# pramasoul/lac

Measured on AMD Instinct MI355X. Metric: encoded symbols/sec at vocab=32000, batch=4096 streams; bit-exact round-trip, higher is better.
Workload: dtype u32; 1 GPU; c3: vocab=32000, 4096 streams/GPU, 16 symbols/stream per job, prec=48, uint32 pmf rows; vocab=32000, streams=4096, prec=48, pmf_bits=32, input=pmf, parallelism=streams sharded over 1 GPU(s)

## Files before the change

include/lac.h:

```cpp
#ifndef LAC_H
#define LAC_H

#include <stdint.h>

#ifdef __cplusplus
extern "C" {
#endif

typedef struct lac_ctx lac_ctx;

enum {
    LAC_OK = 0,
    LAC_E_ARG = -1,
    LAC_E_PREC = -2,
    LAC_E_SYMBOL_RANGE = -3,
    LAC_E_ZERO_WIDTH = -4,
    LAC_E_TABLE = -5,
    LAC_E_DECODE_RANGE = -6,
    LAC_E_CAPACITY = -7,
    LAC_E_HIP = -8,
    LAC_E_STATE = -9,
    LAC_E_FLUSH_ZERO_WIDTH = -10,
    LAC_E_FLUSH_LOOP = -11,
    LAC_E_UNDETERMINED = -12
};

enum {
    LAC_OPT_ENCODE_PATH = 1,
    LAC_OPT_FUSED_MIN_STREAMS = 2,
    LAC_OPT_MAPPING = 3,
    LAC_OPT_TERMINATION = 4,
    LAC_OPT_DECODE_PATH = 5,
    LAC_OPT_Q1_SHAPE = 6,
    LAC_OPT_DECODE_FINE = 7,
    LAC_OPT_BLOCK_WAVES = 8,
    LAC_OPT_DECODE_STOP = 9,
    LAC_OPT_Q1_STEP = 10
};
enum {
    LAC_MAP_CEIL = 0,
    LAC_MAP_FLOOR = 1
};
enum {
    LAC_TERM_FLUSH = 0,
    LAC_TERM_ACSAMPLER = 1
};
enum {
    LAC_PATH_AUTO = 0,
    LAC_PATH_SPLIT = 1,
    LAC_PATH_FUSED = 2,
    LAC_PATH_STATS = 3,
    LAC_PATH_BLOCK = 4
};

const char *lac_version(void);
const char *lac_last_error(void);

int lac_open(int device, int prec, int64_t vocab, int64_t streams, int pmf_bits,
             uint64_t capacity_bits, lac_ctx **out);
int lac_close(lac_ctx *ctx);

int lac_set_option(lac_ctx *ctx, int option, int64_t value);

int lac_set_stream_lengths(lac_ctx *ctx, const int64_t *len_dev, void *stream);

int lac_encode_reset(lac_ctx *ctx, void *stream);

int lac_encode(lac_ctx *ctx, const void *pmf_dev, int64_t step_stride, int64_t stream_stride,
               const int32_t *sym_dev, int64_t steps, uint64_t *trace_dev, void *stream);

int lac_encode_job(lac_ctx *ctx, const void *pmf_dev, int64_t step_stride, int64_t stream_stride,
                   const int32_t *sym_dev, int64_t steps, uint64_t *trace_dev, void *stream);

int lac_encode_rebase(lac_ctx *ctx, void *stream);

int lac_encode_drain(lac_ctx *ctx, uint8_t *dst_dev, uint64_t dst_stride_bytes, uint64_t *fill_dev, void *stream);

int lac_encode_finish(lac_ctx *ctx, void *stream);

int lac_stream_status(lac_ctx *ctx, int32_t *err_host, int64_t *err_step_host, void *stream);

int lac_encoded_lengths(lac_ctx *ctx, uint64_t *nbits_host, void *stream);

int lac_encoded_device(lac_ctx *ctx, const uint8_t **bits_dev, uint64_t *stride_bytes,
                       const uint64_t **nbits_dev);

int lac_copy_bits(lac_ctx *ctx, uint8_t *dst_host, uint64_t dst_stride, void *stream);

int lac_copy_bits_dev(lac_ctx *ctx, uint8_t *dst_dev, uint64_t dst_stride, void *stream);

int lac_copy_nbits_dev(lac_ctx *ctx, uint64_t *dst_dev, void *stream);

int lac_pack_bits(lac_ctx *ctx, uint8_t *dst_dev, int hdr_bytes, uint64_t *len_dev, void *stream);

int lac_pack_bits_at(lac_ctx *ctx, uint8_t *dst_dev, uint64_t dst_bytes, int hdr_bytes, const uint64_t *base_dev,
                     uint64_t *end_dev, uint64_t *len_out, void *stream);

int lac_pack_jobs(int device, const uint64_t *planeA_dev, uint64_t plane_stride, const uint64_t *nbits_dev,
                  int64_t jobs, int64_t streams, uint64_t cap_words, uint8_t *dst_dev, uint64_t dst_bytes,
                  int hdr_bytes, const uint64_t *base_dev, uint64_t *ends_dev, uint64_t *lens_out, void *stream);

int lac_unpack_jobs(int device, const uint8_t *src_dev, uint64_t src_bytes, int hdr_bytes,
                    const uint64_t *counts_dev, const uint64_t *base_dev,
                    int64_t jobs, int64_t streams,
                    uint8_t *bits_dev, uint64_t stride_bytes, uint64_t job_stride_bytes,
                    uint64_t *nbits_dev, uint64_t *ends_dev, int32_t *status_dev, void *stream);

int lac_set_output(lac_ctx *ctx, uint64_t *planeA_dev, uint64_t *nbits_dev);

int lac_host_alloc(uint64_t bytes, void **host_out, void **dev_out);
int lac_host_free(void *host);

int lac_encoder_registers(lac_ctx *ctx, int64_t *l_host, int64_t *h_host, void *stream);

int lac_flush_digits(lac_ctx *ctx, int8_t *digits_host, int32_t *count_host, void *stream);

typedef struct lac_enc_state {
    int64_t l, h;
    uint64_t L, wa, wc;
    int64_t nsym;
    int32_t err, nflush;
    int64_t err_step;
    int8_t flush[8];
} lac_enc_state;
int lac_encode_get_state(lac_ctx *ctx, lac_enc_state *host_out, uint64_t *planes_host, void *stream);
int lac_encode_set_state(lac_ctx *ctx, const lac_enc_state *host_in, const uint64_t *planes_host, void *stream);

int lac_decode_open(lac_ctx *ctx, const uint8_t *bits_dev, uint64_t stride_bytes,
                    const uint64_t *nbits_dev, void *stream);

int lac_decode_open_packed(lac_ctx *ctx, const uint8_t *src_dev, uint64_t src_bytes, int hdr_bytes,
                           const uint64_t *counts_dev, const uint64_t *base_dev, uint64_t *end_dev,
                           void *stream);

int lac_decode_open_window(lac_ctx *ctx, const uint8_t *bits_dev, uint64_t stride_bytes,
                           const uint64_t *nbits_dev, const uint64_t *base_words_dev, void *stream);
int lac_decode_refill(lac_ctx *ctx, void *stream);
int lac_decode_window_base(lac_ctx *ctx, uint64_t *base_words_host, void *stream);

int lac_decode_step(lac_ctx *ctx, const void *pmf_dev, int64_t stream_stride,
                    int32_t *sym_out_dev, void *stream);

int lac_decode_steps(lac_ctx *ctx, const void *pmf_dev, int64_t step_stride, int64_t stream_stride,
                     int64_t steps, int32_t *sym_out_dev, void *stream);

#define LAC_LOGITS_BF16 1
#define LAC_LOGITS_F32 2

int lac_q1_k(int prec, int64_t vocab);

int lac_encode_logits_job(lac_ctx *ctx, const void *logits_dev, int logit_type, int64_t step_stride,
                          int64_t stream_stride, const int32_t *sym_dev, int64_t steps, uint64_t *trace_dev,
                          void *stream);

int lac_encode_logits(lac_ctx *ctx, const void *logits_dev, int logit_type, int64_t step_stride,
                      int64_t stream_stride, const int32_t *sym_dev, int64_t steps, uint64_t *trace_dev,
                      void *stream);

int lac_decode_logits_steps(lac_ctx *ctx, const void *logits_dev, int logit_type, int64_t step_stride,
                            int64_t stream_stride, int64_t steps, int32_t *sym_out_dev, void *stream);

int lac_decode_logits_step(lac_ctx *ctx, const void *logits_dev, int logit_type, int64_t stream_stride,
                           int32_t *sym_out_dev , void *stream);
int lac_encode_logits_step(lac_ctx *ctx, const void *logits_dev, int logit_type, int64_t stream_stride,
                           const int32_t *sym_dev , uint64_t *trace_dev, void *stream);

int lac_q1_group_aborted(lac_ctx *ctx, int64_t *aborted, void *stream);

int lac_quantize_logits(lac_ctx *ctx, const void *logits_dev, int logit_type, int64_t step_stride,
                        int64_t stream_stride, int64_t steps, uint32_t *pmf_out_dev, void *stream);

int lac_decode_determined(lac_ctx *ctx, int64_t *ndet_host, void *stream);

typedef struct lac_dec_state {
    int64_t l, h, x;
    uint64_t pos;
    int64_t nsym;
    int32_t err, det;
    int64_t err_step, ndet;
} lac_dec_state;

int lac_decode_get_state(lac_ctx *ctx, lac_dec_state *host_out, void *stream);
int lac_decode_set_state(lac_ctx *ctx, const lac_dec_state *host_in, void *stream);

#define LAC_TAIL_DECIDE 0
#define LAC_TAIL_FLUSH 1
typedef struct lac_tail_state {
    int64_t l, h, lb, hb;
    int32_t err, done;
    int64_t still, nsym;
} lac_tail_state;

int lac_decode_tail_begin(lac_ctx *ctx, void *stream);
int lac_decode_tail_step(lac_ctx *ctx, const void *pmf_dev, int64_t stream_stride, int mode,
                         int64_t *sym_out_dev, int32_t *code_out_dev, void *stream);
int lac_decode_tail_get_state(lac_ctx *ctx, lac_tail_state *host_out, void *stream);
int lac_decode_tail_set_state(lac_ctx *ctx, const lac_tail_state *host_in, void *stream);

int lac_hc_encode_symbol(int prec, int64_t *l, int64_t *h, int64_t lo, int64_t hi, int8_t *digits,
                         int32_t *ndigits);
int lac_hc_encode_flush(int prec, int64_t l, int64_t h, int8_t *digits, int32_t *ndigits);
int lac_hc_decode_emit(int prec, int64_t *regs, int64_t lo, int64_t hi, int renormalise);

int lac_profile_enable(lac_ctx *ctx, int on);
int lac_profile_read(lac_ctx *ctx, double *ms_total , int64_t *launches , int reset);

#ifdef __cplusplus
}
#endif
#endif
```

lac_amd/_lib.py:

```python
from __future__ import annotations

import ctypes as C
import os

HERE = os.path.dirname(os.path.abspath(__file__))
LIB_PATH = os.environ.get("LAC_LIB") or os.path.join(HERE, "liblac.so")

LAC_OK = 0
LAC_E_ARG = -1
LAC_E_PREC = -2
LAC_E_SYMBOL_RANGE = -3
LAC_E_ZERO_WIDTH = -4
LAC_E_TABLE = -5
LAC_E_DECODE_RANGE = -6
LAC_E_CAPACITY = -7
LAC_E_HIP = -8
LAC_E_STATE = -9
LAC_E_FLUSH_ZERO_WIDTH = -10
LAC_E_FLUSH_LOOP = -11
LAC_E_UNDETERMINED = -12

STATUS_NAMES = {
    LAC_OK: "LAC_OK", LAC_E_ARG: "LAC_E_ARG", LAC_E_PREC: "LAC_E_PREC",
    LAC_E_SYMBOL_RANGE: "LAC_E_SYMBOL_RANGE", LAC_E_ZERO_WIDTH: "LAC_E_ZERO_WIDTH",
    LAC_E_TABLE: "LAC_E_TABLE", LAC_E_DECODE_RANGE: "LAC_E_DECODE_RANGE",
    LAC_E_CAPACITY: "LAC_E_CAPACITY", LAC_E_HIP: "LAC_E_HIP", LAC_E_STATE: "LAC_E_STATE",
    LAC_E_FLUSH_ZERO_WIDTH: "LAC_E_FLUSH_ZERO_WIDTH", LAC_E_FLUSH_LOOP: "LAC_E_FLUSH_LOOP",
    LAC_E_UNDETERMINED: "LAC_E_UNDETERMINED",
}

_vp, _i, _i64, _u64 = C.c_void_p, C.c_int, C.c_int64, C.c_uint64
PROTOTYPES = [
    ("lac_version", C.c_char_p, []),
    ("lac_last_error", C.c_char_p, []),
    ("lac_open", _i, [_i, _i, _i64, _i64, _i, _u64, C.POINTER(_vp)]),
    ("lac_close", _i, [_vp]),
    ("lac_set_stream_lengths", _i, [_vp, _vp, _vp]),
    ("lac_encode_reset", _i, [_vp, _vp]),
    ("lac_encode", _i, [_vp, _vp, _i64, _i64, _vp, _i64, _vp, _vp]),
    ("lac_encode_job", _i, [_vp, _vp, _i64, _i64, _vp, _i64, _vp, _vp]),
    ("lac_set_option", _i, [_vp, _i, _i64]),
    ("lac_encode_finish", _i, [_vp, _vp]),
    ("lac_encode_rebase", _i, [_vp, _vp]),
    ("lac_encode_drain", _i, [_vp, _vp, _u64, _vp, _vp]),
    ("lac_stream_status", _i, [_vp, _vp, _vp, _vp]),
    ("lac_encoded_lengths", _i, [_vp, _vp, _vp]),
    ("lac_encoded_device", _i, [_vp, C.POINTER(_vp), C.POINTER(_u64), C.POINTER(_vp)]),
    ("lac_copy_bits", _i, [_vp, _vp, _u64, _vp]),
    ("lac_copy_bits_dev", _i, [_vp, _vp, _u64, _vp]),
    ("lac_copy_nbits_dev", _i, [_vp, _vp, _vp]),
    ("lac_pack_bits", _i, [_vp, _vp, C.c_int, _vp, _vp]),
    ("lac_pack_bits_at", _i, [_vp, _vp, _u64, C.c_int, _vp, _vp, _vp, _vp]),
    ("lac_pack_jobs", _i, [C.c_int, _vp, _u64, _vp, _i64, _i64, _u64, _vp, _u64, C.c_int, _vp, _vp, _vp, _vp]),
    ("lac_unpack_jobs", _i, [C.c_int, _vp, _u64, C.c_int, _vp, _vp, _i64, _i64, _vp, _u64, _u64, _vp, _vp, _vp, _vp]),
    ("lac_decode_open_packed", _i, [_vp, _vp, _u64, C.c_int, _vp, _vp, _vp, _vp]),
    ("lac_set_output", _i, [_vp, _vp, _vp]),
    ("lac_host_alloc", _i, [_u64, C.POINTER(_vp), C.POINTER(_vp)]),
    ("lac_host_free", _i, [_vp]),
    ("lac_encode_get_state", _i, [_vp, _vp, _vp, _vp]),
    ("lac_encode_set_state", _i, [_vp, _vp, _vp, _vp]),
    ("lac_flush_digits", _i, [_vp, _vp, _vp, _vp]),
    ("lac_encoder_registers", _i, [_vp, _vp, _vp, _vp]),
    ("lac_decode_open", _i, [_vp, _vp, _u64, _vp, _vp]),
    ("lac_decode_open_window", _i, [_vp, _vp, _u64, _vp, _vp, _vp]),
    ("lac_decode_refill", _i, [_vp, _vp]),
    ("lac_decode_window_base", _i, [_vp, _vp, _vp]),
    ("lac_decode_step", _i, [_vp, _vp, _i64, _vp, _vp]),
    ("lac_decode_steps", _i, [_vp, _vp, _i64, _i64, _i64, _vp, _vp]),
    ("lac_decode_determined", _i, [_vp, _vp, _vp]),
    ("lac_decode_get_state", _i, [_vp, _vp, _vp]),
    ("lac_decode_set_state", _i, [_vp, _vp, _vp]),
    ("lac_decode_tail_begin", _i, [_vp, _vp]),
    ("lac_decode_tail_step", _i, [_vp, _vp, _i64, _i, _vp, _vp, _vp]),
    ("lac_decode_tail_get_state", _i, [_vp, _vp, _vp]),
    ("lac_decode_tail_set_state", _i, [_vp, _vp, _vp]),
    ("lac_hc_encode_symbol", _i, [_i, _vp, _vp, _i64, _i64, _vp, _vp]),
    ("lac_hc_encode_flush", _i, [_i, _i64, _i64, _vp, _vp]),
    ("lac_hc_decode_emit", _i, [_i, _vp, _i64, _i64, _i]),
    ("lac_q1_group_aborted", _i, [_vp, _vp, _vp]),
    ("lac_profile_enable", _i, [_vp, _i]),
    ("lac_profile_read", _i, [_vp, _vp, _vp, _i]),
    ("lac_q1_k", _i, [_i, _i64]),
    ("lac_encode_logits_job", _i, [_vp, _vp, _i, _i64, _i64, _vp, _i64, _vp, _vp]),
    ("lac_encode_logits", _i, [_vp, _vp, _i, _i64, _i64, _vp, _i64, _vp, _vp]),
    ("lac_decode_logits_steps", _i, [_vp, _vp, _i, _i64, _i64, _i64, _vp, _vp]),
    ("lac_quantize_logits", _i, [_vp, _vp, _i, _i64, _i64, _i64, _vp, _vp]),
    ("lac_decode_logits_step", _i, [_vp, _vp, _i, _i64, _vp, _vp]),
    ("lac_encode_logits_step", _i, [_vp, _vp, _i, _i64, _vp, _vp, _vp]),
]

KERNEL_IDS = {"row_stats": 0, "encode": 1, "finish": 2, "decode_step": 3, "encode_fused": 4, "decode_wave": 5,
              "q1_stats": 6, "q1_decode": 7}
LAC_LOGITS_BF16, LAC_LOGITS_F32 = 1, 2
LAC_OPT_ENCODE_PATH = 1
LAC_OPT_FUSED_MIN_STREAMS = 2
LAC_PATH_AUTO, LAC_PATH_SPLIT, LAC_PATH_FUSED, LAC_PATH_STATS, LAC_PATH_BLOCK = 0, 1, 2, 3, 4
LAC_OPT_MAPPING = 3
LAC_OPT_TERMINATION = 4
LAC_OPT_DECODE_PATH = 5
LAC_OPT_Q1_SHAPE = 6
LAC_OPT_DECODE_FINE = 7
LAC_OPT_BLOCK_WAVES = 8
LAC_OPT_DECODE_STOP = 9
LAC_OPT_Q1_STEP = 10
Q1_STEP_MODES = {"auto": 0, "fused": 1, "split": 2}
LAC_MAP_CEIL, LAC_MAP_FLOOR = 0, 1
LAC_TERM_FLUSH, LAC_TERM_ACSAMPLER = 0, 1
LAC_TAIL_DECIDE, LAC_TAIL_FLUSH = 0, 1


class LacLibraryError(RuntimeError):
    pass


class LacError(RuntimeError):
    def __init__(self, code, msg=""):
        super().__init__(f"{STATUS_NAMES.get(code, code)}: {msg}")
        self.code = code


_lib = None


def load():
    global _lib
    if _lib is not None:
        return _lib
    if not os.path.exists(LIB_PATH):
        raise LacLibraryError(f"{LIB_PATH} is missing: build it with `python -m lac_amd.build` "
                              "(hipcc --offload-arch=gfx950); there is no CPU fallback")
    try:
        lib = C.CDLL(LIB_PATH)
    except OSError as e:
        raise LacLibraryError(f"cannot load {LIB_PATH}: {e}") from e
    for name, res, args in PROTOTYPES:
        try:
            f = getattr(lib, name)
        except AttributeError:
            if os.environ.get("LAC_LIB"):
                continue
            raise LacLibraryError(f"{LIB_PATH} lacks {name}: rebuild it (python -m lac_amd.build)") from None
        f.restype = res
        f.argtypes = args
    _lib = lib
    return lib


def check(rc):
    if rc != LAC_OK:
        raise LacError(rc, load().lac_last_error().decode(errors="replace"))
    return rc
```

lac_amd/batch.py:

```python
from __future__ import annotations

import ctypes as C
import sys

import numpy as np

from . import _lib
from ._lib import LacError, check



def _torch():
    import torch
    return torch


def _stream_handle(device):
    torch = _torch()
    return C.c_void_p(torch.cuda.current_stream(device).cuda_stream)


ENC_STATE = np.dtype([("l", "<i8"), ("h", "<i8"), ("L", "<u8"), ("wa", "<u8"), ("wc", "<u8"), ("nsym", "<i8"),
                      ("err", "<i4"), ("nflush", "<i4"), ("err_step", "<i8"), ("flush", "i1", (8,))])

# ... 208 lines not shown
            raise ValueError("lengths must fit int64")
        dev = torch.from_numpy(np.ascontiguousarray(n, dtype=np.int64)).to(self.device)
        check(self.lib.lac_set_stream_lengths(self.ctx, C.c_void_p(dev.data_ptr()), self._stream))
        self._len_keep = dev

    def lengths(self):
        n = np.zeros(self.streams, dtype=np.uint64)
        check(self.lib.lac_encoded_lengths(self.ctx, n.ctypes.data_as(C.c_void_p), self._stream))
        return n

    def device_bits(self):
        p, s, n = C.c_void_p(), C.c_uint64(), C.c_void_p()
        check(self.lib.lac_encoded_device(self.ctx, C.byref(p), C.byref(s), C.byref(n)))
        return p.value, s.value, n.value

    def bits_tensor(self, stride=None):
        torch = _torch()
        _, s, _ = self.device_bits()
        stride = int(stride or s)
        out = torch.zeros((self.streams, stride), dtype=torch.uint8, device=self.device)
        check(self.lib.lac_copy_bits_dev(self.ctx, C.c_void_p(out.data_ptr()), stride, self._stream))
        return out

    def bits_stride(self):
        return int(self.device_bits()[1])

    def copy_bits_into(self, out):
        if out.dim() != 2 or out.shape[0] != self.streams or out.stride(1) != 1 or out.dtype != _torch().uint8:
            raise ValueError("out must be a uint8 [streams, W] tensor with contiguous rows")
        check(self.lib.lac_copy_bits_dev(self.ctx, C.c_void_p(out.data_ptr()), out.stride(0), self._stream))
        return out

    def copy_nbits_into(self, out):
        if out.shape != (self.streams,) or not out.is_contiguous() or out.element_size() != 8:
            raise ValueError("out must be a contiguous 8-byte integer tensor [streams]")
        check(self.lib.lac_copy_nbits_dev(self.ctx, C.c_void_p(out.data_ptr()), self._stream))
        return out

    def pack_bits(self, out, hdr_bytes, length):
        if hdr_bytes not in (2, 4) or (hdr_bytes == 2 and self.bits_stride() * 8 >= 1 << 16):
            raise ValueError(f"hdr_bytes={hdr_bytes}: 2-byte headers need streams of < 65536 bits "
                             f"(this coder's hold {self.bits_stride() * 8}), else 4")
        need = self.streams * (hdr_bytes + self.bits_stride())
        if out.dtype != _torch().uint8 or not out.is_contiguous() or out.numel() < need or out.device != self.device:
            raise ValueError(f"out must be a contiguous uint8 device tensor of >= {need} bytes on {self.device}")
        if length.numel() != 1 or length.element_size() != 8 or length.device != self.device:
            raise ValueError("length must be a one-element 8-byte integer tensor on the coder's device")
        check(self.lib.lac_pack_bits(self.ctx, C.c_void_p(out.data_ptr()), int(hdr_bytes),
                                     C.c_void_p(length.data_ptr()), self._stream))
        return out, length

    def pack_bits_at(self, out, hdr_bytes, base, end, len_out=None):
        if hdr_bytes not in (2, 4) or (hdr_bytes == 2 and self.bits_stride() * 8 >= 1 << 16):
            raise ValueError(f"hdr_bytes={hdr_bytes}: 2-byte headers need streams of < 65536 bits "
                             f"(this coder's hold {self.bits_stride() * 8}), else 4")
        if out.dtype != _torch().uint8 or not out.is_contiguous() or out.device != self.device:
            raise ValueError(f"out must be a contiguous uint8 device tensor on {self.device}")
        for t in (base, end):
            if t is not None and (t.numel() < 1 or t.element_size() != 8 or t.device != self.device):
                raise ValueError("base / end must be 8-byte integer tensors on the coder's device")
        check(self.lib.lac_pack_bits_at(self.ctx, C.c_void_p(out.data_ptr()), out.numel(), int(hdr_bytes),
                                        None if base is None else C.c_void_p(base.data_ptr()),
                                        C.c_void_p(end.data_ptr()),
                                        None if len_out is None else C.c_void_p(int(len_out)), self._stream))
        return out

    def set_output(self, planes=None, nbits=None):
        if (planes is None) != (nbits is None):
            raise ValueError("planes and nbits: both or neither")
        if planes is not None:
            for t, n in ((planes, self.output_words()), (nbits, self.streams)):
                if t.element_size() != 8 or not t.is_contiguous() or t.numel() < n or t.device != self.device:
                    raise ValueError(f"output buffers: contiguous 8-byte tensors of >= {n} elements on {self.device}")
        check(self.lib.lac_set_output(self.ctx, None if planes is None else C.c_void_p(planes.data_ptr()),
                                      None if nbits is None else C.c_void_p(nbits.data_ptr())))
        self._output = (planes, nbits)

    def output_words(self):
        return self.streams * (self.bits_stride() // 8) + 1

    def nbits_tensor(self):
        torch = _torch()
        out = torch.empty((self.streams,), dtype=torch.int64, device=self.device)
        check(self.lib.lac_copy_nbits_dev(self.ctx, C.c_void_p(out.data_ptr()), self._stream))
        return out

    def to_bytes(self):
        self.raise_on_error()
        n = self.lengths()
        _, s, _ = self.device_bits()
        host = np.zeros((self.streams, s), dtype=np.uint8)
        check(self.lib.lac_copy_bits(self.ctx, host.ctypes.data_as(C.c_void_p), s, self._stream))
        return [host[b, :(int(n[b]) + 7) // 8].tobytes() for b in range(self.streams)], n

    def flush_digits(self):
        d = np.zeros((self.streams, 8), dtype=np.int8)
        c = np.zeros(self.streams, dtype=np.int32)
        check(self.lib.lac_flush_digits(self.ctx, d.ctypes.data_as(C.c_void_p), c.ctypes.data_as(C.c_void_p),
                                        self._stream))
        return [d[b, :max(int(c[b]), 0)].tolist() for b in range(self.streams)]

    def decode_open(self, bits=None, nbits=None):
        if bits is None:
            check(self.lib.lac_decode_open(self.ctx, None, 0, None, self._stream))
            self._dec_keep = None
            return
        torch = _torch()
        if bits.dtype != torch.uint8 or bits.device != self.device:
            raise TypeError("bits must be a uint8 tensor on the coder's device")
        if bits.dim() != 2 or bits.shape[0] != self.streams or bits.stride(1) != 1:
            raise ValueError("bits must be [streams, stride] with contiguous rows")
        if bits.stride(0) % 8 or bits.data_ptr() % 8:
            raise ValueError("bits rows must be 8-byte aligned (row stride a multiple of 8 bytes)")
        if nbits is None or nbits.dtype not in (torch.int64, torch.uint64) or nbits.device != self.device:
            raise TypeError("nbits must be an int64/uint64 tensor on the coder's device")
        if tuple(nbits.shape) != (self.streams,) or not nbits.is_contiguous():
            raise ValueError(f"nbits must be a contiguous [{self.streams}] tensor")
        self._dec_keep = (bits, nbits)
        check(self.lib.lac_decode_open(self.ctx, C.c_void_p(bits.data_ptr()), bits.stride(0),
                                       C.c_void_p(nbits.data_ptr()), self._stream))

    def decode_open_packed(self, payload, hdr_bytes, counts=None, base=None, end=None):
        torch = _torch()
        if hdr_bytes not in (0, 2, 4):
            raise ValueError(f"hdr_bytes={hdr_bytes}: 2 or 4, or 0 with counts")
        if payload.dtype != torch.uint8 or payload.dim() != 1 or not payload.is_contiguous() \
                or payload.device != self.device:
            raise ValueError(f"payload must be a contiguous 1-D uint8 device tensor on {self.device}")
        if payload.numel() == 0:
            raise ValueError("payload is empty")
        if hdr_bytes == 0:
            if counts is None or counts.element_size() != 8 or counts.is_floating_point() \
                    or counts.device != self.device:
                raise ValueError("hdr_bytes=0 needs counts: an 8-byte integer tensor on the coder's device")
            if tuple(counts.shape) != (self.streams,) or not counts.is_contiguous():
                raise ValueError(f"counts must be a contiguous [{self.streams}] tensor")
        for t in (base, end):
            if t is not None and (t.numel() < 1 or t.element_size() != 8 or t.device != self.device):
                raise ValueError("base / end must be 8-byte integer tensors on the coder's device")
        check(self.lib.lac_decode_open_packed(self.ctx, C.c_void_p(payload.data_ptr()), payload.numel(),
                                              int(hdr_bytes),
                                              C.c_void_p(counts.data_ptr()) if hdr_bytes == 0 else None,
                                              None if base is None else C.c_void_p(base.data_ptr()),
                                              None if end is None else C.c_void_p(end.data_ptr()), self._stream))
        self._dec_keep = None

    def decode_open_window(self, bits, nbits=None, base=None):
        torch = _torch()
        if isinstance(bits, HostBits):
            if bits.streams != self.streams or bits.device != self.device:
                raise ValueError("HostBits of another stream count or device")
            if bits.dev_addr is None:
                raise ValueError("HostBits is closed")
            ptr, stride, nbits = bits.dev_addr, bits.stride, bits.nbits
        else:
            if bits.dtype != torch.uint8 or bits.device != self.device:
                raise TypeError("bits must be a uint8 tensor on the coder's device")
            if bits.dim() != 2 or bits.shape[0] != self.streams or bits.stride(1) != 1:
                raise ValueError("bits must be [streams, stride] with contiguous rows")
            ptr, stride = bits.data_ptr(), bits.stride(0)
        if nbits is None or nbits.dtype not in (torch.int64, torch.uint64) or nbits.device != self.device:
            raise TypeError("nbits must be an int64/uint64 tensor on the coder's device")
        if tuple(nbits.shape) != (self.streams,) or not nbits.is_contiguous():
            raise ValueError(f"nbits must be a contiguous [{self.streams}] tensor")
        if base is not None and not isinstance(base, torch.Tensor):
            b = np.asarray(base)
            if b.shape != (self.streams,) or b.dtype.kind not in "iu" or (b.size and int(b.min()) < 0):
                raise ValueError(f"base must be {self.streams} integers >= 0")
            base = torch.from_numpy(np.ascontiguousarray(b).astype(np.int64)).to(self.device)
        if base is not None and (base.element_size() != 8 or base.is_floating_point() or base.device != self.device
                                 or tuple(base.shape) != (self.streams,) or not base.is_contiguous()):
            raise ValueError(f"base must be a contiguous 8-byte integer [{self.streams}] tensor on the coder's device")
        check(self.lib.lac_decode_open_window(self.ctx, C.c_void_p(ptr), stride, C.c_void_p(nbits.data_ptr()),
                                              None if base is None else C.c_void_p(base.data_ptr()), self._stream))
        self._dec_keep = (bits, nbits, base)

    def refill(self):
        check(self.lib.lac_decode_refill(self.ctx, self._stream))

    def window_base(self):
        n = np.zeros(self.streams, dtype=np.uint64)
        check(self.lib.lac_decode_window_base(self.ctx, n.ctypes.data_as(C.c_void_p), self._stream))
        return n

    def determined(self):
        n = np.zeros(self.streams, dtype=np.int64)
        check(self.lib.lac_decode_determined(self.ctx, n.ctypes.data_as(C.c_void_p), self._stream))
        return n

    def decode(self, pmf, out=None):
        torch = _torch()
        self._check_pmf(pmf)
        if pmf.dim() == 2:
            pmf = pmf.unsqueeze(0)
        if pmf.dim() != 3:
            raise ValueError("give decode a [steps, streams, V] (or expanded) table")
        if pmf.shape[1] not in (1, self.streams):
            raise ValueError(f"pmf must be [steps, {self.streams} or 1, {self.vocab}], got {tuple(pmf.shape)}")
        steps = pmf.shape[0]
        step_stride = pmf.stride(0) if steps > 1 else 0
        stream_stride = pmf.stride(1) if pmf.shape[1] > 1 else 0
        if out is None:
            out = torch.empty((steps, self.streams), dtype=torch.int32, device=self.device)
        else:
            self._check_out(out, steps)
        check(self.lib.lac_decode_steps(self.ctx, C.c_void_p(pmf.data_ptr()), step_stride, stream_stride, steps,
                                        C.c_void_p(out.data_ptr()), self._stream))
        return out


    def _logits_args(self, logits, steps=None):
        torch = _torch()
        typ = {torch.bfloat16: _lib.LAC_LOGITS_BF16, torch.float32: _lib.LAC_LOGITS_F32}.get(logits.dtype)
        if typ is None:
            raise TypeError(f"logits must be bfloat16 or float32, got {logits.dtype}")
        if logits.device != self.device:
            raise ValueError(f"logits are on {logits.device}, coder on {self.device}")
        if logits.dim() == 2:
            logits = logits.unsqueeze(0)
        if logits.dim() != 3 or logits.shape[1] not in (1, self.streams) or logits.shape[2] != self.vocab:
            raise ValueError(f"logits must be [steps, {self.streams}, {self.vocab}]")
        if logits.stride(2) != 1:
            raise ValueError("logit rows must be contiguous")
        n = logits.shape[0] if steps is None else steps
        if logits.shape[0] not in (1, n):
            raise ValueError("logits steps do not match the symbols")
        step_stride = logits.stride(0) if logits.shape[0] > 1 else 0
        stream_stride = logits.stride(1) if logits.shape[1] > 1 else 0
        return typ, step_stride, stream_stride, n, logits

    def _logits_encode_args(self, logits, sym, trace):
        torch = _torch()
        if sym.dtype != torch.int32 or sym.device != self.device:
            raise TypeError("sym must be an int32 tensor on the coder's device")
        sym = sym.contiguous()
        steps = sym.shape[0] if sym.dim() == 2 else 1
        if sym.numel() != steps * self.streams:
            raise ValueError(f"sym must be [steps, {self.streams}]")
        typ, ss, bs, steps, logits = self._logits_args(logits, steps)
        tp = None
        if trace is not None:
            if trace.dtype != torch.int64 or trace.numel() != steps * self.streams * 2 or not trace.is_contiguous():
                raise ValueError("trace must be a contiguous int64 tensor [steps, streams, 2]")
            tp = C.c_void_p(trace.data_ptr())
        self._keep = (logits, sym)
        return (self.ctx, C.c_void_p(logits.data_ptr()), typ, ss, bs, C.c_void_p(sym.data_ptr()), steps, tp,
                self._stream)

    def encode_logits(self, logits, sym, trace=None):
        check(self.lib.lac_encode_logits(*self._logits_encode_args(logits, sym, trace)))

    def encode_logits_job(self, logits, sym, trace=None):
        check(self.lib.lac_encode_logits_job(*self._logits_encode_args(logits, sym, trace)))

    def decode_logits(self, logits, out=None):
        torch = _torch()
        typ, ss, bs, steps, logits = self._logits_args(logits)
        if out is None:
            out = torch.empty((steps, self.streams), dtype=torch.int32, device=self.device)
        else:
            self._check_out(out, steps)
        check(self.lib.lac_decode_logits_steps(self.ctx, C.c_void_p(logits.data_ptr()), typ, ss, bs, steps,
                                               C.c_void_p(out.data_ptr()), self._stream))
        return out

    def _logits_step_args(self, logits):
        typ, _, bs, steps, logits = self._logits_args(logits)
        if steps != 1:
            raise ValueError(f"one position: logits must be [{self.streams}, {self.vocab}]")
        return typ, bs, logits

    def decode_logits_step(self, logits, out=None):
        torch = _torch()
        typ, bs, logits = self._logits_step_args(logits)
        if out is None:
            out = torch.empty((1, self.streams), dtype=torch.int32, device=self.device)
        else:
            self._check_out(out, 1)
        check(self.lib.lac_decode_logits_step(self.ctx, C.c_void_p(logits.data_ptr()), typ, bs,
                                              C.c_void_p(out.data_ptr()), self._stream))
        return out

    def encode_logits_step(self, logits, sym, trace=None):
        args = self._logits_encode_args(logits, sym, trace)
        if args[6] != 1:
            raise ValueError(f"one position: sym must be [{self.streams}]")
        check(self.lib.lac_encode_logits_step(*args[:3], args[4], args[5], args[7], args[8]))

    def set_q1_step(self, mode):
        v = _lib.Q1_STEP_MODES.get(mode, mode)
        check(self.lib.lac_set_option(self.ctx, _lib.LAC_OPT_Q1_STEP, int(v)))

    def quantize_logits(self, logits):
        torch = _torch()
        typ, ss, bs, steps, logits = self._logits_args(logits)
        out = torch.empty((steps, self.streams, self.vocab), dtype=torch.int32, device=self.device)
        check(self.lib.lac_quantize_logits(self.ctx, C.c_void_p(logits.data_ptr()), typ, ss, bs, steps,
                                           C.c_void_p(out.data_ptr()), self._stream))
        return out

    def set_q1_shape(self, shape: int):
        check(self.lib.lac_set_option(self.ctx, _lib.LAC_OPT_Q1_SHAPE, int(shape)))

    def q1_k(self):
        return int(self.lib.lac_q1_k(self.prec, self.vocab))


class DrainSink:

    def __init__(self, coder: BatchCoder, stage_bytes: int | None = None):
        torch = _torch()
        self.coder = coder
        self.stage_bytes = int(stage_bytes if stage_bytes is not None else coder.bits_stride())
        if self.stage_bytes <= 0 or self.stage_bytes % 8:
            raise ValueError("stage_bytes must be a positive multiple of 8")
        self.stage = torch.zeros((coder.streams, self.stage_bytes), dtype=torch.uint8, device=coder.device)
        self.fill = torch.zeros((coder.streams,), dtype=torch.int64, device=coder.device)
        self.parts = [bytearray() for _ in range(coder.streams)]

    def pull(self):
        self.coder.drain(self.stage, self.fill)
        n = self.fill.cpu().numpy()
        if n.any():
            host = self.stage[:, :int(n.max())].cpu().numpy()
            for b in np.flatnonzero(n):
                self.parts[b] += host[b, :int(n[b])].tobytes()
            self.fill.zero_()
        return n

    def finish(self):
        self.pull()
        self.coder.finish()
        tail, nb = self.coder.to_bytes()
        drained = np.array([len(p) for p in self.parts], dtype=np.uint64)
        return [bytes(p) + t for p, t in zip(self.parts, tail)], nb + 8 * drained


class HostBits:

    def __init__(self, data, nbits, device):
        torch = _torch()
        self.lib = _lib.load()
        self.device = torch.device(device)
        self.streams = len(data)
        nb = np.ascontiguousarray(np.asarray(nbits).astype(np.int64))
        if nb.shape != (self.streams,) or (nb.size and int(nb.min()) < 0):
            raise ValueError(f"nbits must be {self.streams} counts >= 0")
        for b, d in enumerate(data):
            if 8 * len(d) < int(nb[b]):
                raise ValueError(f"stream {b}: {len(d)} bytes hold fewer than {int(nb[b])} bits")
        self.stride = max(8, (max((len(d) for d in data), default=0) + 7) // 8 * 8)
        self.nbytes = self.stride * max(self.streams, 1)
        h, d = C.c_void_p(), C.c_void_p()
        with torch.cuda.device(self.device):
            check(self.lib.lac_host_alloc(self.nbytes, C.byref(h), C.byref(d)))
        self._h, self.dev_addr = h.value, d.value
        self.array = np.ctypeslib.as_array((C.c_uint8 * self.nbytes).from_address(self._h)) \
            .reshape(max(self.streams, 1), self.stride)
        self.array[...] = 0
        for b, s in enumerate(data):
            self.array[b, :len(s)] = np.frombuffer(s, dtype=np.uint8)
        self.nbits = torch.from_numpy(nb).to(self.device)

    def close(self):
        if getattr(self, "_h", None):
            self.array = None
            self.lib.lac_host_free(self._h)
            self._h = self.dev_addr = None

    def __del__(self):
        if sys is None or sys.is_finalizing():
            return
        try:
            self.close()
        except Exception:
            pass


def logits_row_multiple(dtype) -> int:
    torch = _torch()
    if dtype not in (torch.bfloat16, torch.float32):
        raise TypeError(f"logits must be bfloat16 or float32, got {dtype}")
    return 8 if dtype == torch.bfloat16 else 4


def pad_logits(logits):
    torch = _torch()
    m = logits_row_multiple(logits.dtype)
    V = logits.shape[-1]
    Vp = (V + m - 1) // m * m
    if Vp != V:
        logits = torch.nn.functional.pad(logits, (0, Vp - V), value=float("-inf"))
    return logits.contiguous()


def digits_of(E: int, k: int):
    if k <= 0:
        return []
    return [E >> (k - 1)] + [(E >> (k - 1 - i)) & 1 for i in range(1, k)]
```

lac_amd/csrc/lac_encode.hip:

```cpp
#include "lac_host.h"
#include "lac_drain.h"
#include "lac_wire.h"

#include <type_traits>

namespace {

#if LAC_ENC_PHASES
__device__ unsigned long long g_enc_phase[8];
#endif
constexpr int kEncUnroll = LAC_ENC_UNROLL;

template <typename E, int VEC>
__global__ __launch_bounds__(256) void k_row_stats(const E *__restrict__ pmf, int64_t step_stride,
                                                   int64_t stream_stride, const int32_t *__restrict__ sym,
                                                   int64_t B, int64_t rows, int64_t V, int64_t t0,
                                                   RowStats *__restrict__ out, const EncState *states,
                                                   const int64_t *__restrict__ slen) {
    const int lane = (int)lane_id();
    const int64_t r = (int64_t)blockIdx.x * kWavesPerBlock + (threadIdx.x >> 6);
    if (r >= rows) return;
    const int64_t t = t0 + r / B, b = r % B;
    if (slen && !live_row(slen, b, states[b].nsym, r / B)) return;
    const RowSums rs = row_reduce<E, VEC>(pmf + t * step_stride + b * stream_stride, V, sym[t * B + b]);
    if (lane == 0) {
        RowStats st;
        if (rs.T >> 64) {
            st.lo = st.hi = st.tot = 0;
            st.minp = 1;
        } else {
            st.lo = (uint64_t)rs.lo;
            st.hi = (uint64_t)rs.lo + rs.ps;
            st.tot = (uint64_t)rs.T;
            st.minp = rs.T ? rs.minp : 0;
        }
        st.inv_tot = st.tot ? 1.0 / (double)st.tot : 0.0;
        st.pad = 0;
        out[r] = st;
    }
}

struct SP {
    uint64_t lo, hi, tot, flo, fhi, fthr;
    int n, prec;
    uint64_t cap_words, *pa, *pc;
    int lane;
};
template <bool CEIL, bool T32, bool FT>
__device__ inline int straight_steps(const SP &sp, EncState &st, int64_t &l, int64_t &h, bool &ok) {
    auto store = [&](uint64_t idx, uint64_t wa, uint64_t wc) {
        if (sp.lane == 0) { sp.pa[idx] = wa; sp.pc[idx] = wc; }
    };
    typedef typename std::conditional<T32, uint32_t, uint64_t>::type CT;
    struct Row {
        CT lo, hi, T;
        uint64_t fl, fh, ft;
    };
    auto rd = [&](int j) {
        Row r;
        if constexpr (T32) {
            r.lo = (uint32_t)__builtin_amdgcn_readlane((int)(uint32_t)sp.lo, j);
            r.hi = (uint32_t)__builtin_amdgcn_readlane((int)(uint32_t)sp.hi, j);
            r.T = (uint32_t)__builtin_amdgcn_readlane((int)(uint32_t)sp.tot, j);
        } else {
            r.lo = readlane_u64(sp.lo, j);
            r.hi = readlane_u64(sp.hi, j);
            r.T = readlane_u64(sp.tot, j);
        }
        r.fl = readlane_u64(sp.flo, j);
        r.fh = readlane_u64(sp.fhi, j);
        r.ft = FT ? readlane_u64(sp.fthr, j) : 0;
        return r;
    };
    const int n = sp.n, prec = sp.prec;
    const int64_t nsym0 = st.nsym;
    Row nx = rd(0);
    int i = 0;
    int kk = 0;
    uint64_t e = 0;
    bool fudged = false;
    while (i < n) {
        for (; i < n; i++) {
            const Row r = LAC_ENC_PIPE ? nx : rd(i);
            if constexpr (LAC_ENC_PIPE) nx = rd(i + 1 < n ? i + 1 : i);
            const uint64_t w = (uint64_t)(h - l + 1);
            if constexpr (FT) {
                if (!nonneg_uni((int64_t)(w - r.ft))) {
                    fudged = true;
                    break;
                }
            }
            uint64_t a, bb;
            if constexpr (T32) {
                a = frac_mul_div32<CEIL>(r.fl, r.lo, w, r.T);
                bb = frac_mul_div32<CEIL>(r.fh, r.hi, w, r.T);
            } else {
                a = frac_mul_div<true>(r.fl, r.lo, w, r.T, CEIL);
                bb = frac_mul_div<true>(r.fh, r.hi, w, r.T, CEIL);
            }
            h = l + (int64_t)bb - 1;
            l = l + (int64_t)a;
            const uint64_t d = (uint64_t)(h - l);
            const int sh = bitlen64(d);
            kk = prec - sh;
            e = kk > 0 ? (uint64_t)l >> sh : 0;
            l = (int64_t)(((uint64_t)l - (e << sh)) << kk);
            h = l + (int64_t)((d + 1) << kk) - 1;
            const int off0 = (int)(st.L & 63);
            const int avail = off0 ? 64 - off0 : 0;
            if (__builtin_expect(kk > avail, 0)) break;
            st.wc |= (e >> kk) << ((64 - off0) & 63);
            st.wa |= (e & ((1ull << kk) - 1)) << ((64 - off0 - kk) & 63);
            st.L += (uint64_t)kk;
        }
        if (i >= n) break;
        if constexpr (FT) {
            if (fudged) break;
        }
        if (!plane_append(st.L, st.wa, st.wc, kk, e, sp.cap_words, store)) {
            st.err = LAC_E_CAPACITY;
            ok = false;
            break;
        }
        i++;
    }
    st.nsym = nsym0 + i;
    return i;
}

template <typename E, int MAP>
__global__ __launch_bounds__(256) void k_encode(const RowStats *__restrict__ stats, const int32_t *__restrict__ sym,
                                                int64_t B, int64_t t0, int64_t nsteps, const E *pmf,
                                                int64_t step_stride, int64_t stream_stride, int64_t V, int prec,
                                                EncState *states, uint64_t *planeA, uint64_t *planeC,
                                                uint64_t cap_words, uint64_t *trace, int mapping,
                                                bool allow_fudge, const int64_t *__restrict__ slen) {
    const int lane = (int)lane_id();
    const int64_t b = (int64_t)blockIdx.x * kWavesPerBlock + wave_in_block();
    if (b >= B) return;
    EncState st = states[b];
    if (slen) {
        nsteps = live_steps(slen, b, st.nsym, nsteps);
        if (nsteps == 0) return;
    }
    if (st.err || st.nflush >= 0) {
        if (lane == 0 && !st.err && st.nflush >= 0) { st.err = LAC_E_STATE; st.err_step = st.nsym; states[b] = st; }
        return;
    }
    uint64_t *pa = planeA + (uint64_t)b * cap_words, *pc = planeC + (uint64_t)b * cap_words;
    int64_t l = (int64_t)rfl_u64((uint64_t)st.l), h = (int64_t)rfl_u64((uint64_t)st.h);
    st.L = rfl_u64(st.L);
    st.wa = rfl_u64(st.wa);
    st.wc = rfl_u64(st.wc);
    st.nsym = (int64_t)rfl_u64((uint64_t)st.nsym);
#if LAC_ENC_PHASES
    PhaseClock clock, *clk = &clock;
    clock.start();
#else
    NoClock *clk = nullptr;
#endif
    bool ok = true;
    for (int64_t g0 = 0; g0 < nsteps && ok; g0 += 64) {
        const int n = (int)((nsteps - g0) < 64 ? (nsteps - g0) : 64);
        RowStats my = {0, 0, 0, 0, 0.0, 0};
        int32_t mys = 0;
        if (lane < n) {
            my = stats[(g0 + lane) * B + b];
            mys = sym[(t0 + g0 + lane) * B + b];
        }
        const bool frac_ok = lane < n && !(my.tot >> 62);
        const uint64_t flo = frac_ok ? row_frac(my.lo, my.tot) : kNoFrac;
        const uint64_t fhi = frac_ok ? row_frac(my.hi, my.tot) : kNoFrac;
        int i0 = 0;
#if LAC_ENC_STRAIGHT
        if constexpr (sizeof(E) == 8) {
            const uint64_t half = 1ull << (prec - 1);
            const bool lfast = lane >= n || (frac_ok && my.tot != 0 && my.hi > my.lo && (uint32_t)mys < (uint32_t)V &&
                                             (MAP != LAC_MAP_FLOOR || ((my.tot - 1) >> (prec - 1)) < my.hi - my.lo));
            const uint64_t d0 = (uint64_t)(h - l);
            if (!trace && prec <= 61 && __ballot(!lfast) == 0 && nonneg_uni((int64_t)(d0 - half)) &&
                !(d0 >> prec)) {
                constexpr bool CEIL = MAP != LAC_MAP_FLOOR;
                const bool t32 = __ballot(lane < n && (my.tot >> 32)) == 0;
                const bool ft = CEIL && __ballot(lane < n && my.tot > half) != 0;
                uint64_t ftl = 0;
                if (ft) {
                    ftl = lane < n && my.minp ? div_floor((u128)my.tot + (my.minp - 1), my.minp) : 0;
                    ftl = ftl < (1ull << 62) ? ftl : (1ull << 62);
                }
                SP sp{my.lo, my.hi, my.tot, flo, fhi, ftl, n, prec, cap_words, pa, pc, lane};
                if (t32)
                    i0 = ft ? straight_steps<CEIL, true, true>(sp, st, l, h, ok)
                            : straight_steps<CEIL, true, false>(sp, st, l, h, ok);
                else
                    i0 = ft ? straight_steps<CEIL, false, true>(sp, st, l, h, ok)
                            : straight_steps<CEIL, false, false>(sp, st, l, h, ok);
                if (!ok || i0 >= n) continue;
            }
        }
        if (i0 == 0) {
            const uint64_t half = 1ull << (prec - 1);
            const bool lfast = lane >= n || (frac_ok && my.tot != 0 && my.tot <= half && !(my.tot >> 32) &&
                                             my.hi > my.lo && (uint32_t)mys < (uint32_t)V);
            const uint64_t d0 = (uint64_t)(h - l);
            if (!trace && prec <= 61 && __ballot(!lfast) == 0 && nonneg_uni((int64_t)(d0 - half)) &&
                !(d0 >> prec)) {
                constexpr bool CEIL = MAP != LAC_MAP_FLOOR;
                const int64_t nsym0 = st.nsym;
                auto store = [&](uint64_t idx, uint64_t wa, uint64_t wc) {
                    if (lane == 0) { pa[idx] = wa; pc[idx] = wc; }
                };
                auto rd = [&](int j, uint32_t &lo, uint32_t &hi, uint32_t &T, uint64_t &fl, uint64_t &fh) {
                    lo = (uint32_t)__builtin_amdgcn_readlane((int)(uint32_t)my.lo, j);
                    hi = (uint32_t)__builtin_amdgcn_readlane((int)(uint32_t)my.hi, j);
                    T = (uint32_t)__builtin_amdgcn_readlane((int)(uint32_t)my.tot, j);
                    fl = readlane_u64(flo, j);
                    fh = readlane_u64(fhi, j);
                };
                uint32_t nlo, nhi, nT;
                uint64_t nfl, nfh;
                if constexpr (LAC_ENC_PIPE) rd(0, nlo, nhi, nT, nfl, nfh);
                int i = 0;
                int kk = 0;
                uint64_t e = 0;
                while (i < n) {
                    for (; i < n; i++) {
                        uint32_t lo, hi, T;
                        uint64_t fl, fh;
                        if constexpr (LAC_ENC_PIPE) {
                            lo = nlo, hi = nhi, T = nT, fl = nfl, fh = nfh;
                            rd(i + 1 < n ? i + 1 : i, nlo, nhi, nT, nfl, nfh);
                        } else {
                            rd(i, lo, hi, T, fl, fh);
                        }
                        const uint64_t w = (uint64_t)(h - l + 1);
                        const uint64_t a = frac_mul_div32<CEIL>(fl, lo, w, T), bb = frac_mul_div32<CEIL>(fh, hi, w, T);
                        h = l + (int64_t)bb - 1;
                        l = l + (int64_t)a;
                        const uint64_t d = (uint64_t)(h - l);
                        const int sh = bitlen64(d);
                        kk = prec - sh;
                        e = kk > 0 ? (uint64_t)l >> sh : 0;
                        l = (int64_t)(((uint64_t)l - (e << sh)) << kk);
                        h = l + (int64_t)((d + 1) << kk) - 1;
                        const int off0 = (int)(st.L & 63);
                        const int avail = off0 ? 64 - off0 : 0;
                        if (__builtin_expect(kk > avail, 0)) break;
                        st.wc |= (e >> kk) << ((64 - off0) & 63);
                        st.wa |= (e & ((1ull << kk) - 1)) << ((64 - off0 - kk) & 63);
                        st.L += (uint64_t)kk;
                    }
                    if (i >= n) break;
                    if (!plane_append(st.L, st.wa, st.wc, kk, e, cap_words, store)) {
                        st.err = LAC_E_CAPACITY;
                        ok = false;
                        break;
                    }
                    i++;
                }
                st.nsym = nsym0 + i;
                continue;
            }
        }
#endif
        uint64_t fthr = lane < n && my.minp ? div_floor((u128)my.tot + (my.minp - 1), my.minp) : 0;
        fthr = fthr < (1ull << 62) ? fthr : (1ull << 62);
        if (clk) clk->mark(4);
        for (int i = i0; i < n; i++) {
            const uint64_t lo = readlane_u64(my.lo, i), hi = readlane_u64(my.hi, i);
            const uint64_t T = readlane_u64(my.tot, i), minp = readlane_u64(my.minp, i);
            const uint64_t invb = readlane_u64(__builtin_bit_cast(uint64_t, my.inv_tot), i);
            const uint64_t fl = readlane_u64(flo, i), fh = readlane_u64(fhi, i), ft = readlane_u64(fthr, i);
            const int64_t s = __builtin_amdgcn_readlane(mys, i);
            const int64_t t = t0 + g0 + i;
            const E *row = pmf + t * step_stride + b * stream_stride;
            if (clk) clk->mark(0);
            if (!coder_step<E, true>(st, l, h, lo, hi, T, minp, s, row, V, prec, pa, pc, cap_words,
                                     trace ? trace + 2 * (t * B + b) : nullptr, lane, MAP,
                                     __builtin_bit_cast(double, invb), allow_fudge, fl, fh, ft, clk)) {
                ok = false;
                break;
            }
        }
    }
    if (lane == 0) store_state(st, l, h, pa, pc, cap_words, &states[b]);
#if LAC_ENC_PHASES
    if (lane == 0) {
        for (int k = 0; k < 5; k++) atomicAdd(&g_enc_phase[k], (unsigned long long)clock.acc[k]);
        atomicAdd(&g_enc_phase[6], (unsigned long long)st.nsym);
    }
#endif
}


template <typename E, int VEC>
__global__ LAC_ENC_BOUNDS void k_encode_fused(const E *__restrict__ pmf, int64_t step_stride,
                                                      int64_t stream_stride, const int32_t *__restrict__ sym,
                                                      int64_t B, int64_t t0, int64_t nsteps, int64_t V, int prec,
                                                      EncState *states, uint64_t *planeA, uint64_t *planeC,
                                                      uint64_t cap_words, uint64_t *trace, uint64_t *nbits, int flags,
                                                      int mapping, int term, const int64_t *__restrict__ slen) {
    const int lane = (int)lane_id();
    const int64_t b = (int64_t)blockIdx.x * kStreamWaves + (threadIdx.x >> 6);
    if (b >= B) return;
    EncState st = (flags & kReset) ? fresh_state(prec) : states[b];
    uint64_t *pa = planeA + (uint64_t)b * cap_words, *pc = planeC + (uint64_t)b * cap_words;
    if (slen) nsteps = live_steps(slen, b, st.nsym, nsteps);
    if (st.err || st.nflush >= 0) {
        if (!st.err && st.nflush >= 0 && nsteps > 0) { st.err = LAC_E_STATE; st.err_step = st.nsym; }
        if (lane == 0) {
            states[b] = st;
            if (flags & kFinish) nbits[b] = st.err ? 0 : st.L;
        }
        return;
    }
    int64_t l = st.l, h = st.h;
    RowGroup<E, VEC> buf;
    if (LAC_XPF && nsteps > 0) row_group_load<E, VEC>(buf, pmf + t0 * step_stride + b * stream_stride, 0, V / VEC);
    for (int64_t i = 0; i < nsteps; i++) {
        const int64_t t = t0 + i;
        const E *row = pmf + t * step_stride + b * stream_stride;
#if LAC_XPF
        const E *next = i + 1 < nsteps ? row + step_stride : nullptr;
#else
        const E *next = nullptr;
        row_group_load<E, VEC>(buf, row, 0, V / VEC);
#endif
        const int64_t s = sym[t * B + b];
        const RowSums rs = row_reduce_pf<E, VEC>(row, V, s, buf, next);
        if (rs.T >> 64) { st.err = LAC_E_TABLE; break; }
        const uint64_t lo = (uint64_t)rs.lo;
        if (!coder_step<E>(st, l, h, lo, lo + rs.ps, (uint64_t)rs.T, rs.minp, s, row, V, prec, pa, pc, cap_words,
                           trace ? trace + 2 * (t * B + b) : nullptr, lane, mapping))
            break;
    }
    if (lane == 0) {
        store_state(st, l, h, pa, pc, cap_words, &st);
        if (flags & kFinish) finish_stream(st, pa, pc, cap_words, prec, &nbits[b], term);
        states[b] = st;
    }
}

__global__ __launch_bounds__(256) void k_finish(EncState *states, uint64_t *planeA, uint64_t *planeC,
                                                uint64_t cap_words, int64_t B, int prec, uint64_t *nbits, int term) {
    const int64_t b = (int64_t)blockIdx.x * blockDim.x + threadIdx.x;
    if (b >= B) return;
    EncState st = states[b];
    finish_stream(st, planeA + (uint64_t)b * cap_words, planeC + (uint64_t)b * cap_words, cap_words, prec, &nbits[b],
                  term);
    states[b] = st;
}

__device__ inline uint64_t block_excl_sum1024(uint64_t v, uint64_t *wsum, uint64_t &total) {
    const int w = threadIdx.x >> 6;
    const uint64_t inc = wave_incl_scan_u64(v);
    if ((threadIdx.x & 63) == 63) wsum[w] = inc;
    __syncthreads();
    uint64_t before = 0;
    total = 0;
    for (int i = 0; i < 16; i++) {
        const uint64_t x = wsum[i];
        before += i < w ? x : 0;
        total += x;
    }
    __syncthreads();
    return before + inc - v;
}

__global__ __launch_bounds__(1024) void k_pack(const uint64_t *__restrict__ planes, uint64_t pstride,
                                               uint64_t cap_words, const uint64_t *__restrict__ nbits_all,
                                               int64_t B, int hdr, uint8_t *__restrict__ dst, uint64_t dst_bytes,
                                               const uint64_t *__restrict__ base_in, uint64_t *__restrict__ ends,
                                               uint64_t *__restrict__ lens) {
    __shared__ uint64_t wsum[16];
    const int t = threadIdx.x;
    const int64_t job = blockIdx.y, first = (int64_t)blockIdx.x * 1024, b = first + t;
    const uint64_t *nbits = nbits_all + job * B;
    const uint64_t *planeA = planes + job * pstride;
    const uint64_t nb = b < B ? nbits[b] : 0, n = (nb + 7) >> 3, nw = (n + 7) >> 3;
    const uint64_t *src = planeA + (uint64_t)(b < B ? b : 0) * cap_words;
    uint64_t w4[4];
#pragma unroll
    for (int i = 0; i < 4; i++) w4[i] = (uint64_t)i < nw ? src[i] : 0;
    const uint64_t base0 = base_in ? *base_in : 0;
    uint64_t pj = 0, pw = 0, all = 0;
    for (int64_t k = t; k < (job + 1) * B; k += 1024) {
        const uint64_t m = (nbits_all[k] + 7) >> 3;
        const int64_t kj = k / B, kb = k - kj * B;
        pj += kj < job ? m : 0;
        pw += kj == job && kb < first ? m : 0;
        all += kj == job ? m : 0;
    }
    uint64_t tj, tw, ta, tb;
    (void)block_excl_sum1024(pj, wsum, tj);
    (void)block_excl_sum1024(pw, wsum, tw);
    (void)block_excl_sum1024(all, wsum, ta);
    const uint64_t excl = block_excl_sum1024(n, wsum, tb);
    const uint64_t hB = (uint64_t)hdr * (uint64_t)B, total = hB + ta;
    const uint64_t start = base0 + (uint64_t)job * hB + tj;
    const uint64_t before_ws = tw;
    const bool fits = start <= dst_bytes && total <= dst_bytes - start;
    if (blockIdx.x == 0 && t == 0) {
        ends[job] = fits ? start + total : start;
        if (lens) lens[job] = fits ? total : ~0ull;
    }
    if (!fits || b >= B) return;
    uint8_t *h = dst + start + (uint64_t)b * hdr;
    for (int i = 0; i < hdr; i++) h[i] = (uint8_t)(nb >> (8 * i));
    uint8_t *d = dst + start + hB + before_ws + excl;
    for (uint64_t wi = 0; wi < nw; wi++) {
        const uint64_t v = wi >= 4 ? src[wi] : wi == 0 ? w4[0] : wi == 1 ? w4[1] : wi == 2 ? w4[2] : w4[3];
        const uint64_t m = n - wi * 8 < 8 ? n - wi * 8 : 8;
        for (uint64_t k = 0; k < m; k++) d[wi * 8 + k] = (uint8_t)(v >> (8 * k));
    }
}

constexpr int kUnpackThreads = 256;

__device__ inline uint64_t unpack_sat_sum(uint64_t v, uint64_t *wsum) {
    const uint64_t s = wave_reduce(v, [](uint64_t a, uint64_t b) { return wire::sat_add(a, b); });
    if ((threadIdx.x & 63) == 0) wsum[threadIdx.x >> 6] = s;
    __syncthreads();
    uint64_t total = 0;
    for (int i = 0; i < kUnpackThreads / 64; i++) total = wire::sat_add(total, wsum[i]);
    __syncthreads();
    return total;
}

__device__ inline uint64_t unpack_excl_scan(uint64_t v, uint64_t *wsum) {
    const int w = threadIdx.x >> 6;
    const uint64_t inc = wave_incl_scan_u64(v);
    if ((threadIdx.x & 63) == 63) wsum[w] = inc;
    __syncthreads();
    uint64_t before = 0;
    for (int i = 0; i < kUnpackThreads / 64; i++) before += i < w ? wsum[i] : 0;
    __syncthreads();
    return before + inc - v;
}

template <int HDR>
__device__ inline void unpack_sum_counts(const uint8_t *__restrict__ src, uint64_t start,
                                         const uint64_t *__restrict__ ck, int64_t B, int64_t first, bool own,
                                         uint64_t stride, uint64_t &all, uint64_t &pw, int &ov) {
#pragma unroll 8
    for (int64_t b = threadIdx.x; b < B; b += kUnpackThreads) {
        const uint64_t nb = wire::read_count(src, start, HDR, ck, b);
        const uint64_t m = wire::stream_bytes(nb);
        all = wire::sat_add(all, m);
        pw = wire::sat_add(pw, own && b < first ? m : 0);
        ov |= own && !wire::stream_fits(nb, stride);
    }
}

__global__ __launch_bounds__(kUnpackThreads) void k_unpack(const uint8_t *__restrict__ src, uint64_t src_bytes, int hdr,
                                                           const uint64_t *__restrict__ counts,
                                                           const uint64_t *__restrict__ base_in, int64_t B,
                                                           uint8_t *__restrict__ bits, uint64_t stride,
                                                           uint64_t job_stride, uint64_t *__restrict__ nbits_out,
                                                           uint64_t *__restrict__ ends, int32_t *__restrict__ status) {
    constexpr int T = kUnpackThreads;
    __shared__ uint64_t wsum[T / 64];
    __shared__ uint64_t s_off[T], s_n[T];
    const int t = threadIdx.x;
    const int64_t job = blockIdx.y, first = (int64_t)blockIdx.x * T;
    wire::Walk w{base_in ? *base_in : 0, true};
    uint64_t before = 0, end = 0;
    int over = 0;
    for (int64_t k = 0; k <= job; k++) {
        if (!wire::walk_header(w, hdr, B, src_bytes)) break;
        const uint64_t *ck = counts ? counts + k * B : nullptr;
        uint64_t all = 0, pw = 0;
        int ov = 0;
        if (hdr == 2) unpack_sum_counts<2>(src, w.start, ck, B, first, k == job, stride, all, pw, ov);
        else if (hdr == 4) unpack_sum_counts<4>(src, w.start, ck, B, first, k == job, stride, all, pw, ov);
        else unpack_sum_counts<0>(src, w.start, ck, B, first, k == job, stride, all, pw, ov);
        const uint64_t payload = unpack_sat_sum(all, wsum);
        if (!wire::walk_payload(w, hdr, B, payload, src_bytes)) break;
        if (k < job) {
            w.start = wire::job_end(w, hdr, B, payload);
        } else {
            before = unpack_sat_sum(pw, wsum);
            over = __syncthreads_or(ov);
            end = wire::job_end(w, hdr, B, payload);
        }
    }
    const int64_t b = first + t;
    uint64_t nb = wire::kNone, m = 0;
    bool sf = false;
    if (w.fits && b < B) {
        nb = wire::read_count(src, w.start, hdr, counts ? counts + job * B : nullptr, b);
        m = wire::stream_bytes(nb);
        sf = wire::stream_fits(nb, stride);
    }
    const uint64_t excl = unpack_excl_scan(m, wsum);
    s_off[t] = w.start + wire::header_bytes(hdr, B) + before + excl;
    s_n[t] = sf ? m : 0;
    if (blockIdx.z == 0) {
        if (b < B) nbits_out[job * B + b] = nb;
        if (blockIdx.x == 0 && t == 0) {
            if (ends) ends[job] = w.fits ? end : w.start;
            if (status) status[job] = wire::job_status(w.fits, over != 0);
        }
    }
    __syncthreads();
    const uint64_t W = stride >> 3;
    const int64_t ns = B - first < T ? B - first : T;
    uint64_t *dst = reinterpret_cast<uint64_t *>(bits + (uint64_t)job * job_stride + (uint64_t)first * stride);
    if (W >= (uint64_t)T) {
        const uint64_t chunk = (W + gridDim.z - 1) / gridDim.z;
        const uint64_t lo = blockIdx.z * chunk, hi = lo + chunk < W ? lo + chunk : W;
        for (int64_t s = 0; s < ns; s++) {
            const uint64_t off = s_off[s], n = s_n[s];
            for (uint64_t wi = lo + t; wi < hi; wi += T) dst[(uint64_t)s * W + wi] = wire::slot_word(src, off, n, wi);
        }
    } else {
        const uint32_t Wn = (uint32_t)W, total = (uint32_t)ns * Wn;
        for (uint32_t q = t; q < total; q += T) {
            const uint32_t s = q / Wn, wi = q - s * Wn;
            dst[q] = wire::slot_word(src, s_off[s], s_n[s], wi);
        }
    }
}

__global__ void k_enc_rebase(EncState *states, int64_t B) {
    const int64_t b = (int64_t)blockIdx.x * blockDim.x + threadIdx.x;
    if (b >= B) return;
    EncState st = states[b];
    if (st.L > 64) st.L = ((st.L - 1) & 63) + 1;
    states[b] = st;
}

__global__ __launch_bounds__(64 * kWavesPerBlock) void k_enc_drain(EncState *states, uint64_t *planeA,
                                                                   uint64_t *planeC, uint64_t cap_words, int64_t B,
                                                                   int prec, uint8_t *dst, uint64_t dst_stride,
                                                                   uint64_t *fill) {
    const int lane = (int)lane_id();
    const int64_t b = (int64_t)blockIdx.x * kWavesPerBlock + wave_in_block();
    if (b >= B) return;
    const EncState st = states[b];
    if (drain::is_idle(__builtin_amdgcn_readfirstlane(st.err), __builtin_amdgcn_readfirstlane(st.nflush),
                       rfl_u64(st.L)))
        return;
    const uint64_t L = rfl_u64(st.L), wlast = (L - 1) >> 6;
    if (wlast >= cap_words) return;
    const uint64_t wa = rfl_u64(st.wa), wc = rfl_u64(st.wc);
    uint64_t *pa = planeA + (uint64_t)b * cap_words, *pc = planeC + (uint64_t)b * cap_words;
    uint64_t g = 0, sg = 0, cy = 0;
    const bool certain = drain::is_certain((int64_t)rfl_u64((uint64_t)st.l), (int64_t)rfl_u64((uint64_t)st.h), prec);
    if (certain) {
        g = wlast;
        sg = drain::resolve_word(wa, wc, 0, &cy);
    } else {
        for (uint64_t top = wlast; top > 0; top = top > 64 ? top - 64 : 0) {
            const bool in = (uint64_t)lane < top;
            const uint64_t i = in ? top - 1 - (uint64_t)lane : 0;
            const uint64_t a = pa[i], c = pc[i];
            uint64_t co;
            const uint64_t s = drain::resolve_word(a, c, 0, &co);
            const uint64_t m = __ballot(in && drain::is_guard(a, c));
            if (m) {
                const int first = __builtin_ctzll(m);
                g = top - 1 - (uint64_t)first;
                sg = rfl_u64(shfl_u64(s, first));
                cy = (__ballot(co != 0) >> first) & 1;
                break;
            }
        }
    }
    if (g == 0) return;
    const uint64_t f = rfl_u64(fill[b]);
    if (!drain::slot_fits(g, f, dst_stride)) return;
    uint64_t *out = reinterpret_cast<uint64_t *>(dst + (uint64_t)b * dst_stride + f);
    uint64_t carry = cy;
    for (uint64_t top = g; top > 0; top = top > 64 ? top - 64 : 0) {
        const bool in = (uint64_t)lane < top;
        const uint64_t i = in ? top - 1 - (uint64_t)lane : 0;
        const uint64_t a0 = pa[i], c0 = pc[i];
        const uint64_t a = in ? a0 : 0, c = in ? c0 : 0;
        uint64_t co;
        const uint64_t s = drain::resolve_word(a, c, 0, &co);
        const uint64_t gen = __ballot(co != 0), prop = __ballot(s == ~0ull);
        uint64_t cout;
        const uint64_t cin = drain::block_carries(gen, prop, carry, &cout);
        if (in) out[i] = drain::to_big_endian(s + ((cin >> lane) & 1));
        carry = cout;
    }
// ... 344 lines not shown
```

lac_amd/csrc/lac_logits.hip:

```cpp
#include "lac_host.h"
#include "lac_dec_dev.h"

namespace {

__constant__ uint32_t c_q1_tab[LAC_Q1_TAB_SIZE] = LAC_Q1_TAB_INIT;

#ifndef LAC_Q1_NT
#define LAC_Q1_NT 1
#endif
#ifndef LAC_Q1_DMA_NT
#define LAC_Q1_DMA_NT LAC_Q1_NT
#endif
#if LAC_Q1_DMA_NT
#define LAC_Q1_DMA_POLICY " nt"
#else
#define LAC_Q1_DMA_POLICY ""
#endif
#ifndef LAC_Q1_DEC_DIRECT
#define LAC_Q1_DEC_DIRECT 1
#endif
#ifndef LAC_Q1_SCHED
#define LAC_Q1_SCHED 0
#endif
#ifndef LAC_Q1_DEFER_DEC
#define LAC_Q1_DEFER_DEC 0
#endif

typedef uint32_t u32x4 __attribute__((ext_vector_type(4)));
typedef short s16x2 __attribute__((ext_vector_type(2)));
__device__ inline s16x2 as_s16x2(uint32_t w) {
    s16x2 r;
    __builtin_memcpy(&r, &w, 4);
    return r;
}
#ifndef LAC_Q1_IMAX
#define LAC_Q1_IMAX 1
#endif

template <typename LT> struct LogitN { static constexpr int N = 16 / sizeof(LT); };

template <typename LT>
__device__ inline float logit_at(const u32x4 &v, int j) {
    if constexpr (sizeof(LT) == 2) {
        const uint32_t w = v[j >> 1];
        return __uint_as_float((j & 1) ? (w & 0xFFFF0000u) : (w << 16));
    } else {
        return __uint_as_float(v[j]);
    }
}

__device__ inline u32x4 ld16(const void *row, int64_t vi, bool nt) {
    const u32x4 *p = reinterpret_cast<const u32x4 *>(row) + vi;
    return nt ? __builtin_nontemporal_load(p) : *p;
}

constexpr int kQ1L = LAC_Q1_DMAX * LAC_Q1_STEPS;

__device__ inline uint32_t cvt_sat_u32(float y) {
    uint32_t r;
    asm("v_cvt_u32_f32 %0, %1" : "=v"(r) : "v"(y));
    return r;
}
__device__ inline float q1_c(float m) { return (float)kQ1L - (float)LAC_Q1_STEPS * m; }
__device__ inline uint32_t q1_j(float x, float c) {
    const uint32_t j = cvt_sat_u32(fmaf(x, (float)LAC_Q1_STEPS, c));
    return j < (uint32_t)kQ1L ? j : (uint32_t)kQ1L;
}
__device__ inline bool q1_fast_row(float m) { return fabsf(m) < 0x1p18f; }

__device__ inline uint32_t q1_entry(int j, uint32_t xsh) {
    const uint32_t v = c_q1_tab[kQ1L - j] >> xsh;
    return v ? v : 1u;
}

__device__ inline void q1_load_tab(uint32_t *tab, uint32_t xsh) {
    for (int i = threadIdx.x; i < LAC_Q1_TAB_SIZE; i += blockDim.x) tab[i] = q1_entry(i, xsh);
    __syncthreads();
}
__device__ inline uint32_t q1_val(float x, float c, const uint32_t *tab) { return tab[q1_j(x, c)]; }

#ifndef LAC_Q1_REP
#define LAC_Q1_REP 32
#endif
#ifndef LAC_Q1_MINW
#define LAC_Q1_MINW 4
#endif
constexpr int kQ1Rep = LAC_Q1_REP;
#ifndef LAC_Q1_FASTFILL
#define LAC_Q1_FASTFILL 1
#endif
template <int REP = kQ1Rep>
__device__ inline void q1_load_tab_rep(uint32_t *tabr, uint32_t xsh) {
    for (int i = threadIdx.x; i < LAC_Q1_TAB_SIZE * REP; i += blockDim.x) tabr[i] = q1_entry(i / REP, xsh);
    __syncthreads();
}
template <int REP, int NTHR>
__device__ inline void q1_fill_tab_rep(uint32_t *tabr, uint32_t xsh) {
    if constexpr (!LAC_Q1_FASTFILL) {
        q1_load_tab_rep<REP>(tabr, xsh);
    } else {
        static_assert(REP % 4 == 0, "16-B writes of copies");
        constexpr int Q = REP / 4, ITEMS = LAC_Q1_TAB_SIZE * Q, IT = (ITEMS + NTHR - 1) / NTHR;
        uint32_t v[IT];
#pragma unroll
        for (int k = 0; k < IT; k++) {
            const int item = (int)threadIdx.x + k * NTHR;
            v[k] = item < ITEMS ? c_q1_tab[kQ1L - item / Q] : 0u;
        }
#pragma unroll
        for (int k = 0; k < IT; k++) {
            const int item = (int)threadIdx.x + k * NTHR;
            uint32_t e = v[k] >> xsh;
            e = e ? e : 1u;
            if (item < ITEMS) reinterpret_cast<u32x4 *>(tabr)[item] = u32x4{e, e, e, e};
        }
        __syncthreads();
    }
}

template <int REP = kQ1Rep>
__device__ inline uint32_t q1_rep_at(const uint32_t *tabr, uint32_t j, uint32_t loff) {
    return *reinterpret_cast<const uint32_t *>(reinterpret_cast<const char *>(tabr) + ((j * (REP * 4)) | loff));
}

typedef float f32x2 __attribute__((ext_vector_type(2)));

template <typename LT, int REP = kQ1Rep>
__device__ inline uint32_t q1_vec_sum(const u32x4 &x, float c, bool fast, const uint32_t *tabr, uint32_t loff) {
    constexpr int N = LogitN<LT>::N;
    uint32_t s = 0;
    if (fast) {
        const f32x2 k = {(float)LAC_Q1_STEPS, (float)LAC_Q1_STEPS}, cc = {c, c};
#pragma unroll
        for (int j = 0; j < N; j += 2) {
            const f32x2 v = {logit_at<LT>(x, j), logit_at<LT>(x, j + 1)};
            const f32x2 y = __builtin_elementwise_fma(v, k, cc);
            s += q1_rep_at<REP>(tabr, cvt_sat_u32(y.x), loff);
            s += q1_rep_at<REP>(tabr, cvt_sat_u32(y.y), loff);
        }
    } else {
#pragma unroll
        for (int j = 0; j < N; j++) s += q1_rep_at<REP>(tabr, q1_j(logit_at<LT>(x, j), c), loff);
    }
    return s;
}

__device__ inline float wave_max_f32(float v) {
    auto mx = [](uint32_t a, uint32_t b) { return __float_as_uint(fmaxf(__uint_as_float(a), __uint_as_float(b))); };
    return __uint_as_float(wave_reduce(__float_as_uint(v), mx));
}

template <int R>
__device__ inline uint64_t wave_multi_sum(uint64_t (&v)[R]) {
    const int lane = (int)lane_id();
    int m = 32;
#pragma unroll
    for (int live = R; live > 1; live >>= 1, m >>= 1) {
        const bool upper = lane & m;
#pragma unroll
        for (int i = 0; i < live / 2; i++) {
            const uint64_t keep = upper ? v[i + live / 2] : v[i];
            const uint64_t give = upper ? v[i] : v[i + live / 2];
            v[i] = keep + shfl_xor_u64(give, m);
        }
    }
    uint64_t r = v[0];
#pragma unroll
    for (int k = 32 / R; k >= 1; k >>= 1) r += shfl_xor_u64(r, k);
    return r;
}

template <int R, int BIT>
__device__ inline void multi_halve(uint32_t (&v)[R]) {
    if constexpr ((R >> BIT) > 1) {
        constexpr int live = R >> BIT;
        const bool upper = (lane_id() >> BIT) & 1;
#pragma unroll
        for (int i = 0; i < live / 2; i++) {
            const uint32_t keep = upper ? v[i + live / 2] : v[i];
            const uint32_t give = upper ? v[i] : v[i + live / 2];
            v[i] = keep + xor_dpp<BIT>(give);
        }
        multi_halve<R, BIT + 1>(v);
    }
}

__device__ inline uint64_t cross_row_sum64(uint32_t r) {
    const auto a = __builtin_amdgcn_permlane16_swap(r, r, false, false);
    const uint64_t r2 = (uint64_t)a[0] + a[1];
    const auto lo = __builtin_amdgcn_permlane32_swap((uint32_t)r2, (uint32_t)r2, false, false);
    const auto hi = __builtin_amdgcn_permlane32_swap((uint32_t)(r2 >> 32), (uint32_t)(r2 >> 32), false, false);
    return (((uint64_t)hi[0] << 32) | lo[0]) + (((uint64_t)hi[1] << 32) | lo[1]);
}

template <int R>
__device__ inline uint64_t wave_multi_sum32(uint32_t (&v)[R]) {
    static_assert(R >= 1 && R <= 16 && (R & (R - 1)) == 0, "R: power of two <= 16");
    multi_halve<R, 0>(v);
    uint32_t r = v[0];
    if constexpr (R < 2) r += xor_dpp<0>(r);
    if constexpr (R < 4) r += xor_dpp<1>(r);
    if constexpr (R < 8) r += xor_dpp<2>(r);
    if constexpr (R < 16) r += xor_dpp<3>(r);
    return cross_row_sum64(r);
}
template <int BIT>
__device__ inline uint32_t halve_pair(uint32_t lo, uint32_t hi) {
    const bool upper = (lane_id() >> BIT) & 1;
    return (upper ? hi : lo) + xor_dpp<BIT>(upper ? lo : hi);
}
__device__ inline uint64_t wave_multi_sum32_tail8(uint32_t r) {
    r += xor_dpp<3>(r);
    return cross_row_sum64(r);
}
constexpr int kHalveOrder[8] = {0, 4, 2, 6, 1, 5, 3, 7};

template <int R>
__device__ inline int q_index(int lane) {
    int idx = 0;
#pragma unroll
    for (int b = 0; (1 << b) < R; b++) idx |= ((lane >> b) & 1) << (__builtin_ctz(R) - 1 - b);
    return idx;
}


__device__ inline u32x4 neg_inf16(int type_bytes) {
    const uint32_t w = type_bytes == 2 ? 0xFF80FF80u : 0xFF800000u;
    return u32x4{w, w, w, w};
}
template <bool BUF, int TB> struct RowSrc;
template <int TB> struct RowSrc<true, TB> {
    __amdgpu_buffer_rsrc_t rs;
    int nvec;
    __device__ RowSrc(const void *row, bool, int nv)
        : rs(__builtin_amdgcn_make_buffer_rsrc(const_cast<void *>(row), 0, nv * 16, 0x00020000)), nvec(nv) {}
    __device__ u32x4 operator()(int vi) const {
        const uint32_t v = (uint32_t)(vi < nvec ? vi : nvec - 1);
        return __builtin_amdgcn_raw_buffer_load_b128(rs, v * 16u, 0, LAC_Q1_NT ? 2 : 0);
    }
};
template <int TB> struct RowSrc<false, TB> {
    const void *row;
    bool ok;
    int nvec;
    __device__ RowSrc(const void *r, bool v, int nv) : row(r), ok(v), nvec(nv) {}
    __device__ u32x4 operator()(int vi) const { return ok && vi < nvec ? ld16(row, vi, LAC_Q1_NT) : neg_inf16(TB); }
};

constexpr int kQ1Waves = 8;

template <int R, typename Src>
__device__ inline void q1_load_tile(u32x4 (&x)[R], const Src &src, int base, int gt, int NT) {
#pragma unroll
    for (int j = 0; j < R; j++) x[j] = src(base + gt + NT * j);
}

template <typename LT, int RW, int R, bool DEC, bool MULTI, bool PF, int NWB>
__global__ __launch_bounds__(64 * NWB, LAC_Q1_MINW) void k_q1_stats(const LT *__restrict__ lg, int64_t step_stride,
                                                              int64_t stream_stride, const int32_t *__restrict__ sym,
                                                              int64_t B, int64_t rows, int64_t V, int64_t t0,
                                                              uint32_t xsh, int64_t G, RowStats *__restrict__ out,
                                                              uint64_t *__restrict__ chunks,
                                                              float *__restrict__ mrow, const uint64_t *gate) {
    if (gate && __hip_atomic_load(gate, __ATOMIC_RELAXED, __HIP_MEMORY_SCOPE_AGENT) == 0) return;
    constexpr int N = LogitN<LT>::N, NT = 64 * RW, NR = NWB / RW;
    constexpr bool IMAX = LAC_Q1_IMAX && sizeof(LT) == 2 && NR == 1 && !MULTI;
    constexpr bool BUF = R <= 8 && !MULTI;
    typedef RowSrc<BUF, sizeof(LT)> Src;
    static_assert(R * N <= 128, "lane sums must fit 32 bits");
    __shared__ uint32_t tabr[LAC_Q1_TAB_SIZE * kQ1Rep];
    constexpr bool DIRECT = DEC && !MULTI && RW * R == 64 && !LAC_Q1_DEFER_DEC && LAC_Q1_DEC_DIRECT;
    __shared__ float smax[2][NWB];
    __shared__ int smaxi[2][NWB];
    __shared__ uint64_t ssum[NWB][2];
    __shared__ uint32_t sps[NR];
    __shared__ unsigned long long bins[DEC ? NR : 1][64];
    const int tid = threadIdx.x, lane = tid & 63, w = BUF ? wave_in_block() : tid >> 6;
    const int g = NR == 1 ? 0 : w / RW, wg = NR == 1 ? w : w % RW;
    int gt = tid - g * NT;
    if (DEC && wg == 0) bins[g][lane] = 0;
    const int nvec = (int)(V / N);
    const int ntiles = MULTI ? (nvec + NT * R - 1) / (NT * R) : 1;
    const int64_t stride = (int64_t)gridDim.x * NR;
    auto row_of = [&](int64_t r) { return lg + (t0 + r / B) * step_stride + (r % B) * stream_stride; };
    u32x4 x[R];
    if (PF) {
        const int64_t r0 = (int64_t)blockIdx.x * NR + g;
        q1_load_tile<R>(x, Src(r0 < rows ? row_of(r0) : lg, r0 < rows, nvec), 0, gt, NT);
    }
    if constexpr (R > 8) q1_load_tab_rep<kQ1Rep>(tabr, xsh);
    else q1_fill_tab_rep<kQ1Rep, 64 * NWB>(tabr, xsh);
    const uint32_t loff = (uint32_t)(lane & (kQ1Rep - 1)) << 2;
    auto ld_vec = [&](const Src &src, int tile, int j) { return src(tile * NT * R + gt + NT * j); };
    constexpr bool DEFER = DEC && LAC_Q1_DEFER_DEC;
    uint64_t pend_tot = 0;
    float pend_m = 0.f;
    int64_t pend_r = -1;
    auto flush_pending = [&]() {
        if (DEFER && pend_r >= 0) {
            chunks[pend_r * 64 + lane] = pend_tot;
            if (lane == 0) mrow[pend_r] = pend_m;
            pend_r = -1;
        }
    };
    int par = 0;
    for (int64_t rb = (int64_t)blockIdx.x * NR; rb < rows; rb += stride, par ^= 1) {
        if (R > 8 && !DEC) asm volatile("" : "+v"(gt));
        const int64_t r = rb + g;
        const bool valid = r < rows;
        const Src row(valid ? row_of(r) : lg, valid, nvec);
        float mx = -INFINITY;
        if (MULTI) {
            for (int tile = 0; tile < ntiles; tile++) {
                if (!PF) q1_load_tile<R>(x, row, tile * NT * R, gt, NT);
#pragma unroll
                for (int j = 0; j < R; j++) {
#pragma unroll
                    for (int e = 0; e < N; e++) mx = fmaxf(mx, logit_at<LT>(x[j], e));
                    if (PF && tile + 1 < ntiles) {
                        x[j] = ld_vec(row, tile + 1, j);
                        __builtin_amdgcn_sched_barrier(0);
                    }
                }
            }
        } else {
            if (!PF) q1_load_tile<R>(x, row, 0, gt, NT);
            if constexpr (!IMAX) {
#pragma unroll
                for (int j = 0; j < R; j++)
#pragma unroll
                    for (int e = 0; e < N; e++) mx = fmaxf(mx, logit_at<LT>(x[j], e));
            }
        }
        float m;
        if constexpr (IMAX) {
            s16x2 pm = {(short)-32768, (short)-32768};
#pragma unroll
            for (int j = 0; j < R; j++) {
                pm = __builtin_elementwise_max(pm, as_s16x2(x[j].x));
                pm = __builtin_elementwise_max(pm, as_s16x2(x[j].y));
                pm = __builtin_elementwise_max(pm, as_s16x2(x[j].z));
                pm = __builtin_elementwise_max(pm, as_s16x2(x[j].w));
            }
            const int li = pm.x > pm.y ? (int)pm.x : (int)pm.y;
            const int wi = (int)wave_reduce((uint32_t)li, [](uint32_t a, uint32_t b) {
                return (uint32_t)((int)a > (int)b ? (int)a : (int)b);
            });
            if (lane == 0) smaxi[par][w] = wi;
            if (!DEC && gt == 0) sps[g] = 0;
            __syncthreads();
            int bi = smaxi[par][0];
#pragma unroll
            for (int i = 1; i < NWB; i++) bi = smaxi[par][i] > bi ? smaxi[par][i] : bi;
            if (bi >= 0 && bi <= 0x7F80) {
                m = __uint_as_float((uint32_t)bi << 16);
            } else {
#pragma unroll
                for (int j = 0; j < R; j++)
#pragma unroll
                    for (int e = 0; e < N; e++) mx = fmaxf(mx, logit_at<LT>(x[j], e));
                mx = wave_max_f32(mx);
                if (lane == 0) smax[par][w] = mx;
                __syncthreads();
                m = smax[par][0];
#pragma unroll
                for (int i = 1; i < NWB; i++) m = fmaxf(m, smax[par][i]);
            }
        } else {
            mx = wave_max_f32(mx);
            if (lane == 0) smax[par][w] = mx;
            if (!DEC && gt == 0) sps[g] = 0;
            __syncthreads();
            m = smax[par][g * RW];
#pragma unroll
            for (int i = 1; i < RW; i++) m = fmaxf(m, smax[par][g * RW + i]);
        }
        const bool fast = q1_fast_row(m);
        const float c = q1_c(m);
        flush_pending();
        int sfull = -1, sr = 0;
        if (!DEC && valid) {
            const int64_t s = sym[(t0 + r / B) * B + r % B];
            const int sc = (int)(s < 0 ? 0 : (s > V ? V : s));
            sfull = sc / N;
            sr = sc - sfull * N;
        }
        uint32_t tot = 0, lo = 0;
        if (sizeof(LT) == 2) {
#pragma unroll
            for (int j = 0; j < R; j++) asm volatile("" : "+v"(x[j]));
        }
        for (int tile = ntiles - 1; tile >= 0; tile--) {
            if (MULTI && !PF && tile != ntiles - 1) q1_load_tile<R>(x, row, tile * NT * R, gt, NT);
            uint32_t sv[R];
            auto take = [&](int j, uint32_t sl) {
                const int vi = tile * NT * R + gt + NT * j;
                sl = vi < nvec ? sl : 0;
                if (DEC) {
                    sv[j] = sl;
                } else {
                    tot += sl;
                    lo += vi < sfull ? sl : 0;
                    if (vi == sfull) {
                        uint32_t pl = 0, ps = 0;
#pragma unroll
                        for (int e = 0; e < N; e++) {
                            const uint32_t q = q1_rep_at(tabr, q1_j(logit_at<LT>(x[j], e), c), loff);
                            pl += e < sr ? q : 0;
                            ps += e == sr ? q : 0;
                        }
                        lo += pl;
                        sps[g] = ps;
                    }
                }
            };
            const int64_t rn = r + stride;
            const bool nvalid = rn < rows;
            const bool down = MULTI && tile > 0;
            const Src rroll = down ? row : Src(nvalid ? row_of(rn) : lg, nvalid, nvec);
            const int troll = down ? tile - 1 : 0;
            auto roll = [&](int j) {
                if (PF) {
                    x[j] = ld_vec(rroll, troll, j);
                    __builtin_amdgcn_sched_barrier(0);
                }
            };
            constexpr bool STREAM = DEC && R == 8;
            auto pair_halve = [&](int k) {
                if constexpr (STREAM) {
                    if (k == 4) sv[0] = halve_pair<0>(sv[0], sv[4]);
                    if (k == 6) { sv[2] = halve_pair<0>(sv[2], sv[6]); sv[0] = halve_pair<1>(sv[0], sv[2]); }
                    if (k == 5) sv[1] = halve_pair<0>(sv[1], sv[5]);
                    if (k == 7) {
                        sv[3] = halve_pair<0>(sv[3], sv[7]);
                        sv[1] = halve_pair<1>(sv[1], sv[3]);
                        sv[0] = halve_pair<2>(sv[0], sv[1]);
                    }
                }
            };
            if (fast) {
#pragma unroll
                for (int q = 0; q < R; q++) {
                    const int j = STREAM ? kHalveOrder[q] : q;
                    take(j, q1_vec_sum<LT>(x[j], c, true, tabr, loff));
                    if (q > 0) pair_halve(STREAM ? kHalveOrder[q - 1] : q - 1);
                    roll(j);
                }
            } else {
#pragma unroll
                for (int q = 0; q < R; q++) {
                    const int j = STREAM ? kHalveOrder[q] : q;
                    take(j, q1_vec_sum<LT>(x[j], c, false, tabr, loff));
                    if (q > 0) pair_halve(STREAM ? kHalveOrder[q - 1] : q - 1);
                    roll(j);
                }
            }
            pair_halve(STREAM ? kHalveOrder[R - 1] : R - 1);
            if (DEC) {
                uint64_t gsum;
                if constexpr (STREAM) gsum = wave_multi_sum32_tail8(sv[0]);
                else gsum = wave_multi_sum32<R>(sv);
                if constexpr (DIRECT) {
                    const int grp = wg + RW * q_index<R>(lane);
                    if (lane < R && valid) chunks[r * 64 + grp] = grp * 64 < nvec ? gsum : 0;
                } else if (lane < R) {
                    const int grp = tile * RW * R + wg + RW * q_index<R>(lane);
                    if (grp * 64 < nvec) atomicAdd(&bins[g][grp / (int)G], (unsigned long long)gsum);
                }
            }
        }
        if (!DEC) {
            const uint64_t t64 = wave_sum_u64(tot), l64 = wave_sum_u64(lo);
            if (lane == 0) { ssum[w][0] = t64; ssum[w][1] = l64; }
        }
        if constexpr (DIRECT) {
            if (valid && w == 0 && lane == 0) mrow[r] = m;
        } else {
            __syncthreads();
        }
        if (DEC) {
            if (!DIRECT && wg == 0) {
                if constexpr (DEFER) {
                    pend_tot = bins[g][lane];
                    pend_m = m;
                    pend_r = valid ? r : -1;
                } else {
                    if (valid) chunks[r * 64 + lane] = bins[g][lane];
                    if (valid && lane == 0) mrow[r] = m;
                }
                bins[g][lane] = 0;
            }
        } else if (gt == 0 && valid) {
            uint64_t T = 0, L = 0;
#pragma unroll
            for (int i = 0; i < RW; i++) { T += ssum[g * RW + i][0]; L += ssum[g * RW + i][1]; }
            RowStats st;
            st.lo = L;
            st.hi = L + sps[g];
            st.tot = T;
            st.minp = 1;
            st.inv_tot = 1.0 / (double)T;
            st.pad = 0;
            out[r] = st;
        }
    }
    flush_pending();
}

typedef __attribute__((address_space(3))) void lvoid_t;

constexpr uint32_t kGroupSpinMax = 1u << 17;

#ifndef LAC_Q1_DEFER
#define LAC_Q1_DEFER 1
#endif

__device__ inline uint64_t group_ld(const uint64_t *p) {
    return __hip_atomic_load(p, __ATOMIC_RELAXED, __HIP_MEMORY_SCOPE_AGENT);
}

template <int NRB>
__device__ inline void group_post(uint64_t *xch, int g, uint32_t seq, uint32_t m) {
    const unsigned b = blockIdx.x;
    __hip_atomic_store(&xch[2 * (b * NRB + g) + (seq & 1)], ((uint64_t)seq << 32) | m, __ATOMIC_RELAXED,
                       __HIP_MEMORY_SCOPE_AGENT);
}
template <int NRB, typename Op>
__device__ inline uint32_t group_poll(uint64_t *xch, uint64_t *abortw, int g, int kg, uint32_t seq, uint32_t m,
                                      Op op, bool *ok) {
    const unsigned b = blockIdx.x, sl = seq & 1, xcd = b & 7, q = (b >> 3) * NRB + g, q0 = (q / kg) * kg;
    const unsigned lane = (unsigned)lane_fresh();
    const unsigned pq = q0 + lane;
    uint32_t val = m;
    bool fine = true;
    if (lane < (unsigned)kg && pq != q && group_ld(abortw) == 0) {
        const unsigned pb = (pq / NRB) * 8 + xcd;
        const uint64_t *px = &xch[2 * (pb * NRB + pq % NRB) + sl];
        uint64_t v = group_ld(px);
        uint32_t n = 0;
        for (; (uint32_t)(v >> 32) != seq && n < kGroupSpinMax; n++) {
            __builtin_amdgcn_s_sleep(2);
            if ((n & 63) == 63 && group_ld(abortw)) break;
            v = group_ld(px);
        }
        if ((uint32_t)(v >> 32) != seq) {
            fine = false;
            if (n >= kGroupSpinMax)
                __hip_atomic_store(abortw, (uint64_t)1, __ATOMIC_RELAXED, __HIP_MEMORY_SCOPE_AGENT);
        }
        val = (uint32_t)v;
    } else if (lane < (unsigned)kg && pq != q) {
        fine = false;
    }
    *ok = __ballot(!fine) == 0;
    return wave_reduce(val, op);
}

__device__ inline uint32_t f32_max_bits(uint32_t a, uint32_t b) {
    return __float_as_uint(fmaxf(__uint_as_float(a), __uint_as_float(b)));
}

__device__ inline void group_add(uint64_t *p, uint64_t v) {
    (void)__hip_atomic_fetch_add(p, v, __ATOMIC_RELAXED, __HIP_MEMORY_SCOPE_AGENT);
}
constexpr uint64_t kGroupPoison = 1ull << 62;

template <typename LT, bool DEC, int REP = kRLRep, int LASTN = 1024, int NT = 1024, bool GROUP = false>
__global__ __launch_bounds__(1024, 4) void k_q1_stats_rl(const LT *__restrict__ lg, int64_t step_stride,
                                                         int64_t stream_stride, const int32_t *__restrict__ sym,
                                                         int64_t B, int64_t rows, int64_t V, int64_t t0, uint32_t xsh,
                                                         int64_t G, RowStats *__restrict__ out,
                                                         uint64_t *__restrict__ chunks, float *__restrict__ mrow,
                                                         uint64_t *__restrict__ xch, int split, int kg, int rpx) {
    constexpr int N = LogitN<LT>::N, R = 8, L = 8, NW = 16, NRB = 1024 / NT, NWR = NT / 64;
    constexpr int SL = (L - 1) * NT + LASTN;
    constexpr bool IMAX = LAC_Q1_IMAX && sizeof(LT) == 2;
    static_assert(R == kRLRegVec && L == kRLSlots, "q1_slot_cap (lac_select.h) counts these vectors");
    static_assert((R + L) * N <= 128, "lane sums must fit 32 bits");
    constexpr bool DEFER = LAC_Q1_DEFER && !(sizeof(LT) == 2 && REP == kRLRep);
    static_assert(NT == 256 || NT == 512 || NT == 1024, "rows of 4, 8 or 16 waves");
    static_assert(LASTN % 64 == 0 && LASTN <= NT, "the last slot is trimmed by whole waves");
    constexpr bool TRIM = LASTN < NT;
    __shared__ uint32_t tabr[LAC_Q1_TAB_SIZE * REP];
    __shared__ u32x4 slots[NRB * SL];
    __shared__ float smax[NW];
    __shared__ int smaxi[NW];
    __shared__ uint64_t ssum[NW][2];
    __shared__ uint32_t sps[NRB];
    __shared__ unsigned long long gtot[DEC ? NRB * NWR * (R + L) : 1];
    int tid = threadIdx.x;
    const int lane = tid & 63, w = wave_in_block();
    const int g = w / NWR, wg = w % NWR;
    q1_load_tab_rep<REP>(tabr, xsh);
    const uint32_t loff = (uint32_t)(lane & (REP - 1)) << 2;
    const int sq = (int)(blockIdx.x >> 3) * NRB + g;
    const int hh = GROUP ? sq % kg : 0;
    const bool idle = GROUP && sq / kg >= rpx;
    const int vofs = hh * split;
    const int nvec = GROUP ? (idle ? 1 : hh < kg - 1 ? split : (int)(V / N) - (kg - 1) * split) : (int)(V / N);
    const bool noslot = TRIM && wg * 64 >= LASTN;
    const int64_t stride = GROUP ? 8 * (int64_t)rpx : (int64_t)gridDim.x * NRB;
    const int64_t b0 = GROUP ? 0 : (int64_t)blockIdx.x * NRB;
    const int64_t roff = GROUP ? (int64_t)(sq / kg) * 8 + (blockIdx.x & 7) : g;
    auto row_of = [&](int64_t r) {
        return lg + (t0 + r / B) * step_stride + (r % B) * stream_stride + (int64_t)vofs * N;
    };
    __shared__ uint32_t sxv[NRB];
    __shared__ int sxok[NRB];
    __shared__ int sxact[NRB];
    uint32_t seq = 0;
    bool pok = true;
    auto group_post_v = [&](uint32_t v, bool act) {
        seq += act ? 1 : 0;
        if (act && tid == g * NT) group_post<NRB>(xch, g, seq, v);
    };
    auto group_poll_v = [&](uint32_t v, bool act, auto op) {
        if (wg == 0) {
            bool ok = true;
            const uint32_t res = act ? group_poll<NRB>(xch, xch + 2 * NRB * gridDim.x, g, kg, seq, v, op, &ok) : v;
            if (tid == g * NT) {
                sxv[g] = res;
                sxok[g] = ok;
                sxact[g] = act;
            }
        }
        __syncthreads();
        pok = pok && sxok[g] != 0;
        return sxv[g];
    };
    auto group_combine = [&](uint32_t v, bool act, auto op) {
        group_post_v(v, act);
        return group_poll_v(v, act, op);
    };
    int64_t pend_r = -1;
    uint64_t pend = 0;
    auto flush_chunks = [&]() {
        if (pend_r < 0) return;
        const int ln = lane_fresh();
        if constexpr (GROUP) {
            if (pend) group_add(&chunks[pend_r * 64 + ln], pend);
        } else {
            chunks[pend_r * 64 + ln] = pend;
        }
        pend_r = -1;
    };
    auto gti = [&]() { return tid - g * NT; };
    auto vidx = [&](int j) { const int vi = j * NT + gti(); return vi < nvec ? vi : nvec - 1; };
    auto ld_reg = [&](const RowSrc<true, sizeof(LT)> &src, int j) { return src(j * NT + gti()); };
    const uint32_t slot_base = (uint32_t)(uintptr_t)(lvoid_t *)&slots[g * SL + wg * 64];
    auto ld_lds = [&](const LT *rw, int k) {
        if ((k == L - 1 && noslot) || idle) return;
        const u32x4 *src = reinterpret_cast<const u32x4 *>(rw) + vidx(R + k);
        uint32_t keep;
        asm volatile("s_mov_b32 %0, m0\n\ts_mov_b32 m0, %2\n\ts_nop 0\n\tglobal_load_lds_dwordx4 %1, off" LAC_Q1_DMA_POLICY "\n\ts_mov_b32 m0, %0"
                     : "=&s"(keep)
                     : "v"(src), "s"(slot_base + (uint32_t)(k * NT * 16))
                     : "memory");
    };
    auto epilogue = [&](int64_t er, bool eok) {
        if constexpr (DEC) {
            if (wg == 0 && er >= 0) {
                const int ngrp = (nvec + 63) / 64, ln = lane_fresh(), gofs = vofs / 64;
                const int g0 = ln * (int)G, ga = g0 > gofs ? g0 : gofs;
                const int gb = g0 + (int)G < gofs + ngrp ? g0 + (int)G : gofs + ngrp;
                uint64_t ct = 0;
                for (int gi = ga; gi < gb; gi++) ct += gtot[g * NWR * (R + L) + gi - gofs];
                pend = ct + (GROUP && !eok ? kGroupPoison : 0);
                pend_r = er;
                if (!DEFER) flush_chunks();
            }
        } else if (gti() == 0) {
            const uint64_t ps = sps[g];
            if (er < 0) return;
            uint64_t T = 0, Ls = 0;
#pragma unroll
            for (int i = 0; i < NWR; i++) { T += ssum[g * NWR + i][0]; Ls += ssum[g * NWR + i][1]; }
            if constexpr (GROUP) {
                RowStats *o = out + er;
                group_add(&o->tot, T + (eok ? 0 : kGroupPoison));
                group_add(&o->lo, Ls);
                group_add(&o->hi, Ls + ps);
                if (hh == 0) __hip_atomic_store(&o->minp, (uint64_t)1, __ATOMIC_RELAXED, __HIP_MEMORY_SCOPE_AGENT);
            } else {
                RowStats st;
                st.lo = Ls;
                st.hi = Ls + ps;
                st.tot = T;
                st.minp = 1;
                st.inv_tot = 1.0 / (double)T;
                st.pad = 0;
                out[er] = st;
            }
        }
    };
    u32x4 x[R];
    {
        const int64_t r0 = b0 + roff;
        const LT *rw = r0 < rows ? row_of(r0) : lg;
        const RowSrc<true, sizeof(LT)> src(rw, true, idle ? 0 : nvec);
#pragma unroll
        for (int k = 0; k < L; k++) ld_lds(rw, k);
#pragma unroll
        for (int j = 0; j < R; j++) x[j] = ld_reg(src, j);
    }
    for (int64_t rb = b0; rb < rows; rb += stride) {
        asm volatile("" : "+v"(tid));
        const int64_t r = rb + roff;
        const bool valid = !idle && r < rows;
        const int64_t rn = r + stride;
        const LT *nrow = rn < rows ? row_of(rn) : lg;
        __builtin_amdgcn_s_waitcnt(0);
        asm volatile("" ::: "memory");
        auto slot = [&](int k) {
            return (k == L - 1 && noslot) ? neg_inf16(sizeof(LT)) : slots[g * SL + k * NT + gti()];
        };
        float m;
        pok = true;
        if constexpr (IMAX) {
            s16x2 pm = {(short)-32768, (short)-32768};
            auto pmax = [&](const u32x4 &v) {
                pm = __builtin_elementwise_max(pm, as_s16x2(v.x));
                pm = __builtin_elementwise_max(pm, as_s16x2(v.y));
                pm = __builtin_elementwise_max(pm, as_s16x2(v.z));
                pm = __builtin_elementwise_max(pm, as_s16x2(v.w));
            };
#pragma unroll
            for (int j = 0; j < R; j++) pmax(x[j]);
#pragma unroll
            for (int k = 0; k < L; k++) pmax(slot(k));
            const int li = pm.x > pm.y ? (int)pm.x : (int)pm.y;
            const int wi = (int)wave_reduce((uint32_t)li, [](uint32_t a, uint32_t b) {
                return (uint32_t)((int)a > (int)b ? (int)a : (int)b);
            });
            if (lane == 0) smaxi[w] = wi;
            if (!DEC && gti() == 0) sps[g] = 0;
            __syncthreads();
            int bi = 0;
            bool all_ok = true;
#pragma unroll
            for (int gg = 0; gg < NRB; gg++) {
                int bm = smaxi[gg * NWR];
#pragma unroll
                for (int i = 1; i < NWR; i++) bm = smaxi[gg * NWR + i] > bm ? smaxi[gg * NWR + i] : bm;
                all_ok = all_ok && bm >= 0 && bm <= 0x7F80;
                bi = gg == g ? bm : bi;
            }
            bool my_ok = true;
            if constexpr (GROUP) {
                bi = (int)group_combine((uint32_t)bi, valid, [](uint32_t a, uint32_t b) {
                    return (int)a > (int)b ? a : b;
                });
                my_ok = !valid || (bi >= 0 && bi <= 0x7F80);
                all_ok = true;
#pragma unroll
                for (int gg = 0; gg < NRB; gg++)
                    all_ok = all_ok && (!sxact[gg] || ((int)sxv[gg] >= 0 && (int)sxv[gg] <= 0x7F80));
            }
            if (all_ok) {
                m = __uint_as_float((uint32_t)bi << 16);
            } else {
                float mx = -INFINITY;
#pragma unroll
                for (int j = 0; j < R; j++)
#pragma unroll
                    for (int e = 0; e < N; e++) mx = fmaxf(mx, logit_at<LT>(x[j], e));
#pragma unroll
                for (int k = 0; k < L; k++) {
                    const u32x4 v = slot(k);
#pragma unroll
                    for (int e = 0; e < N; e++) mx = fmaxf(mx, logit_at<LT>(v, e));
                }
                mx = wave_max_f32(mx);
                if (lane == 0) smax[w] = mx;
                __syncthreads();
                m = smax[g * NWR];
#pragma unroll
                for (int i = 1; i < NWR; i++) m = fmaxf(m, smax[g * NWR + i]);
                if constexpr (GROUP) {
                    const float mf = __uint_as_float(group_combine(
                        __float_as_uint(m), valid && !my_ok, [](uint32_t a, uint32_t b) { return f32_max_bits(a, b); }));
                    m = my_ok ? __uint_as_float((uint32_t)bi << 16) : mf;
                }
            }
        } else {
            float mx = -INFINITY;
#pragma unroll
            for (int j = 0; j < R; j++)
#pragma unroll
                for (int e = 0; e < N; e++) mx = fmaxf(mx, logit_at<LT>(x[j], e));
#pragma unroll
            for (int k = 0; k < L; k++) {
                const u32x4 v = slot(k);
#pragma unroll
                for (int e = 0; e < N; e++) mx = fmaxf(mx, logit_at<LT>(v, e));
            }
            mx = wave_max_f32(mx);
            if (lane == 0) smax[w] = mx;
            if (!DEC && gti() == 0) sps[g] = 0;
            __syncthreads();
            m = smax[g * NWR];
#pragma unroll
            for (int i = 1; i < NWR; i++) m = fmaxf(m, smax[g * NWR + i]);
            if constexpr (GROUP)
                m = __uint_as_float(group_combine(__float_as_uint(m), valid,
                                                  [](uint32_t a, uint32_t b) { return f32_max_bits(a, b); }));
        }
        if (DEC && valid && gti() == 0 && hh == 0) mrow[r] = m;
        if constexpr (DEC) flush_chunks();
        const bool fast = q1_fast_row(m);
// ... 655 lines not shown
        s[j] = v0 + 64 * j < nvec ? q : 0u;
    }
}

template <typename LT>
__device__ inline void q1_step_entries(const u32x4 &xv, float c, const uint32_t *tab, uint32_t loff,
                                       uint32_t (&loc)[LogitN<LT>::N]) {
    uint32_t ls = 0;
#pragma unroll
    for (int e = 0; e < LogitN<LT>::N; e++) {
        ls += q1_rep_at<kStepRep>(tab, q1_j(logit_at<LT>(xv, e), c), loff);
        loc[e] = ls;
    }
}

template <typename LT, int R, bool SMALL>
__global__ __launch_bounds__(kQ1StepMaxThreads) void k_q1_step_dec(const LT *__restrict__ lg, int64_t stream_stride,
                                                                   int64_t V, int prec, uint32_t xsh,
                                                                   DecState *states, const uint8_t *bits,
                                                                   uint64_t stride, const uint64_t *nbits,
                                                                   int32_t *sym_out,
                                                                   const int64_t *__restrict__ slen) {
    __shared__ StepShared sh;
    constexpr int N = LogitN<LT>::N;
    const int lane = (int)lane_id(), w = wave_in_block(), nw = (int)(blockDim.x >> 6);
    const int64_t b = blockIdx.x;
    DecState st = states[b];
    dec_state_uniform(st);
    if (st.err || live_steps(slen, b, st.nsym, 1) == 0) {
        if (threadIdx.x == 0) sym_out[b] = -1;
        return;
    }
    const int nvec = (int)(V / N);
    const uint8_t *mybits = bits + b * stride;
    const uint64_t mynbits = rfl_u64(nbits[b]);
    BitWin win{0, 0};
    if (w == 0) win = bit_window(mybits, mynbits, st.pos);
    if (threadIdx.x == 0) sh.found = 0;
    u32x4 x[R];
    uint32_t s[R];
    float c;
    q1_step_row<LT, R>(lg + b * stream_stride, nvec, xsh, sh, x, s, c);
    uint32_t ts = 0, sv[R];
#pragma unroll
    for (int j = 0; j < R; j++) {
        ts += s[j];
        sv[j] = s[j];
    }
    const uint64_t wt = wave_sum_u64((uint64_t)ts);
    const uint64_t gsum = wave_multi_sum32<R>(sv);
    if (lane < R) sh.jtot[w * kQ1StepMaxR + q_index<R>(lane)] = gsum;
    if (lane == 0) sh.wtot[w] = wt;
    __syncthreads();
    uint64_t T = 0, wb = 0;
    for (int i = 0; i < nw; i++) {
        const uint64_t t = sh.wtot[i];
        wb += i < w ? t : 0;
        T += t;
    }
    int err = 0;
    uint64_t wd = 0, vh = 0, thi = 0, tgt = 0;
    {
        T = rfl_u64(T);
        const int64_t l = st.l, h = st.h, xx = st.x;
        if (xx < l || xx > h) err = LAC_E_DECODE_RANGE;
        wd = (uint64_t)(h - l + 1);
        const uint64_t v = (uint64_t)(xx - l);
        if (!err && T > wd) err = LAC_E_TABLE;
        if (!err) {
            const uint64_t past = st.pos > mynbits ? st.pos - mynbits : 0;
            const int u = past < (uint64_t)prec ? (int)past : prec;
            vh = v + ((1ull << u) - 1);
            if (SMALL) {
                const double iw = recip(wd);
                tgt = div_small_u<false>(v, T, 0, wd, iw);
                thi = vh == v ? tgt : (vh < wd ? div_small_u<false>(vh, T, 0, wd, iw) : 0);
            } else {
                div_pair(v, vh < wd ? vh : 0, T, 0, wd, recip(wd), &tgt, &thi);
            }
        }
    }
    if (!err && wb <= tgt && tgt < wb + wt) {
        uint64_t base = wb;
        int js = -1;
#pragma unroll
        for (int j = 0; j < R; j++) {
            const uint64_t t = sh.jtot[w * kQ1StepMaxR + j];
            const bool in = js < 0 && tgt < base + t;
            js = in ? j : js;
            base += js < 0 ? t : 0;
        }
        js = __builtin_amdgcn_readfirstlane(js);
        u32x4 xv = x[0];
        uint32_t sj = s[0];
#pragma unroll
        for (int j = 1; j < R; j++)
            if (j == js) {
                xv = x[j];
                sj = s[j];
            }
        const uint64_t in = wave_incl_scan_u64((uint64_t)sj);
        const uint64_t exb = base + in - sj;
        const uint64_t mk = __ballot(exb + sj > tgt);
        if (js >= 0 && mk) {
            const int L = __ffsll((unsigned long long)mk) - 1;
            const uint32_t rel = (uint32_t)(tgt - exb);
            uint32_t loc[N];
            q1_step_entries<LT>(xv, c, sh.tab, (uint32_t)(lane & (kStepRep - 1)) * 4u, loc);
            uint32_t k = 0, lo = 0, hi = ~0u;
#pragma unroll
            for (int e = 0; e < N; e++) {
                const bool le = loc[e] <= rel;
                k += le ? 1u : 0u;
                lo = le ? loc[e] : lo;
                hi = (!le && loc[e] < hi) ? loc[e] : hi;
            }
            if (lane == L) {
                sh.res[0] = (uint64_t)(w * 64 * R + 64 * js + L) * N + k;
                sh.res[1] = exb + lo;
                sh.res[2] = exb + hi;
                sh.found = 1;
            }
        }
    }
    __syncthreads();
    if (w == 0) {
        int64_t sym = -1;
        if (!err && !sh.found) err = LAC_E_DECODE_RANGE;
        if (!err) {
            sym = (int64_t)rfl_u64(sh.res[0]);
            const uint64_t lo_c = rfl_u64(sh.res[1]), hi_c = rfl_u64(sh.res[2]);
            uint64_t a, bb;
            if (SMALL) {
                div_small_u2<false>(lo_c, hi_c, wd, T - 1, T, recip(T), &a, &bb);
            } else {
                div_pair(lo_c, hi_c, wd, T - 1, T, recip(T), &a, &bb);
            }
            const bool det = vh < wd && thi < hi_c;
            if (st.det && det) st.ndet++;
            else st.det = 0;
            err = LAC_Q1D_NB ? decode_advance_nb(st, a, bb, win, mynbits, prec)
                             : decode_advance<true>(st, a, bb, win, mynbits, prec);
        }
        if (err) {
            st.err = err;
            st.err_step = st.nsym;
        }
        if (lane == 0) {
            states[b] = st;
            sym_out[b] = err ? -1 : (int32_t)sym;
        }
    }
}

template <typename LT, int R>
__global__ __launch_bounds__(kQ1StepMaxThreads) void k_q1_step_enc(const LT *__restrict__ lg, int64_t stream_stride,
                                                                   const int32_t *__restrict__ sym, int64_t V,
                                                                   int prec, uint32_t xsh,
                                                                   EncState *states, uint64_t *planeA,
                                                                   uint64_t *planeC, uint64_t cap_words,
                                                                   uint64_t *trace,
                                                                   const int64_t *__restrict__ slen) {
    __shared__ StepShared sh;
    constexpr int N = LogitN<LT>::N;
    const int lane = (int)lane_id(), w = wave_in_block(), nw = (int)(blockDim.x >> 6);
    const int64_t b = blockIdx.x;
    EncState st = states[b];
    if (live_steps(slen, b, st.nsym, 1) == 0) return;
    if (st.err || st.nflush >= 0) {
        if (threadIdx.x == 0 && !st.err && st.nflush >= 0) {
            st.err = LAC_E_STATE;
            st.err_step = st.nsym;
            states[b] = st;
        }
        return;
    }
    const int nvec = (int)(V / N);
    const int32_t s0 = __builtin_amdgcn_readfirstlane(sym[b]);
    const int sc = (uint32_t)s0 < (uint32_t)V ? s0 : 0;
    const int vs = sc / N, es = sc % N, ws = vs / (64 * R), js = (vs / 64) % R, ls = vs % 64;
    u32x4 x[R];
    uint32_t s[R];
    float c;
    q1_step_row<LT, R>(lg + b * stream_stride, nvec, xsh, sh, x, s, c);
    uint32_t ts = 0;
#pragma unroll
    for (int j = 0; j < R; j++) ts += s[j];
    const uint64_t wt = wave_sum_u64((uint64_t)ts);
    if (lane == 0) sh.wtot[w] = wt;
    if (w == ws) {
        uint32_t cl = 0, sj = s[0];
        u32x4 xv = x[0];
#pragma unroll
        for (int j = 0; j < R; j++) {
            cl += j < js ? s[j] : 0u;
            if (j == js) {
                xv = x[j];
                sj = s[j];
            }
        }
        cl += lane < ls ? sj : 0u;
        const uint64_t pre = wave_sum_u64((uint64_t)cl);
        uint32_t loc[N];
        q1_step_entries<LT>(xv, c, sh.tab, (uint32_t)(lane & (kStepRep - 1)) * 4u, loc);
        uint32_t below = 0, upto = loc[0];
#pragma unroll
        for (int e = 1; e < N; e++) {
            below = e == es ? loc[e - 1] : below;
            upto = e == es ? loc[e] : upto;
        }
        if (lane == ls) {
            sh.res[0] = pre + below;
            sh.res[1] = (uint64_t)(upto - below);
        }
    }
    __syncthreads();
    if (w != 0) return;
    uint64_t T = 0, lo = sh.res[0];
    for (int i = 0; i < nw; i++) {
        const uint64_t t = sh.wtot[i];
        lo += i < ws ? t : 0;
        T += t;
    }
    T = rfl_u64(T);
    lo = rfl_u64(lo);
    const uint64_t hi = lo + rfl_u64(sh.res[1]);
    uint64_t *pa = planeA + (uint64_t)b * cap_words, *pc = planeC + (uint64_t)b * cap_words;
    int64_t l = (int64_t)rfl_u64((uint64_t)st.l), h = (int64_t)rfl_u64((uint64_t)st.h);
    st.L = rfl_u64(st.L);
    st.wa = rfl_u64(st.wa);
    st.wc = rfl_u64(st.wc);
    st.nsym = (int64_t)rfl_u64((uint64_t)st.nsym);
    int64_t err_step0 = st.err_step;
    const uint64_t fthr = T < (1ull << 62) ? T : (1ull << 62);
    const double inv = 1.0 / (double)T;
    coder_step<uint32_t, true>(st, l, h, lo, hi, T, 1, (int64_t)s0, (const uint32_t *)nullptr, V, prec, pa, pc,
                               cap_words, trace ? trace + 2 * b : nullptr, lane, LAC_MAP_CEIL, inv, false, kNoFrac,
                               kNoFrac, fthr);
    asm volatile("" : "+v"(err_step0));
    st.err_step = err_step0;
    if (lane == 0) store_state(st, l, h, pa, pc, cap_words, &states[b]);
}


}

static int q1_shift(lac_ctx *c, uint32_t *xsh) {
    int cl = 0;
    while (((int64_t)1 << cl) < c->V) cl++;
    int k = c->prec - 1 - cl;
    if (k > LAC_Q1_KMAX) k = LAC_Q1_KMAX;
    if (k < 1) return fail(LAC_E_PREC, "prec %d leaves no q1 precision for vocab %lld", c->prec, (long long)c->V);
    *xsh = (uint32_t)(LAC_Q1_KMAX - k);
    return LAC_OK;
}

static int logits_check(lac_ctx *c, const void *lg, int type, int64_t step_stride, int64_t stream_stride,
                        int64_t steps) {
    if (type != LAC_LOGITS_BF16 && type != LAC_LOGITS_F32) return fail(LAC_E_ARG, "logit type %d", type);
    if (steps < 0 || step_stride < 0 || stream_stride < 0) return fail(LAC_E_ARG, "negative size/stride");
    const int n = type == LAC_LOGITS_BF16 ? 8 : 4;
    if (steps > 0 && ((uintptr_t)lg % 16 || c->V % n || step_stride % n || stream_stride % n))
        return fail(LAC_E_ARG, "logits rows must be 16-byte aligned with vocab and strides multiples of %d", n);
    if (c->mapping != LAC_MAP_CEIL || c->term != LAC_TERM_FLUSH)
        return fail(LAC_E_STATE, "the logits path codes with the CDFPredictor mapping and flush termination");
    return LAC_OK;
}

struct Q1Args {
    const void *lg;
    int64_t ss, bs;
    const int32_t *sym;
    int64_t rows, t0;
    uint32_t xsh;
};

#define LAC_Q1_ARGS                                                                                            \
    (const LT *)a.lg, a.ss, a.bs, a.sym, c->B, a.rows, c->V, a.t0, a.xsh, p.groups_per_chunk, c->stats, c->q1chunks, \
        c->q1m

template <typename LT, bool DEC, int I = 0>
static int q1_tiled_launch(lac_ctx *c, const Q1Args &a, hipStream_t st, const Q1Plan &p,
                           const uint64_t *gate = nullptr) {
    if constexpr (I == kQ1TiledForms) {
        return fail(LAC_E_ARG, "q1 shape %d has no tiled form", p.shape);
    } else {
        if (p.tiled != I) return q1_tiled_launch<LT, DEC, I + 1>(c, a, st, p, gate);
        constexpr int RW = kQ1Tiled[I][1], R = kQ1Tiled[I][2], NWB = kQ1Tiled[I][5];
        constexpr bool MULTI = kQ1Tiled[I][3] != 0, PF = kQ1Tiled[I][4] != 0;
        static_assert(NWB == 16 || NWB == kQ1Waves, "kQ1Tiled's block sizes");
        static int per_cu = 0;
        if (!per_cu) {
            int n = 0;
            if (hipOccupancyMaxActiveBlocksPerMultiprocessor(&n, k_q1_stats<LT, RW, R, DEC, MULTI, PF, NWB>, 64 * NWB,
                                                             0) != hipSuccess ||
                n < 1)
                n = 1;
            per_cu = n;
        }
        constexpr int NR = NWB / RW;
        const int64_t need = (a.rows + NR - 1) / NR, cap = (int64_t)c->cus * per_cu;
        const unsigned grid = (unsigned)(need < cap ? need : cap);
        ProfScope ps(c, gate ? -1 : KID_Q1_STATS, st);
        k_q1_stats<LT, RW, R, DEC, MULTI, PF, NWB><<<grid, 64 * NWB, 0, st>>>(LAC_Q1_ARGS, gate);
        CHECK_LAUNCH();
        return LAC_OK;
    }
}

static int q1_group_setup(lac_ctx *c, const Q1Args &a, hipStream_t st, const Q1Group &g, bool dec, unsigned *grid,
                          int *rpx_out) {
    if (!c->pxch) HIPCHK(hipMalloc(&c->pxch, sizeof(uint64_t) * (8 * (int64_t)c->cus + 1)));
    const int64_t spx = (int64_t)(c->cus / 8) * g.nrb, rcap = spx / g.k, rneed = (a.rows + 7) / 8;
    const int64_t rpx = rneed < rcap ? rneed : rcap;
    *grid = (unsigned)(8 * ((rpx * g.k + g.nrb - 1) / g.nrb));
    *rpx_out = (int)rpx;
    HIPCHK(hipMemsetAsync(c->pxch, 0, sizeof(uint64_t) * (2 * g.nrb * (int64_t)*grid + 1), st));
    if (dec) HIPCHK(hipMemsetAsync(c->q1chunks, 0, sizeof(uint64_t) * 64 * a.rows, st));
    else HIPCHK(hipMemsetAsync(c->stats, 0, sizeof(RowStats) * a.rows, st));
    return LAC_OK;
}

template <typename LT, bool DEC>
static int q1_group_repair(lac_ctx *c, const Q1Args &a, hipStream_t st, const Q1Plan &p, unsigned grid) {
    c->xch_abort = 2 * p.group.nrb * (int64_t)grid;
    return q1_tiled_launch<LT, DEC>(c, a, st, p, c->pxch + c->xch_abort);
}

template <typename LT, bool DEC, bool GROUP>
static int q1_slot_launch(lac_ctx *c, const Q1Args &a, hipStream_t st, const Q1Plan &p) {
    const bool wide = p.family == Q1_WIDE || p.family == Q1_WIDE_GROUP;
    const int64_t nrb = wide ? 1 : 1024 / p.nt, need = (a.rows + nrb - 1) / nrb;
    unsigned grid = (unsigned)(need < c->cus ? need : c->cus);
    int rpx = 0, rc;
    if (GROUP && (rc = q1_group_setup(c, a, st, p.group, DEC, &grid, &rpx))) return rc;
#define LAC_Q1_SLOT_ARGS LAC_Q1_ARGS, GROUP ? c->pxch : nullptr, GROUP ? p.group.split : 0, GROUP ? p.group.k : 1, rpx
#define LAC_Q1_RL(REP, LASTN, NT)                       \
    if (p.rep == REP && p.lastn == LASTN && p.nt == NT) \
    k_q1_stats_rl<LT, DEC, REP, LASTN, NT, GROUP><<<grid, 1024, 0, st>>>(LAC_Q1_SLOT_ARGS)
    {
        ProfScope ps(c, KID_Q1_STATS, st);
        if (wide && (GROUP || !p.wide_slots)) {
            k_q1_stats_wide<LT, kQ1WideR, DEC, GROUP><<<grid, 512, 0, st>>>(LAC_Q1_SLOT_ARGS);
        } else if (wide) {
            if constexpr (!GROUP)
                k_q1_stats_wide<LT, kQ1WideR, DEC, false, kQ1WideL><<<grid, 512, 0, st>>>(LAC_Q1_SLOT_ARGS);
        } else LAC_Q1_RL(16, kRLLastTrim, 1024);
        else LAC_Q1_RL(kRLRep, 1024, 1024);
        else LAC_Q1_RL(16, 320, 512);
        else LAC_Q1_RL(kRLRep, 512, 512);
        else LAC_Q1_RL(kRLRep, 256, 256);
        else if constexpr (!DEC) {
            LAC_Q1_RL(16, 192, 256);
        } else if constexpr (!GROUP) {
            LAC_Q1_RL(kRLRep, 192, 256);
        }
        CHECK_LAUNCH();
    }
#undef LAC_Q1_RL
#undef LAC_Q1_SLOT_ARGS
    if constexpr (GROUP) return q1_group_repair<LT, DEC>(c, a, st, p, grid);
    return LAC_OK;
}

template <typename LT, bool DEC>
static int q1_launch(lac_ctx *c, const Q1Args &a, hipStream_t st, const Q1Plan &p) {
    if (p.family == Q1_TILED) return q1_tiled_launch<LT, DEC>(c, a, st, p);
    if (p.family == Q1_RL || p.family == Q1_WIDE) return q1_slot_launch<LT, DEC, false>(c, a, st, p);
    return q1_slot_launch<LT, DEC, true>(c, a, st, p);
}

template <typename LT, bool DEC>
static int q1_stats(lac_ctx *c, const Q1Args &a, hipStream_t st) {
    Q1Plan p;
    if (q1_plan(c->cus, c->V, (int)sizeof(LT), DEC, c->q1_shape, &p))
        return fail(LAC_E_ARG, "q1 shape %d does not hold a row of %lld vectors", c->q1_shape,
                    (long long)(c->V / LogitN<LT>::N));
    return q1_launch<LT, DEC>(c, a, st, p);
}

template <typename LT>
static int q1_encode(lac_ctx *c, const Q1Args &a0, int64_t steps, uint64_t *trace, hipStream_t st, int flags) {
    int rc;
    if ((flags & kReset) && (rc = enc_reset_launch(c, st))) return rc;
    for (int64_t t0 = 0; t0 < steps; t0 += c->chunk_steps) {
        const int64_t n = (steps - t0) < c->chunk_steps ? (steps - t0) : c->chunk_steps;
        Q1Args a = a0;
        a.rows = n * c->B;
        a.t0 = t0;
        if ((rc = q1_stats<LT, false>(c, a, st))) return rc;
        if ((rc = enc_stats_launch(c, a.sym, t0, n, trace, st))) return rc;
    }
    if ((flags & kFinish) && (rc = enc_finish_launch(c, LAC_TERM_FLUSH, st))) return rc;
    return LAC_OK;
}

template <typename LT>
static int q1_decode(lac_ctx *c, const Q1Args &a0, int64_t steps, int32_t *out, hipStream_t st) {
    int rc0 = ensure_chunk_buffers(c);
    if (rc0) return rc0;
    const unsigned blocks = (unsigned)((c->B + kWavesPerBlock - 1) / kWavesPerBlock);
    const int64_t nvec = c->V / LogitN<LT>::N;
    for (int64_t t0 = 0; t0 < steps; t0 += c->chunk_steps) {
        const int64_t n = (steps - t0) < c->chunk_steps ? (steps - t0) : c->chunk_steps;
        Q1Args a = a0;
        a.rows = n * c->B;
        a.t0 = t0;
        int rc = q1_stats<LT, true>(c, a, st);
        if (rc) return rc;
        ProfScope ps(c, KID_Q1_DECODE, st);
        const int64_t G = q1_groups_per_chunk(nvec);
#define LAC_Q1_DEC(GC)                                                                                            \
    k_q1_decode<LT, GC><<<blocks, 64 * kWavesPerBlock, 0, st>>>((const LT *)a.lg, a.ss, a.bs, t0, n, c->V, c->prec, \
                                                               a.xsh, G, c->q1chunks, c->q1m, c->dec, c->dbits,    \
                                                               c->dstride, c->dnbits, out, c->B, stream_lengths(c))
        if (c->prec > 50)
            k_q1_decode<LT, 0, false><<<blocks, 64 * kWavesPerBlock, 0, st>>>(
                (const LT *)a.lg, a.ss, a.bs, t0, n, c->V, c->prec, a.xsh, G, c->q1chunks, c->q1m, c->dec, c->dbits,
                c->dstride, c->dnbits, out, c->B, stream_lengths(c));
        else switch (G) {
        case 1: LAC_Q1_DEC(1); break;
        case 2: LAC_Q1_DEC(2); break;
        case 3: LAC_Q1_DEC(3); break;
        case 4: LAC_Q1_DEC(4); break;
        case 5: LAC_Q1_DEC(5); break;
        case 6: LAC_Q1_DEC(6); break;
        case 7: LAC_Q1_DEC(7); break;
        case 8: LAC_Q1_DEC(8); break;
        default: LAC_Q1_DEC(0); break;
        }
#undef LAC_Q1_DEC
        CHECK_LAUNCH();
    }
    return LAC_OK;
}

template <typename LT>
static int q1_step_decode(lac_ctx *c, const Q1Args &a, const Q1StepPlan &p, int32_t *out, hipStream_t st) {
    ProfScope ps(c, KID_Q1_DECODE, st);
#define LAC_Q1_STEP_DEC(R, SMALL)                                                                               \
    k_q1_step_dec<LT, R, SMALL><<<(unsigned)c->B, p.threads, 0, st>>>((const LT *)a.lg, a.bs, c->V, c->prec, a.xsh, \
                                                                      c->dec, c->dbits, c->dstride, c->dnbits, out, \
                                                                      stream_lengths(c))
    if (c->prec > 50) {
        if (p.R == 4) LAC_Q1_STEP_DEC(4, false);
        else if (p.R == 8) LAC_Q1_STEP_DEC(8, false);
        else LAC_Q1_STEP_DEC(16, false);
    } else {
        if (p.R == 4) LAC_Q1_STEP_DEC(4, true);
        else if (p.R == 8) LAC_Q1_STEP_DEC(8, true);
        else LAC_Q1_STEP_DEC(16, true);
    }
#undef LAC_Q1_STEP_DEC
    CHECK_LAUNCH();
    return LAC_OK;
}

template <typename LT>
static int q1_step_encode(lac_ctx *c, const Q1Args &a, const Q1StepPlan &p, uint64_t *trace, hipStream_t st) {
    ProfScope ps(c, KID_ENCODE, st);
#define LAC_Q1_STEP_ENC(R)                                                                                        \
    k_q1_step_enc<LT, R><<<(unsigned)c->B, p.threads, 0, st>>>((const LT *)a.lg, a.bs, a.sym, c->V, c->prec, a.xsh, \
                                                               c->enc, c->planeA, c->planeC, c->cap_words, trace,   \
                                                               stream_lengths(c))
    if (p.R == 4) LAC_Q1_STEP_ENC(4);
    else if (p.R == 8) LAC_Q1_STEP_ENC(8);
    else LAC_Q1_STEP_ENC(16);
#undef LAC_Q1_STEP_ENC
    CHECK_LAUNCH();
    return LAC_OK;
}

static int q1_step_choose(lac_ctx *c, int logit_type, Q1StepPlan *p) {
    *p = q1_step_plan(c->cus, c->V, logit_type == LAC_LOGITS_BF16 ? 2 : 4, c->B, c->q1_step);
    if (p->rc)
        return fail(p->rc, "the fused logits step holds rows of <= %d vectors for <= %lld streams", kQ1StepMaxVec,
                    (long long)(kQ1StepMaxStreams < c->cus ? kQ1StepMaxStreams : c->cus));
    return LAC_OK;
}

extern "C" {

int lac_decode_logits_step(lac_ctx *c, const void *logits_dev, int logit_type, int64_t stream_stride,
                           int32_t *sym_out_dev, void *stream) {
    if (!c || !logits_dev || !sym_out_dev) return fail(LAC_E_ARG, "NULL argument");
    if (c->mode != 1) return fail(LAC_E_STATE, "call lac_decode_open first");
    int rc = logits_check(c, logits_dev, logit_type, 0, stream_stride, 1);
    uint32_t xsh = 0;
    Q1StepPlan p;
    if (rc || (rc = q1_shift(c, &xsh)) || (rc = q1_step_choose(c, logit_type, &p))) return rc;
    HIPCHK(hipSetDevice(c->device));
    const Q1Args a{logits_dev, 0, stream_stride, nullptr, 0, 0, xsh};
    if (!p.fused)
        return logit_type == LAC_LOGITS_BF16 ? q1_decode<uint16_t>(c, a, 1, sym_out_dev, S(stream))
                                             : q1_decode<float>(c, a, 1, sym_out_dev, S(stream));
    return logit_type == LAC_LOGITS_BF16 ? q1_step_decode<uint16_t>(c, a, p, sym_out_dev, S(stream))
                                         : q1_step_decode<float>(c, a, p, sym_out_dev, S(stream));
}

int lac_encode_logits_step(lac_ctx *c, const void *logits_dev, int logit_type, int64_t stream_stride,
                           const int32_t *sym_dev, uint64_t *trace_dev, void *stream) {
    if (!c || !logits_dev || !sym_dev) return fail(LAC_E_ARG, "NULL argument");
    int rc = logits_check(c, logits_dev, logit_type, 0, stream_stride, 1);
    uint32_t xsh = 0;
    Q1StepPlan p;
    if (rc || (rc = q1_shift(c, &xsh)) || (rc = q1_step_choose(c, logit_type, &p))) return rc;
    HIPCHK(hipSetDevice(c->device));
    c->mode = 0;
    const Q1Args a{logits_dev, 0, stream_stride, sym_dev, 0, 0, xsh};
    if (!p.fused)
        rc = logit_type == LAC_LOGITS_BF16 ? q1_encode<uint16_t>(c, a, 1, trace_dev, S(stream), 0)
                                           : q1_encode<float>(c, a, 1, trace_dev, S(stream), 0);
    else
        rc = logit_type == LAC_LOGITS_BF16 ? q1_step_encode<uint16_t>(c, a, p, trace_dev, S(stream))
                                           : q1_step_encode<float>(c, a, p, trace_dev, S(stream));
    if (rc == LAC_OK) enc_mark_open(c);
    return rc;
}

static int logits_encode(lac_ctx *c, const void *logits_dev, int logit_type, int64_t step_stride,
                         int64_t stream_stride, const int32_t *sym_dev, int64_t steps, uint64_t *trace_dev,
                         void *stream, int flags) {
    if (!c || (steps > 0 && (!logits_dev || !sym_dev))) return fail(LAC_E_ARG, "NULL argument");
    int rc = logits_check(c, logits_dev, logit_type, step_stride, stream_stride, steps);
    uint32_t xsh = 0;
    if (rc || (rc = q1_shift(c, &xsh))) return rc;
    if (steps == 0 && !flags) return LAC_OK;
    HIPCHK(hipSetDevice(c->device));
    c->mode = 0;
    const Q1Args a{logits_dev, step_stride, stream_stride, sym_dev, 0, 0, xsh};
    return logit_type == LAC_LOGITS_BF16 ? q1_encode<uint16_t>(c, a, steps, trace_dev, S(stream), flags)
                                         : q1_encode<float>(c, a, steps, trace_dev, S(stream), flags);
}

int lac_encode_logits_job(lac_ctx *c, const void *logits_dev, int logit_type, int64_t step_stride,
                          int64_t stream_stride, const int32_t *sym_dev, int64_t steps, uint64_t *trace_dev,
                          void *stream) {
    const int rc = logits_encode(c, logits_dev, logit_type, step_stride, stream_stride, sym_dev, steps, trace_dev,
                                 stream, kReset | kFinish);
    if (rc == LAC_OK) enc_mark_finished(c);
    return rc;
}

int lac_encode_logits(lac_ctx *c, const void *logits_dev, int logit_type, int64_t step_stride,
                      int64_t stream_stride, const int32_t *sym_dev, int64_t steps, uint64_t *trace_dev,
                      void *stream) {
    const int rc = logits_encode(c, logits_dev, logit_type, step_stride, stream_stride, sym_dev, steps, trace_dev,
                                 stream, 0);
    if (rc == LAC_OK && steps > 0) enc_mark_open(c);
    return rc;
}

int lac_decode_logits_steps(lac_ctx *c, const void *logits_dev, int logit_type, int64_t step_stride,
                            int64_t stream_stride, int64_t steps, int32_t *sym_out_dev, void *stream) {
    if (!c || (steps > 0 && (!logits_dev || !sym_out_dev))) return fail(LAC_E_ARG, "NULL argument");
    if (c->mode != 1) return fail(LAC_E_STATE, "call lac_decode_open first");
    int rc = logits_check(c, logits_dev, logit_type, step_stride, stream_stride, steps);
    uint32_t xsh = 0;
    if (rc || (rc = q1_shift(c, &xsh))) return rc;
    if (steps == 0) return LAC_OK;
    HIPCHK(hipSetDevice(c->device));
    const Q1Args a{logits_dev, step_stride, stream_stride, nullptr, 0, 0, xsh};
    return logit_type == LAC_LOGITS_BF16 ? q1_decode<uint16_t>(c, a, steps, sym_out_dev, S(stream))
                                         : q1_decode<float>(c, a, steps, sym_out_dev, S(stream));
}

int lac_quantize_logits(lac_ctx *c, const void *logits_dev, int logit_type, int64_t step_stride,
                        int64_t stream_stride, int64_t steps, uint32_t *pmf_out_dev, void *stream) {
    if (!c || (steps > 0 && (!logits_dev || !pmf_out_dev))) return fail(LAC_E_ARG, "NULL argument");
    if (logit_type != LAC_LOGITS_BF16 && logit_type != LAC_LOGITS_F32) return fail(LAC_E_ARG, "logit type");
    const int n = logit_type == LAC_LOGITS_BF16 ? 8 : 4;
    if (steps < 0 || step_stride < 0 || stream_stride < 0) return fail(LAC_E_ARG, "negative size/stride");
    if (steps > 0 && ((uintptr_t)logits_dev % 16 || c->V % n || step_stride % n || stream_stride % n))
        return fail(LAC_E_ARG, "logits rows must be 16-byte aligned with vocab and strides multiples of %d", n);
    uint32_t xsh = 0;
    int rc = q1_shift(c, &xsh);
    if (rc) return rc;
    if (steps == 0) return LAC_OK;
    HIPCHK(hipSetDevice(c->device));
    hipStream_t st = S(stream);
    const int64_t rows = steps * c->B;
    const unsigned blocks = (unsigned)((rows + kWavesPerBlock - 1) / kWavesPerBlock);
    if (logit_type == LAC_LOGITS_BF16)
        k_quantize_logits<uint16_t><<<blocks, 64 * kWavesPerBlock, 0, st>>>(
            (const uint16_t *)logits_dev, step_stride, stream_stride, c->B, rows, c->V, xsh, pmf_out_dev);
    else
        k_quantize_logits<float><<<blocks, 64 * kWavesPerBlock, 0, st>>>(
            (const float *)logits_dev, step_stride, stream_stride, c->B, rows, c->V, xsh, pmf_out_dev);
    CHECK_LAUNCH();
    return LAC_OK;
}

int lac_q1_group_aborted(lac_ctx *c, int64_t *aborted, void *stream) {
    if (!c || !aborted) return fail(LAC_E_ARG, "NULL argument");
    *aborted = 0;
    if (c->xch_abort < 0 || !c->pxch) return LAC_OK;
    HIPCHK(hipSetDevice(c->device));
    uint64_t v = 0;
    HIPCHK(hipMemcpyAsync(&v, c->pxch + c->xch_abort, sizeof v, hipMemcpyDeviceToHost, S(stream)));
    HIPCHK(hipStreamSynchronize(S(stream)));
    *aborted = v ? 1 : 0;
    return LAC_OK;
}

}
```

lac_amd/csrc/lac_select.h:

```cpp
#pragma once
#include <stdint.h>

#include "lac.h"

#if defined(__HIPCC__) || defined(__CUDACC__)
#define LAC_SEL_HD __host__ __device__
#else
#define LAC_SEL_HD
#endif

constexpr int kRLRep = 8;
constexpr int kRLRegVec = 8, kRLSlots = 8;
constexpr int kRLLastTrim = 704;
constexpr int kRLTrimMaxVec = 15 * 1024 + kRLLastTrim;
constexpr int kQ1WideR = 40;
constexpr int kQ1WideThreads = 512;
constexpr int kQ1WideMaxVec = kQ1WideThreads * kQ1WideR;
constexpr int kQ1WideL = 11;
constexpr int kQ1WideSlotMaxVec = kQ1WideThreads * (kQ1WideR + kQ1WideL);
constexpr int kQ1MaxSeg = 16;

constexpr int kQ1Shapes[][3] = {{1, 4, 0}, {2, 8, 0}, {4, 8, 0}, {8, 8, 0}, {8, 16, 0}, {8, 8, 1}, {8, 4, 1}};
constexpr int kQ1Tiled[][6] = {{1, 1, 4, 0, 0, 8}, {2, 2, 8, 0, 0, 8},  {3, 4, 8, 0, 0, 8},     {4, 8, 8, 0, 0, 8},
                               {6, 8, 8, 0, 1, 8}, {8, 8, 8, 1, 0, 8}, {10, 16, 16, 1, 0, 16}, {14, 16, 8, 1, 1, 16}};
constexpr int kQ1TiledForms = sizeof(kQ1Tiled) / sizeof(kQ1Tiled[0]);
inline bool q1_shape_live(int sh) {
    return sh >= 0 && sh <= 23 && sh != 5 && sh != 7 && sh != 9 && sh != 11 && sh != 12 && sh != 13 && sh != 16;
}

inline int64_t q1_groups_per_chunk(int64_t nvec) {
    const int64_t groups = (nvec + 63) / 64;
    return groups <= 64 ? 1 : (groups + 63) / 64;
}

struct Q1Group {
    int k = 0, split = 0, nrb = 1;
    bool rep16 = false;
    double score = 0;
};
inline int q1_rl_lastn(int nrb, bool rep16) {
    const int nt = 1024 / nrb;
    return !rep16 ? nt : nrb == 1 ? kRLLastTrim : nrb == 2 ? 320 : 192;
}
inline int64_t q1_slot_cap(int nrb, bool rep16) {
    return (int64_t)(kRLRegVec + kRLSlots - 1) * (1024 / nrb) + q1_rl_lastn(nrb, rep16);
}
inline bool q1_split(int64_t nvec, int64_t kmin, int64_t kmax, int64_t lim, Q1Group *g) {
    const int64_t ngrp = (nvec + 63) / 64;
    for (int64_t k = kmin < 2 ? 2 : kmin; k <= kQ1MaxSeg && k <= kmax; k++) {
        const int64_t sp = 64 * ((ngrp + k - 1) / k), last = nvec - (k - 1) * sp;
        if (last > 0 && sp <= lim && last <= lim) {
            g->k = (int)k;
            g->split = (int)sp;
            return true;
        }
    }
    return false;
}
inline bool q1_group_form(int cus, int64_t nvec, int nrb, bool rep16, Q1Group *g) {
    const int64_t spx = (int64_t)(cus / 8) * nrb;
    if (!q1_split(nvec, 2, spx, q1_slot_cap(nrb, rep16), g)) return false;
    g->nrb = nrb;
    g->rep16 = rep16;
    g->score = (double)nvec / (g->k * (16384.0 / nrb)) * (double)((spx / g->k) * g->k) / (double)spx;
    return true;
}
inline bool q1_group(int cus, int64_t nvec, bool dec, bool bf16, int nrb, Q1Group *best) {
    bool any = false;
    for (int n = 1; n <= 4; n *= 2) {
        if (nrb && n != nrb) continue;
        for (int rep16 = 1; rep16 >= 0; rep16--) {
            if (dec && n == 4 && rep16) continue;
            Q1Group g;
            if (!q1_group_form(cus, nvec, n, rep16 != 0, &g)) continue;
            if (!rep16) g.score *= dec ? 0.95 : bf16 ? 0.75 : 1.0;
            if (!any || g.score > best->score + 1e-9) *best = g;
            any = true;
        }
    }
    return any;
}
inline bool q1_wide_group(int cus, int64_t nvec, Q1Group *g) {
    g->nrb = 1;
    return q1_split(nvec, (nvec + kQ1WideMaxVec - 1) / kQ1WideMaxVec, cus / 8, kQ1WideMaxVec, g);
}

enum { Q1_TILED, Q1_RL, Q1_WIDE, Q1_RL_GROUP, Q1_WIDE_GROUP };
struct Q1Plan {
    int shape = 0;
    int family = Q1_TILED;
    int tiled = -1;
    int rep = 0, lastn = 0, nt = 0;
    bool wide_slots = false;
    Q1Group group;
    int repair = 0;
    int64_t groups_per_chunk = 1;
};

inline int q1_tiled_form(int sh) {
    for (int i = 0; i < kQ1TiledForms; i++)
        if (kQ1Tiled[i][0] == sh) return i;
    return -1;
}

inline int q1_plan(int cus, int64_t V, int type_bytes, bool dec, int forced_shape, Q1Plan *out) {
    const bool bf16 = type_bytes == 2;
    const int64_t nvec = V / (bf16 ? 8 : 4);
    auto holds = [&](int i) { return nvec <= 64 * kQ1Shapes[i - 1][0] * kQ1Shapes[i - 1][1]; };
    Q1Plan p;
    p.groups_per_chunk = q1_groups_per_chunk(nvec);
    int sh = forced_shape;
    bool grouped = false;
    if (sh == 0) {
        static const int order[] = {1, 2, 3, 6};
        if (nvec > 4096 && nvec <= 8192) sh = 18;
        else if (!dec && !bf16 && nvec > 2048 && nvec <= 4096) sh = 17;
        for (int i : order) {
            if (sh) break;
            if (holds(i)) sh = i;
        }
        if (sh == 0 && nvec <= 16384) sh = 15;
        if (sh == 0 && nvec <= kQ1WideSlotMaxVec) sh = 22;
        if (sh == 0 && q1_group(cus, nvec, dec, bf16, 0, &p.group)) {
            Q1Group wg;
            grouped = true;
            sh = p.group.nrb == 1 ? 19 : p.group.nrb == 2 ? 20 : 21;
            if (p.group.nrb > 1 && q1_wide_group(cus, nvec, &wg) && nvec >= 0.75 * wg.k * kQ1WideMaxVec) {
                p.group = wg;
                sh = 23;
            }
        }
        if (sh == 0) sh = dec ? 10 : (!bf16 ? 14 : 8);
    } else if (sh >= 19 && sh <= 21) {
        grouped = q1_group(cus, nvec, dec, bf16, sh == 19 ? 1 : sh == 20 ? 2 : 4, &p.group);
    } else if (sh == 23) {
        grouped = q1_wide_group(cus, nvec, &p.group);
    }
    p.shape = sh;
    const int nrb = sh == 15 || sh == 19 ? 1 : sh == 18 || sh == 20 ? 2 : 4;
    if (sh == 15 || (sh >= 17 && sh <= 21)) {
        if (sh >= 19 ? !grouped : nvec > q1_slot_cap(nrb, false)) return LAC_E_ARG;
        const bool trim = sh >= 19 ? p.group.rep16 : nvec <= q1_slot_cap(nrb, true);
        p.family = sh >= 19 ? Q1_RL_GROUP : Q1_RL;
        p.rep = trim && !(sh == 17 && dec) ? 16 : kRLRep;
        p.lastn = q1_rl_lastn(nrb, trim);
        p.nt = 1024 / nrb;
    } else if (sh == 22 || sh == 23) {
        if (sh == 23 ? !grouped : nvec > kQ1WideSlotMaxVec) return LAC_E_ARG;
        p.family = sh == 23 ? Q1_WIDE_GROUP : Q1_WIDE;
        p.wide_slots = sh == 22 && nvec > kQ1WideMaxVec;
    } else {
        if (sh != 8 && sh != 10 && sh != 14 && (sh > 7 || !q1_shape_live(sh) || !holds(sh))) return LAC_E_ARG;
        p.tiled = q1_tiled_form(sh);
    }
    if (grouped) p.tiled = q1_tiled_form(p.repair = dec ? 10 : (!bf16 ? 14 : 8));
    *out = p;
    return LAC_OK;
}

constexpr int kQ1StepMaxThreads = 1024;
constexpr int kQ1StepMaxR = 16;
constexpr int kQ1StepMaxVec = kQ1StepMaxThreads * kQ1StepMaxR;
#ifndef LAC_Q1_STEP_MAX_STREAMS
#define LAC_Q1_STEP_MAX_STREAMS 256
#endif
constexpr int64_t kQ1StepMaxStreams = LAC_Q1_STEP_MAX_STREAMS;
enum { Q1_STEP_AUTO = 0, Q1_STEP_FUSED = 1, Q1_STEP_SPLIT = 2 };
struct Q1StepPlan {
    bool fused = false;
    int rc = LAC_OK;
    int threads = 0, R = 0;
};
inline Q1StepPlan q1_step_plan(int cus, int64_t V, int type_bytes, int64_t streams, int mode) {
    Q1StepPlan p;
    const int64_t nvec = V / (type_bytes == 2 ? 8 : 4);
    const int64_t cap = kQ1StepMaxStreams < cus ? kQ1StepMaxStreams : cus;
    const bool fits = nvec >= 1 && nvec <= kQ1StepMaxVec && streams >= 1 && streams <= cap;
    if (mode == Q1_STEP_SPLIT) return p;
    if (!fits) {
        if (mode == Q1_STEP_FUSED) p.rc = LAC_E_ARG;
        return p;
    }
    p.fused = true;
    p.R = nvec <= 4 * kQ1StepMaxThreads ? 4 : nvec <= 8 * kQ1StepMaxThreads ? 8 : 16;
    const int64_t thr = ((nvec + p.R - 1) / p.R + 63) / 64 * 64;
    p.threads = (int)(thr < kQ1StepMaxThreads ? thr : kQ1StepMaxThreads);
    return p;
}

#ifndef LAC_LEAN
#define LAC_LEAN 1
#endif
#ifndef LAC_LEAN_HELP
#define LAC_LEAN_HELP 1
#endif
#ifndef LAC_LEAN_CW32
#define LAC_LEAN_CW32 1
#endif
template <typename E> constexpr int LeanCW = sizeof(E) == 8 ? 2 : LAC_LEAN_CW32;
LAC_SEL_HD inline void lean_chunk_layout_n(int64_t V, int vec, int cw, int64_t *CI, int64_t *nch) {
    const int64_t nvec = V / vec, nit = (nvec + 63) / 64, per = 64 * cw;
    const int64_t ci = nit ? (nit + per - 1) / per : 1;
    *CI = ci;
    *nch = (nit + ci - 1) / ci;
}
template <typename E, int VEC>
LAC_SEL_HD inline void lean_chunk_layout(int64_t V, int64_t *CI, int64_t *nch) {
    lean_chunk_layout_n(V, VEC, LeanCW<E>, CI, nch);
}
#ifndef LAC_LEAN_HELPERS
#define LAC_LEAN_HELPERS 16
#endif
constexpr int kLeanHelpers = LAC_LEAN_HELPERS;
#ifndef LAC_LEAN_MAX_STREAMS
#define LAC_LEAN_MAX_STREAMS 44
#endif
constexpr int64_t kLeanMaxStreams = LAC_LEAN_MAX_STREAMS;
constexpr int kLeanHelpMaxStreams = 16;
#ifndef LAC_LEAN_BYTES
#define LAC_LEAN_BYTES (512ll << 20)
#endif
constexpr int64_t kLeanBytes = LAC_LEAN_BYTES;
#ifndef LAC_LEAN_ROUNDS
#define LAC_LEAN_ROUNDS 3
#endif
constexpr int kLeanRounds = LAC_LEAN_ROUNDS;

struct DecodeKnobs {
    int dpath;
    int64_t wave_decode_min_streams, block_decode_min_streams, block_window_lo, block_window_hi;
    int block_waves, fine_decode, dec_stop;
    bool has_len;
    int64_t chunk_steps;
};
enum { DEC_PER_STEP, DEC_WAVE, DEC_BLOCK, DEC_STATS };
struct DecodePlan {
    int rc = LAC_OK;
    int path = DEC_PER_STEP;
    int vec = 1;
    int fine_nr = 0;
    int block_nw = 0;
    int G = 0, step_waves = 0;
    bool lean = false, help = false;
    int64_t CI = 0, cs = 0;
    bool static_rows = false;
};

inline DecodePlan decode_plan(const DecodeKnobs &k, int64_t B, int64_t V, int pmf_bits, int prec, bool aligned16,
                              int64_t step_stride, int64_t stream_stride, int64_t steps) {
    DecodePlan p;
    const int vw = pmf_bits == 32 ? 4 : 2, esize = pmf_bits / 8;
    const bool vec = aligned16 && V % vw == 0 && step_stride % vw == 0 && stream_stride % vw == 0;
    p.vec = vec ? vw : 1;
    const int64_t nit = (V / p.vec + 63) / 64;
    const bool wave = k.dpath == LAC_PATH_FUSED || (k.dpath == LAC_PATH_AUTO && B >= k.wave_decode_min_streams);
    const bool blockable = vec && nit <= 512;
    if (k.dec_stop) {
        p.path = DEC_STATS;
    } else if (blockable && (k.dpath == LAC_PATH_BLOCK ||
                             (k.dpath == LAC_PATH_AUTO && !wave &&
                              ((B >= k.block_window_lo && B <= k.block_window_hi) || B >= k.block_decode_min_streams)))) {
        p.path = DEC_BLOCK;
        const int nw = k.block_waves ? k.block_waves : (B >= 1024 ? 4 : B >= 512 ? 8 : 16);
        p.block_nw = nw == 4 || nw == 8 ? nw : 16;
    } else if (k.dpath == LAC_PATH_STATS || k.dpath == LAC_PATH_BLOCK || (k.dpath == LAC_PATH_AUTO && !wave)) {
        p.path = DEC_STATS;
    } else if (wave) {
        p.path = DEC_WAVE;
        if (vec && k.fine_decode && nit <= 512) p.fine_nr = nit <= 128 ? 2 : nit <= 256 ? 4 : 8;
    } else {
        const bool few = B <= 256;
        p.G = !vec || few ? 8 : pmf_bits == 32 ? 2 : 4;
        p.step_waves = few ? 16 : 4;
        if ((V + 64 * p.vec * p.G - 1) / (64 * p.vec * p.G) * 8 > 64 * 1024) p.rc = LAC_E_ARG;
    }
    if (p.path != DEC_STATS) return p;
    p.static_rows = step_stride == 0;
    int64_t lnch;
    lean_chunk_layout_n(V, p.vec, esize == 8 ? 2 : LAC_LEAN_CW32, &p.CI, &lnch);
    p.lean = LAC_LEAN && vec && prec <= 50 && p.CI <= 4 && V / p.vec > 0 && B <= kLeanMaxStreams && !k.has_len;
    p.cs = p.static_rows ? steps : k.chunk_steps;
    if (p.lean && !p.static_rows) {
        const int64_t fit = kLeanBytes / (V * esize) / B;
        const int64_t ls = fit < 64 ? 64 : fit / 64 * 64;
        p.cs = ls < p.cs ? ls : p.cs;
    }
    p.help = p.lean && !p.static_rows && LAC_LEAN_HELP && B <= kLeanHelpMaxStreams;
    return p;
}
```

Before: 53.97 million symbols/s.

## Fuse logit quantization stats and range encoding into one persistent q1 kernel

Moves the per-block range-coder loop into a shared device header and adds a fused mode to the q1 stats kernel. Each persistent block owns a set of streams, buffers per-symbol interval rows in a ring, and encodes them in batches inside the same kernel, so the separate stats buffer and encode kernel launch are no longer needed. A plan function enables the fusion only for certain tiled shapes when the stream count covers the resident block capacity. A query API reports the fused plan. The cost is more register and LDS pressure plus serial per-wave encoding interleaved with the quantization work.

```diff
diff --git a/include/lac.h b/include/lac.h
--- a/include/lac.h
+++ b/include/lac.h
@@ -167,6 +167,8 @@
 
 int lac_q1_group_aborted(lac_ctx *ctx, int64_t *aborted, void *stream);
 
+int lac_q1_fuse_info(lac_ctx *ctx, int logit_type, int64_t *out5);
+
 int lac_quantize_logits(lac_ctx *ctx, const void *logits_dev, int logit_type, int64_t step_stride,
                         int64_t stream_stride, int64_t steps, uint32_t *pmf_out_dev, void *stream);
 
diff --git a/lac_amd/_lib.py b/lac_amd/_lib.py
--- a/lac_amd/_lib.py
+++ b/lac_amd/_lib.py
@@ -78,6 +78,7 @@
     ("lac_hc_encode_flush", _i, [_i, _i64, _i64, _vp, _vp]),
     ("lac_hc_decode_emit", _i, [_i, _vp, _i64, _i64, _i]),
     ("lac_q1_group_aborted", _i, [_vp, _vp, _vp]),
+    ("lac_q1_fuse_info", _i, [_vp, _i, _vp]),
     ("lac_profile_enable", _i, [_vp, _i]),
     ("lac_profile_read", _i, [_vp, _vp, _vp, _i]),
     ("lac_q1_k", _i, [_i, _i64]),
diff --git a/lac_amd/batch.py b/lac_amd/batch.py
--- a/lac_amd/batch.py
+++ b/lac_amd/batch.py
@@ -534,6 +534,12 @@
     def set_q1_shape(self, shape: int):
         check(self.lib.lac_set_option(self.ctx, _lib.LAC_OPT_Q1_SHAPE, int(shape)))
 
+    def q1_fuse_info(self, bf16=True):
+        o = (C.c_int64 * 5)()
+        check(self.lib.lac_q1_fuse_info(self.ctx, _lib.LAC_LOGITS_BF16 if bf16 else _lib.LAC_LOGITS_F32, o))
+        return {"fused": bool(o[0]), "grid": int(o[1]), "max_own": int(o[2]), "batch": int(o[3]),
+                "resident": int(o[4])}
+
     def q1_k(self):
         return int(self.lib.lac_q1_k(self.prec, self.vocab))
 
diff --git a/lac_amd/csrc/lac_enc_dev.h b/lac_amd/csrc/lac_enc_dev.h
--- /dev/null
+++ b/lac_amd/csrc/lac_enc_dev.h
@@ -0,0 +1,217 @@
+#pragma once
+#include "lac_dev.h"
+
+#include <type_traits>
+
+namespace {
+
+struct SP {
+    uint64_t lo, hi, tot, flo, fhi, fthr;
+    int n, prec;
+    uint64_t cap_words, *pa, *pc;
+    int lane;
+};
+template <bool CEIL, bool T32, bool FT>
+__device__ inline int straight_steps(const SP &sp, EncState &st, int64_t &l, int64_t &h, bool &ok) {
+    auto store = [&](uint64_t idx, uint64_t wa, uint64_t wc) {
+        if (sp.lane == 0) { sp.pa[idx] = wa; sp.pc[idx] = wc; }
+    };
+    typedef typename std::conditional<T32, uint32_t, uint64_t>::type CT;
+    struct Row {
+        CT lo, hi, T;
+        uint64_t fl, fh, ft;
+    };
+    auto rd = [&](int j) {
+        Row r;
+        if constexpr (T32) {
+            r.lo = (uint32_t)__builtin_amdgcn_readlane((int)(uint32_t)sp.lo, j);
+            r.hi = (uint32_t)__builtin_amdgcn_readlane((int)(uint32_t)sp.hi, j);
+            r.T = (uint32_t)__builtin_amdgcn_readlane((int)(uint32_t)sp.tot, j);
+        } else {
+            r.lo = readlane_u64(sp.lo, j);
+            r.hi = readlane_u64(sp.hi, j);
+            r.T = readlane_u64(sp.tot, j);
+        }
+        r.fl = readlane_u64(sp.flo, j);
+        r.fh = readlane_u64(sp.fhi, j);
+        r.ft = FT ? readlane_u64(sp.fthr, j) : 0;
+        return r;
+    };
+    const int n = sp.n, prec = sp.prec;
+    const int64_t nsym0 = st.nsym;
+    Row nx = rd(0);
+    int i = 0;
+    int kk = 0;
+    uint64_t e = 0;
+    bool fudged = false;
+    while (i < n) {
+        for (; i < n; i++) {
+            const Row r = LAC_ENC_PIPE ? nx : rd(i);
+            if constexpr (LAC_ENC_PIPE) nx = rd(i + 1 < n ? i + 1 : i);
+            const uint64_t w = (uint64_t)(h - l + 1);
+            if constexpr (FT) {
+                if (!nonneg_uni((int64_t)(w - r.ft))) {
+                    fudged = true;
+                    break;
+                }
+            }
+            uint64_t a, bb;
+            if constexpr (T32) {
+                a = frac_mul_div32<CEIL>(r.fl, r.lo, w, r.T);
+                bb = frac_mul_div32<CEIL>(r.fh, r.hi, w, r.T);
+            } else {
+                a = frac_mul_div<true>(r.fl, r.lo, w, r.T, CEIL);
+                bb = frac_mul_div<true>(r.fh, r.hi, w, r.T, CEIL);
+            }
+            h = l + (int64_t)bb - 1;
+            l = l + (int64_t)a;
+            const uint64_t d = (uint64_t)(h - l);
+            const int sh = bitlen64(d);
+            kk = prec - sh;
+            e = kk > 0 ? (uint64_t)l >> sh : 0;
+            l = (int64_t)(((uint64_t)l - (e << sh)) << kk);
+            h = l + (int64_t)((d + 1) << kk) - 1;
+            const int off0 = (int)(st.L & 63);
+            const int avail = off0 ? 64 - off0 : 0;
+            if (__builtin_expect(kk > avail, 0)) break;
+            st.wc |= (e >> kk) << ((64 - off0) & 63);
+            st.wa |= (e & ((1ull << kk) - 1)) << ((64 - off0 - kk) & 63);
+            st.L += (uint64_t)kk;
+        }
+        if (i >= n) break;
+        if constexpr (FT) {
+            if (fudged) break;
+        }
+        if (!plane_append(st.L, st.wa, st.wc, kk, e, sp.cap_words, store)) {
+            st.err = LAC_E_CAPACITY;
+            ok = false;
+            break;
+        }
+        i++;
+    }
+    st.nsym = nsym0 + i;
+    return i;
+}
+
+template <typename E, int MAP, typename Clock>
+__device__ inline void encode_block(const RowStats &my, int32_t mys, int n, int lane, int64_t tb, int64_t b,
+                                    int64_t B, const E *pmf, int64_t step_stride, int64_t stream_stride, int64_t V,
+                                    int prec, EncState &st, int64_t &l, int64_t &h, uint64_t *pa, uint64_t *pc,
+                                    uint64_t cap_words, uint64_t *trace, bool allow_fudge, bool &ok, Clock *clk) {
+    const bool frac_ok = lane < n && !(my.tot >> 62);
+    const uint64_t flo = frac_ok ? row_frac(my.lo, my.tot) : kNoFrac;
+    const uint64_t fhi = frac_ok ? row_frac(my.hi, my.tot) : kNoFrac;
+    int i0 = 0;
+#if LAC_ENC_STRAIGHT
+    if constexpr (sizeof(E) == 8) {
+        const uint64_t half = 1ull << (prec - 1);
+        const bool lfast = lane >= n || (frac_ok && my.tot != 0 && my.hi > my.lo && (uint32_t)mys < (uint32_t)V &&
+                                         (MAP != LAC_MAP_FLOOR || ((my.tot - 1) >> (prec - 1)) < my.hi - my.lo));
+        const uint64_t d0 = (uint64_t)(h - l);
+        if (!trace && prec <= 61 && __ballot(!lfast) == 0 && nonneg_uni((int64_t)(d0 - half)) &&
+            !(d0 >> prec)) {
+            constexpr bool CEIL = MAP != LAC_MAP_FLOOR;
+            const bool t32 = __ballot(lane < n && (my.tot >> 32)) == 0;
+            const bool ft = CEIL && __ballot(lane < n && my.tot > half) != 0;
+            uint64_t ftl = 0;
+            if (ft) {
+                ftl = lane < n && my.minp ? div_floor((u128)my.tot + (my.minp - 1), my.minp) : 0;
+                ftl = ftl < (1ull << 62) ? ftl : (1ull << 62);
+            }
+            SP sp{my.lo, my.hi, my.tot, flo, fhi, ftl, n, prec, cap_words, pa, pc, lane};
+            if (t32)
+                i0 = ft ? straight_steps<CEIL, true, true>(sp, st, l, h, ok)
+                        : straight_steps<CEIL, true, false>(sp, st, l, h, ok);
+            else
+                i0 = ft ? straight_steps<CEIL, false, true>(sp, st, l, h, ok)
+                        : straight_steps<CEIL, false, false>(sp, st, l, h, ok);
+            if (!ok || i0 >= n) return;
+        }
+    }
+    if (i0 == 0) {
+        const uint64_t half = 1ull << (prec - 1);
+        const bool lfast = lane >= n || (frac_ok && my.tot != 0 && my.tot <= half && !(my.tot >> 32) &&
+                                         my.hi > my.lo && (uint32_t)mys < (uint32_t)V);
+        const uint64_t d0 = (uint64_t)(h - l);
+        if (!trace && prec <= 61 && __ballot(!lfast) == 0 && nonneg_uni((int64_t)(d0 - half)) &&
+            !(d0 >> prec)) {
+            constexpr bool CEIL = MAP != LAC_MAP_FLOOR;
+            const int64_t nsym0 = st.nsym;
+            auto store = [&](uint64_t idx, uint64_t wa, uint64_t wc) {
+                if (lane == 0) { pa[idx] = wa; pc[idx] = wc; }
+            };
+            auto rd = [&](int j, uint32_t &lo, uint32_t &hi, uint32_t &T, uint64_t &fl, uint64_t &fh) {
+                lo = (uint32_t)__builtin_amdgcn_readlane((int)(uint32_t)my.lo, j);
+                hi = (uint32_t)__builtin_amdgcn_readlane((int)(uint32_t)my.hi, j);
+                T = (uint32_t)__builtin_amdgcn_readlane((int)(uint32_t)my.tot, j);
+                fl = readlane_u64(flo, j);
+                fh = readlane_u64(fhi, j);
+            };
+            uint32_t nlo, nhi, nT;
+            uint64_t nfl, nfh;
+            if constexpr (LAC_ENC_PIPE) rd(0, nlo, nhi, nT, nfl, nfh);
+            int i = 0;
+            int kk = 0;
+            uint64_t e = 0;
+            while (i < n) {
+                for (; i < n; i++) {
+                    uint32_t lo, hi, T;
+                    uint64_t fl, fh;
+                    if constexpr (LAC_ENC_PIPE) {
+                        lo = nlo, hi = nhi, T = nT, fl = nfl, fh = nfh;
+                        rd(i + 1 < n ? i + 1 : i, nlo, nhi, nT, nfl, nfh);
+                    } else {
+                        rd(i, lo, hi, T, fl, fh);
+                    }
+                    const uint64_t w = (uint64_t)(h - l + 1);
+                    const uint64_t a = frac_mul_div32<CEIL>(fl, lo, w, T), bb = frac_mul_div32<CEIL>(fh, hi, w, T);
+                    h = l + (int64_t)bb - 1;
+                    l = l + (int64_t)a;
+                    const uint64_t d = (uint64_t)(h - l);
+                    const int sh = bitlen64(d);
+                    kk = prec - sh;
+                    e = kk > 0 ? (uint64_t)l >> sh : 0;
+                    l = (int64_t)(((uint64_t)l - (e << sh)) << kk);
+                    h = l + (int64_t)((d + 1) << kk) - 1;
+                    const int off0 = (int)(st.L & 63);
+                    const int avail = off0 ? 64 - off0 : 0;
+                    if (__builtin_expect(kk > avail, 0)) break;
+                    st.wc |= (e >> kk) << ((64 - off0) & 63);
+                    st.wa |= (e & ((1ull << kk) - 1)) << ((64 - off0 - kk) & 63);
+                    st.L += (uint64_t)kk;
+                }
+                if (i >= n) break;
+                if (!plane_append(st.L, st.wa, st.wc, kk, e, cap_words, store)) {
+                    st.err = LAC_E_CAPACITY;
+                    ok = false;
+                    break;
+                }
+                i++;
+            }
+            st.nsym = nsym0 + i;
+            return;
+        }
+    }
+#endif
+    uint64_t fthr = lane < n && my.minp ? div_floor((u128)my.tot + (my.minp - 1), my.minp) : 0;
+    fthr = fthr < (1ull << 62) ? fthr : (1ull << 62);
+    if (clk) clk->mark(4);
+    for (int i = i0; i < n; i++) {
+        const uint64_t lo = readlane_u64(my.lo, i), hi = readlane_u64(my.hi, i);
+        const uint64_t T = readlane_u64(my.tot, i), minp = readlane_u64(my.minp, i);
+        const uint64_t invb = readlane_u64(__builtin_bit_cast(uint64_t, my.inv_tot), i);
+        const uint64_t fl = readlane_u64(flo, i), fh = readlane_u64(fhi, i), ft = readlane_u64(fthr, i);
+        const int64_t s = __builtin_amdgcn_readlane(mys, i);
+        const int64_t t = tb + i;
+        const E *row = pmf + t * step_stride + b * stream_stride;
+        if (clk) clk->mark(0);
+        if (!coder_step<E, true>(st, l, h, lo, hi, T, minp, s, row, V, prec, pa, pc, cap_words,
+                                 trace ? trace + 2 * (t * B + b) : nullptr, lane, MAP,
+                                 __builtin_bit_cast(double, invb), allow_fudge, fl, fh, ft, clk)) {
+            ok = false;
+            break;
+        }
+    }
+}
+
+}
diff --git a/lac_amd/csrc/lac_encode.hip b/lac_amd/csrc/lac_encode.hip
--- a/lac_amd/csrc/lac_encode.hip
+++ b/lac_amd/csrc/lac_encode.hip
@@ -1,4 +1,5 @@
 #include "lac_host.h"
+#include "lac_enc_dev.h"
 #include "lac_drain.h"
 #include "lac_wire.h"
 
@@ -40,94 +41,6 @@
     }
 }
 
-struct SP {
-    uint64_t lo, hi, tot, flo, fhi, fthr;
-    int n, prec;
-    uint64_t cap_words, *pa, *pc;
-    int lane;
-};
-template <bool CEIL, bool T32, bool FT>
-__device__ inline int straight_steps(const SP &sp, EncState &st, int64_t &l, int64_t &h, bool &ok) {
-    auto store = [&](uint64_t idx, uint64_t wa, uint64_t wc) {
-        if (sp.lane == 0) { sp.pa[idx] = wa; sp.pc[idx] = wc; }
-    };
-    typedef typename std::conditional<T32, uint32_t, uint64_t>::type CT;
-    struct Row {
-        CT lo, hi, T;
-        uint64_t fl, fh, ft;
-    };
-    auto rd = [&](int j) {
-        Row r;
-        if constexpr (T32) {
-            r.lo = (uint32_t)__builtin_amdgcn_readlane((int)(uint32_t)sp.lo, j);
-            r.hi = (uint32_t)__builtin_amdgcn_readlane((int)(uint32_t)sp.hi, j);
-            r.T = (uint32_t)__builtin_amdgcn_readlane((int)(uint32_t)sp.tot, j);
-        } else {
-            r.lo = readlane_u64(sp.lo, j);
-            r.hi = readlane_u64(sp.hi, j);
-            r.T = readlane_u64(sp.tot, j);
-        }
-        r.fl = readlane_u64(sp.flo, j);
-        r.fh = readlane_u64(sp.fhi, j);
-        r.ft = FT ? readlane_u64(sp.fthr, j) : 0;
-        return r;
-    };
-    const int n = sp.n, prec = sp.prec;
-    const int64_t nsym0 = st.nsym;
-    Row nx = rd(0);
-    int i = 0;
-    int kk = 0;
-    uint64_t e = 0;
-    bool fudged = false;
-    while (i < n) {
-        for (; i < n; i++) {
-            const Row r = LAC_ENC_PIPE ? nx : rd(i);
-            if constexpr (LAC_ENC_PIPE) nx = rd(i + 1 < n ? i + 1 : i);
-            const uint64_t w = (uint64_t)(h - l + 1);
-            if constexpr (FT) {
-                if (!nonneg_uni((int64_t)(w - r.ft))) {
-                    fudged = true;
-                    break;
-                }
-            }
-            uint64_t a, bb;
-            if constexpr (T32) {
-                a = frac_mul_div32<CEIL>(r.fl, r.lo, w, r.T);
-                bb = frac_mul_div32<CEIL>(r.fh, r.hi, w, r.T);
-            } else {
-                a = frac_mul_div<true>(r.fl, r.lo, w, r.T, CEIL);
-                bb = frac_mul_div<true>(r.fh, r.hi, w, r.T, CEIL);
-            }
-            h = l + (int64_t)bb - 1;
-            l = l + (int64_t)a;
-            const uint64_t d = (uint64_t)(h - l);
-            const int sh = bitlen64(d);
-            kk = prec - sh;
-            e = kk > 0 ? (uint64_t)l >> sh : 0;
-            l = (int64_t)(((uint64_t)l - (e << sh)) << kk);
-            h = l + (int64_t)((d + 1) << kk) - 1;
-            const int off0 = (int)(st.L & 63);
-            const int avail = off0 ? 64 - off0 : 0;
-            if (__builtin_expect(kk > avail, 0)) break;
-            st.wc |= (e >> kk) << ((64 - off0) & 63);
-            st.wa |= (e & ((1ull << kk) - 1)) << ((64 - off0 - kk) & 63);
-            st.L += (uint64_t)kk;
-        }
-        if (i >= n) break;
-        if constexpr (FT) {
-            if (fudged) break;
-        }
-        if (!plane_append(st.L, st.wa, st.wc, kk, e, sp.cap_words, store)) {
-            st.err = LAC_E_CAPACITY;
-            ok = false;
-            break;
-        }
-        i++;
-    }
-    st.nsym = nsym0 + i;
-    return i;
-}
-
 template <typename E, int MAP>
 __global__ __launch_bounds__(256) void k_encode(const RowStats *__restrict__ stats, const int32_t *__restrict__ sym,
                                                 int64_t B, int64_t t0, int64_t nsteps, const E *pmf,
@@ -168,120 +81,8 @@
             my = stats[(g0 + lane) * B + b];
             mys = sym[(t0 + g0 + lane) * B + b];
         }
-        const bool frac_ok = lane < n && !(my.tot >> 62);
-        const uint64_t flo = frac_ok ? row_frac(my.lo, my.tot) : kNoFrac;
-        const uint64_t fhi = frac_ok ? row_frac(my.hi, my.tot) : kNoFrac;
-        int i0 = 0;
-#if LAC_ENC_STRAIGHT
-        if constexpr (sizeof(E) == 8) {
-            const uint64_t half = 1ull << (prec - 1);
-            const bool lfast = lane >= n || (frac_ok && my.tot != 0 && my.hi > my.lo && (uint32_t)mys < (uint32_t)V &&
-                                             (MAP != LAC_MAP_FLOOR || ((my.tot - 1) >> (prec - 1)) < my.hi - my.lo));
-            const uint64_t d0 = (uint64_t)(h - l);
-            if (!trace && prec <= 61 && __ballot(!lfast) == 0 && nonneg_uni((int64_t)(d0 - half)) &&
-                !(d0 >> prec)) {
-                constexpr bool CEIL = MAP != LAC_MAP_FLOOR;
-                const bool t32 = __ballot(lane < n && (my.tot >> 32)) == 0;
-                const bool ft = CEIL && __ballot(lane < n && my.tot > half) != 0;
-                uint64_t ftl = 0;
-                if (ft) {
-                    ftl = lane < n && my.minp ? div_floor((u128)my.tot + (my.minp - 1), my.minp) : 0;
-                    ftl = ftl < (1ull << 62) ? ftl : (1ull << 62);
-                }
-                SP sp{my.lo, my.hi, my.tot, flo, fhi, ftl, n, prec, cap_words, pa, pc, lane};
-                if (t32)
-                    i0 = ft ? straight_steps<CEIL, true, true>(sp, st, l, h, ok)
-                            : straight_steps<CEIL, true, false>(sp, st, l, h, ok);
-                else
-                    i0 = ft ? straight_steps<CEIL, false, true>(sp, st, l, h, ok)
-                            : straight_steps<CEIL, false, false>(sp, st, l, h, ok);
-                if (!ok || i0 >= n) continue;
-            }
-        }
-        if (i0 == 0) {
-            const uint64_t half = 1ull << (prec - 1);
-            const bool lfast = lane >= n || (frac_ok && my.tot != 0 && my.tot <= half && !(my.tot >> 32) &&
-                                             my.hi > my.lo && (uint32_t)mys < (uint32_t)V);
-            const uint64_t d0 = (uint64_t)(h - l);
-            if (!trace && prec <= 61 && __ballot(!lfast) == 0 && nonneg_uni((int64_t)(d0 - half)) &&
-                !(d0 >> prec)) {
-                constexpr bool CEIL = MAP != LAC_MAP_FLOOR;
-                const int64_t nsym0 = st.nsym;
-                auto store = [&](uint64_t idx, uint64_t wa, uint64_t wc) {
-                    if (lane == 0) { pa[idx] = wa; pc[idx] = wc; }
-                };
-                auto rd = [&](int j, uint32_t &lo, uint32_t &hi, uint32_t &T, uint64_t &fl, uint64_t &fh) {
-                    lo = (uint32_t)__builtin_amdgcn_readlane((int)(uint32_t)my.lo, j);
-                    hi = (uint32_t)__builtin_amdgcn_readlane((int)(uint32_t)my.hi, j);
-                    T = (uint32_t)__builtin_amdgcn_readlane((int)(uint32_t)my.tot, j);
-                    fl = readlane_u64(flo, j);
-                    fh = readlane_u64(fhi, j);
-                };
-                uint32_t nlo, nhi, nT;
-                uint64_t nfl, nfh;
-                if constexpr (LAC_ENC_PIPE) rd(0, nlo, nhi, nT, nfl, nfh);
-                int i = 0;
-                int kk = 0;
-                uint64_t e = 0;
-                while (i < n) {
-                    for (; i < n; i++) {
-                        uint32_t lo, hi, T;
-                        uint64_t fl, fh;
-                        if constexpr (LAC_ENC_PIPE) {
-                            lo = nlo, hi = nhi, T = nT, fl = nfl, fh = nfh;
-                            rd(i + 1 < n ? i + 1 : i, nlo, nhi, nT, nfl, nfh);
-                        } else {
-                            rd(i, lo, hi, T, fl, fh);
-                        }
-                        const uint64_t w = (uint64_t)(h - l + 1);
-                        const uint64_t a = frac_mul_div32<CEIL>(fl, lo, w, T), bb = frac_mul_div32<CEIL>(fh, hi, w, T);
-                        h = l + (int64_t)bb - 1;
-                        l = l + (int64_t)a;
-                        const uint64_t d = (uint64_t)(h - l);
-                        const int sh = bitlen64(d);
-                        kk = prec - sh;
-                        e = kk > 0 ? (uint64_t)l >> sh : 0;
-                        l = (int64_t)(((uint64_t)l - (e << sh)) << kk);
-                        h = l + (int64_t)((d + 1) << kk) - 1;
-                        const int off0 = (int)(st.L & 63);
-                        const int avail = off0 ? 64 - off0 : 0;
-                        if (__builtin_expect(kk > avail, 0)) break;
-                        st.wc |= (e >> kk) << ((64 - off0) & 63);
-                        st.wa |= (e & ((1ull << kk) - 1)) << ((64 - off0 - kk) & 63);
-                        st.L += (uint64_t)kk;
-                    }
-                    if (i >= n) break;
-                    if (!plane_append(st.L, st.wa, st.wc, kk, e, cap_words, store)) {
-                        st.err = LAC_E_CAPACITY;
-                        ok = false;
-                        break;
-                    }
-                    i++;
-                }
-                st.nsym = nsym0 + i;
-                continue;
-            }
-        }
-#endif
-        uint64_t fthr = lane < n && my.minp ? div_floor((u128)my.tot + (my.minp - 1), my.minp) : 0;
-        fthr = fthr < (1ull << 62) ? fthr : (1ull << 62);
-        if (clk) clk->mark(4);
-        for (int i = i0; i < n; i++) {
-            const uint64_t lo = readlane_u64(my.lo, i), hi = readlane_u64(my.hi, i);
-            const uint64_t T = readlane_u64(my.tot, i), minp = readlane_u64(my.minp, i);
-            const uint64_t invb = readlane_u64(__builtin_bit_cast(uint64_t, my.inv_tot), i);
-            const uint64_t fl = readlane_u64(flo, i), fh = readlane_u64(fhi, i), ft = readlane_u64(fthr, i);
-            const int64_t s = __builtin_amdgcn_readlane(mys, i);
-            const int64_t t = t0 + g0 + i;
-            const E *row = pmf + t * step_stride + b * stream_stride;
-            if (clk) clk->mark(0);
-            if (!coder_step<E, true>(st, l, h, lo, hi, T, minp, s, row, V, prec, pa, pc, cap_words,
-                                     trace ? trace + 2 * (t * B + b) : nullptr, lane, MAP,
-                                     __builtin_bit_cast(double, invb), allow_fudge, fl, fh, ft, clk)) {
-                ok = false;
-                break;
-            }
-        }
+        encode_block<E, MAP>(my, mys, n, lane, t0 + g0, b, B, pmf, step_stride, stream_stride, V, prec, st, l, h, pa,
+                             pc, cap_words, trace, allow_fudge, ok, clk);
     }
     if (lane == 0) store_state(st, l, h, pa, pc, cap_words, &states[b]);
 #if LAC_ENC_PHASES
diff --git a/lac_amd/csrc/lac_logits.hip b/lac_amd/csrc/lac_logits.hip
--- a/lac_amd/csrc/lac_logits.hip
+++ b/lac_amd/csrc/lac_logits.hip
@@ -1,5 +1,6 @@
 #include "lac_host.h"
 #include "lac_dec_dev.h"
+#include "lac_enc_dev.h"
 
 namespace {
 
@@ -249,23 +250,46 @@
 
 constexpr int kQ1Waves = 8;
 
+struct Q1Fuse {
+    EncState *enc;
+    uint64_t *planeA, *planeC, *nbits;
+    uint64_t cap_words;
+    const int64_t *slen;
+    int64_t nsteps;
+    int prec, flags;
+};
+struct Q1NoFuse {};
+struct Q1FuseRow {
+    uint64_t lo, hi, tot;
+    int32_t sym, pad;
+};
+template <bool FUSE> struct Q1FuseLds {};
+template <> struct Q1FuseLds<true> {
+    Q1FuseRow ring[kQ1FuseMaxOwn][kQ1FuseBatch];
+    EncState st[kQ1FuseMaxOwn];
+    int64_t live[kQ1FuseMaxOwn];
+    int dead[kQ1FuseMaxOwn];
+};
+
 template <int R, typename Src>
 __device__ inline void q1_load_tile(u32x4 (&x)[R], const Src &src, int base, int gt, int NT) {
 #pragma unroll
     for (int j = 0; j < R; j++) x[j] = src(base + gt + NT * j);
 }
 
-template <typename LT, int RW, int R, bool DEC, bool MULTI, bool PF, int NWB>
+template <typename LT, int RW, int R, bool DEC, bool MULTI, bool PF, int NWB, bool FUSE = false>
 __global__ __launch_bounds__(64 * NWB, LAC_Q1_MINW) void k_q1_stats(const LT *__restrict__ lg, int64_t step_stride,
                                                               int64_t stream_stride, const int32_t *__restrict__ sym,
                                                               int64_t B, int64_t rows, int64_t V, int64_t t0,
                                                               uint32_t xsh, int64_t G, RowStats *__restrict__ out,
                                                               uint64_t *__restrict__ chunks,
-                                                              float *__restrict__ mrow, const uint64_t *gate) {
+                                                              float *__restrict__ mrow, const uint64_t *gate,
+                                                              typename std::conditional<FUSE, Q1Fuse, Q1NoFuse>::type fa) {
     if (gate && __hip_atomic_load(gate, __ATOMIC_RELAXED, __HIP_MEMORY_SCOPE_AGENT) == 0) return;
     constexpr int N = LogitN<LT>::N, NT = 64 * RW, NR = NWB / RW;
     constexpr bool IMAX = LAC_Q1_IMAX && sizeof(LT) == 2 && NR == 1 && !MULTI;
     constexpr bool BUF = R <= 8 && !MULTI;
+    static_assert(!FUSE || (NR == 1 && !MULTI && !DEC && BUF), "the fused encode: one row per block, encode");
     typedef RowSrc<BUF, sizeof(LT)> Src;
     static_assert(R * N <= 128, "lane sums must fit 32 bits");
     __shared__ uint32_t tabr[LAC_Q1_TAB_SIZE * kQ1Rep];
@@ -275,6 +299,7 @@
     __shared__ uint64_t ssum[NWB][2];
     __shared__ uint32_t sps[NR];
     __shared__ unsigned long long bins[DEC ? NR : 1][64];
+    __shared__ Q1FuseLds<FUSE> fl;
     const int tid = threadIdx.x, lane = tid & 63, w = BUF ? wave_in_block() : tid >> 6;
     const int g = NR == 1 ? 0 : w / RW, wg = NR == 1 ? w : w % RW;
     int gt = tid - g * NT;
@@ -283,10 +308,21 @@
     const int ntiles = MULTI ? (nvec + NT * R - 1) / (NT * R) : 1;
     const int64_t stride = (int64_t)gridDim.x * NR;
     auto row_of = [&](int64_t r) { return lg + (t0 + r / B) * step_stride + (r % B) * stream_stride; };
+    int64_t fnk = 0, frows = 0;
+    if constexpr (FUSE) {
+        fnk = q1_fuse_own(B, gridDim.x, blockIdx.x);
+        frows = fnk * fa.nsteps;
+    }
+    auto own = [&](int64_t j) { return (int64_t)blockIdx.x + j * (int64_t)gridDim.x; };
+    auto row_at = [&](int64_t t, int64_t j) { return lg + (t0 + t) * step_stride + own(j) * stream_stride; };
     u32x4 x[R];
     if (PF) {
-        const int64_t r0 = (int64_t)blockIdx.x * NR + g;
-        q1_load_tile<R>(x, Src(r0 < rows ? row_of(r0) : lg, r0 < rows, nvec), 0, gt, NT);
+        if constexpr (FUSE) {
+            q1_load_tile<R>(x, Src(frows > 0 ? row_at(0, 0) : lg, frows > 0, nvec), 0, gt, NT);
+        } else {
+            const int64_t r0 = (int64_t)blockIdx.x * NR + g;
+            q1_load_tile<R>(x, Src(r0 < rows ? row_of(r0) : lg, r0 < rows, nvec), 0, gt, NT);
+        }
     }
     if constexpr (R > 8) q1_load_tab_rep<kQ1Rep>(tabr, xsh);
     else q1_fill_tab_rep<kQ1Rep, 64 * NWB>(tabr, xsh);
@@ -303,12 +339,31 @@
             pend_r = -1;
         }
     };
+    if constexpr (FUSE) {
+        for (int64_t js = w; js < fnk; js += NWB) {
+            const int64_t b = own(js);
+            EncState st = (fa.flags & kReset) ? fresh_state(fa.prec) : fa.enc[b];
+            const int64_t live = live_steps(fa.slen, b, st.nsym, fa.nsteps);
+            int dead = 0;
+            if (st.err || st.nflush >= 0) {
+                dead = 1;
+                if (!st.err && live > 0) { st.err = LAC_E_STATE; st.err_step = st.nsym; }
+            }
+            if (lane == 0) {
+                fl.st[js] = st;
+                fl.live[js] = live;
+                fl.dead[js] = dead;
+            }
+        }
+    }
     int par = 0;
-    for (int64_t rb = (int64_t)blockIdx.x * NR; rb < rows; rb += stride, par ^= 1) {
+    int64_t ft = 0, fj = 0;
+    for (int64_t rb = FUSE ? 0 : (int64_t)blockIdx.x * NR; rb < (FUSE ? frows : rows);
+         rb += FUSE ? 1 : stride, par ^= 1) {
         if (R > 8 && !DEC) asm volatile("" : "+v"(gt));
         const int64_t r = rb + g;
-        const bool valid = r < rows;
-        const Src row(valid ? row_of(r) : lg, valid, nvec);
+        const bool valid = FUSE || r < rows;
+        const Src row(FUSE ? row_at(ft, fj) : valid ? row_of(r) : lg, valid, nvec);
         float mx = -INFINITY;
         if (MULTI) {
             for (int tile = 0; tile < ntiles; tile++) {
@@ -379,8 +434,11 @@
         const float c = q1_c(m);
         flush_pending();
         int sfull = -1, sr = 0;
+        int32_t fsym = 0;
         if (!DEC && valid) {
-            const int64_t s = sym[(t0 + r / B) * B + r % B];
+            int64_t s;
+            if constexpr (FUSE) s = fsym = sym[(t0 + ft) * B + own(fj)];
+            else s = sym[(t0 + r / B) * B + r % B];
             const int sc = (int)(s < 0 ? 0 : (s > V ? V : s));
             sfull = sc / N;
             sr = sc - sfull * N;
@@ -415,9 +473,12 @@
                 }
             };
             const int64_t rn = r + stride;
-            const bool nvalid = rn < rows;
+            const bool nvalid = FUSE ? rb + 1 < frows : rn < rows;
             const bool down = MULTI && tile > 0;
-            const Src rroll = down ? row : Src(nvalid ? row_of(rn) : lg, nvalid, nvec);
+            const bool fwrap = fj + 1 == fnk;
+            const Src rroll = down   ? row
+                              : FUSE ? Src(nvalid ? row_at(fwrap ? ft + 1 : ft, fwrap ? 0 : fj + 1) : lg, nvalid, nvec)
+                                     : Src(nvalid ? row_of(rn) : lg, nvalid, nvec);
             const int troll = down ? tile - 1 : 0;
             auto roll = [&](int j) {
                 if (PF) {
@@ -494,17 +555,74 @@
             uint64_t T = 0, L = 0;
 #pragma unroll
             for (int i = 0; i < RW; i++) { T += ssum[g * RW + i][0]; L += ssum[g * RW + i][1]; }
-            RowStats st;
-            st.lo = L;
-            st.hi = L + sps[g];
-            st.tot = T;
-            st.minp = 1;
-            st.inv_tot = 1.0 / (double)T;
-            st.pad = 0;
-            out[r] = st;
+            if constexpr (FUSE) {
+                fl.ring[fj][ft % kQ1FuseBatch] = Q1FuseRow{L, L + sps[g], T, fsym, 0};
+            } else {
+                RowStats st;
+                st.lo = L;
+                st.hi = L + sps[g];
+                st.tot = T;
+                st.minp = 1;
+                st.inv_tot = 1.0 / (double)T;
+                st.pad = 0;
+                out[r] = st;
+            }
+        }
+        if constexpr (FUSE) {
+            if (fj + 1 == fnk && q1_fuse_batch_end(ft, fa.nsteps, kQ1FuseBatch)) {
+                __syncthreads();
+                const int64_t first = q1_fuse_batch_first(ft, kQ1FuseBatch);
+                for (int64_t js = w; js < fnk; js += NWB) {
+                    if (__builtin_amdgcn_readfirstlane(fl.dead[js])) continue;
+                    EncState st = fl.st[js];
+                    if (__builtin_amdgcn_readfirstlane(st.err)) continue;
+                    const int64_t left = (int64_t)rfl_u64((uint64_t)fl.live[js]) - first, cnt = ft - first + 1;
+                    const int n = (int)(left < cnt ? left : cnt);
+                    if (n <= 0) continue;
+                    const int64_t b = own(js);
+                    uint64_t *pa = fa.planeA + (uint64_t)b * fa.cap_words, *pc = fa.planeC + (uint64_t)b * fa.cap_words;
+                    int64_t l = (int64_t)rfl_u64((uint64_t)st.l), h = (int64_t)rfl_u64((uint64_t)st.h);
+                    st.L = rfl_u64(st.L);
+                    st.wa = rfl_u64(st.wa);
+                    st.wc = rfl_u64(st.wc);
+                    st.nsym = (int64_t)rfl_u64((uint64_t)st.nsym);
+                    RowStats my = {0, 0, 0, 0, 0.0, 0};
+                    int32_t mys = 0;
+                    if (lane < n) {
+                        const Q1FuseRow q = fl.ring[js][lane];
+                        my.lo = q.lo;
+                        my.hi = q.hi;
+                        my.tot = q.tot;
+                        my.minp = 1;
+                        my.inv_tot = 1.0 / (double)q.tot;
+                        mys = q.sym;
+                    }
+                    bool ok = true;
+                    encode_block<uint32_t, LAC_MAP_CEIL>(my, mys, n, lane, t0 + first, b, B, (const uint32_t *)nullptr, 0,
+                                                         0, V, fa.prec, st, l, h, pa, pc, fa.cap_words,
+                                                         (uint64_t *)nullptr, false, ok, (NoClock *)nullptr);
+                    if (lane == 0) {
+                        st.l = l;
+                        st.h = h;
+                        fl.st[js] = st;
+                    }
+                }
+            }
+            if (++fj == fnk) { fj = 0; ft++; }
         }
     }
     flush_pending();
+    if constexpr (FUSE) {
+        for (int64_t js = w; js < fnk; js += NWB) {
+            if (lane != 0) continue;
+            const int64_t b = own(js);
+            uint64_t *pa = fa.planeA + (uint64_t)b * fa.cap_words, *pc = fa.planeC + (uint64_t)b * fa.cap_words;
+            EncState st = fl.st[js];
+            if (!fl.dead[js]) store_state(st, st.l, st.h, pa, pc, fa.cap_words, &st);
+            if (fa.flags & kFinish) finish_stream(st, pa, pc, fa.cap_words, fa.prec, &fa.nbits[b], LAC_TERM_FLUSH);
+            fa.enc[b] = st;
+        }
+    }
 }
 
 typedef __attribute__((address_space(3))) void lvoid_t;
@@ -1766,10 +1884,56 @@
         const int64_t need = (a.rows + NR - 1) / NR, cap = (int64_t)c->cus * per_cu;
         const unsigned grid = (unsigned)(need < cap ? need : cap);
         ProfScope ps(c, gate ? -1 : KID_Q1_STATS, st);
-        k_q1_stats<LT, RW, R, DEC, MULTI, PF, NWB><<<grid, 64 * NWB, 0, st>>>(LAC_Q1_ARGS, gate);
+        k_q1_stats<LT, RW, R, DEC, MULTI, PF, NWB><<<grid, 64 * NWB, 0, st>>>(LAC_Q1_ARGS, gate, Q1NoFuse{});
         CHECK_LAUNCH();
         return LAC_OK;
     }
+}
+
+template <typename LT, int I = 0>
+static int q1_fused_form(lac_ctx *c, const Q1Plan &p, const Q1Args *a, const Q1Fuse *fa, unsigned grid,
+                         hipStream_t st) {
+    if constexpr (I == kQ1TiledForms) {
+        return 0;
+    } else {
+        if (p.tiled != I) return q1_fused_form<LT, I + 1>(c, p, a, fa, grid, st);
+        constexpr int RW = kQ1Tiled[I][1], R = kQ1Tiled[I][2], NWB = kQ1Tiled[I][5];
+        constexpr bool MULTI = kQ1Tiled[I][3] != 0, PF = kQ1Tiled[I][4] != 0;
+        if constexpr (RW == NWB && NWB == kQ1Waves && !MULTI && R <= 8) {
+            if (!fa) {
+                static int per_cu = 0;
+                if (!per_cu) {
+                    int n = 0;
+                    if (hipOccupancyMaxActiveBlocksPerMultiprocessor(
+                            &n, k_q1_stats<LT, RW, R, false, MULTI, PF, NWB, true>, 64 * NWB, 0) != hipSuccess ||
+                        n < 1)
+                        n = 1;
+                    per_cu = n;
+                }
+                return per_cu;
+            }
+            ProfScope ps(c, KID_Q1_STATS, st);
+            k_q1_stats<LT, RW, R, false, MULTI, PF, NWB, true><<<grid, 64 * NWB, 0, st>>>(
+                (const LT *)a->lg, a->ss, a->bs, a->sym, c->B, a->rows, c->V, a->t0, a->xsh, p.groups_per_chunk,
+                (RowStats *)nullptr, (uint64_t *)nullptr, (float *)nullptr, (const uint64_t *)nullptr, *fa);
+            CHECK_LAUNCH();
+            return LAC_OK;
+        } else {
+            return 0;
+        }
+    }
+}
+
+template <typename LT>
+static int q1_fuse_choose(lac_ctx *c, bool has_trace, Q1Plan *p, Q1FusePlan *f) {
+    *f = Q1FusePlan();
+    if (q1_plan(c->cus, c->V, (int)sizeof(LT), false, c->q1_shape, p))
+        return fail(LAC_E_ARG, "q1 shape %d does not hold a row of %lld vectors", c->q1_shape,
+                    (long long)(c->V / LogitN<LT>::N));
+    if (p->family != Q1_TILED) return LAC_OK;
+    const int per_cu = q1_fused_form<LT>(c, *p, nullptr, nullptr, 0, nullptr);
+    *f = q1_fuse_plan(c->cus, per_cu, c->B, *p, c->path, has_trace);
+    return LAC_OK;
 }
 
 static int q1_group_setup(lac_ctx *c, const Q1Args &a, hipStream_t st, const Q1Group &g, bool dec, unsigned *grid,
@@ -1846,6 +2010,23 @@
 template <typename LT>
 static int q1_encode(lac_ctx *c, const Q1Args &a0, int64_t steps, uint64_t *trace, hipStream_t st, int flags) {
     int rc;
+    Q1Plan p;
+    Q1FusePlan f;
+    if (steps > 0) {
+        if ((rc = q1_fuse_choose<LT>(c, trace != nullptr, &p, &f))) return rc;
+    }
+    if (f.fused) {
+        for (int64_t t0 = 0; t0 < steps; t0 += c->chunk_steps) {
+            const int64_t n = (steps - t0) < c->chunk_steps ? (steps - t0) : c->chunk_steps;
+            Q1Args a = a0;
+            a.rows = n * c->B;
+            a.t0 = t0;
+            const int fl = (t0 == 0 ? flags & kReset : 0) | (t0 + n >= steps ? flags & kFinish : 0);
+            const Q1Fuse fa{c->enc, c->planeA, c->planeC, c->nbits, c->cap_words, stream_lengths(c), n, c->prec, fl};
+            if ((rc = q1_fused_form<LT>(c, p, &a, &fa, (unsigned)f.grid, st))) return rc;
+        }
+        return LAC_OK;
+    }
     if ((flags & kReset) && (rc = enc_reset_launch(c, st))) return rc;
     for (int64_t t0 = 0; t0 < steps; t0 += c->chunk_steps) {
         const int64_t n = (steps - t0) < c->chunk_steps ? (steps - t0) : c->chunk_steps;
@@ -2067,4 +2248,17 @@
     return LAC_OK;
 }
 
-}
+int lac_q1_fuse_info(lac_ctx *c, int logit_type, int64_t *out5) {
+    if (!c || !out5) return fail(LAC_E_ARG, "NULL argument");
+    if (logit_type != LAC_LOGITS_BF16 && logit_type != LAC_LOGITS_F32) return fail(LAC_E_ARG, "logit type %d", logit_type);
+    HIPCHK(hipSetDevice(c->device));
+    Q1Plan p;
+    Q1FusePlan f;
+    const int rc = logit_type == LAC_LOGITS_BF16 ? q1_fuse_choose<uint16_t>(c, false, &p, &f)
+                                                 : q1_fuse_choose<float>(c, false, &p, &f);
+    if (rc) return rc;
+    out5[0] = f.fused, out5[1] = f.grid, out5[2] = f.max_own, out5[3] = f.batch, out5[4] = f.resident;
+    return LAC_OK;
+}
+
+}
diff --git a/lac_amd/csrc/lac_select.h b/lac_amd/csrc/lac_select.h
--- a/lac_amd/csrc/lac_select.h
+++ b/lac_amd/csrc/lac_select.h
@@ -156,6 +156,49 @@
     if (grouped) p.tiled = q1_tiled_form(p.repair = dec ? 10 : (!bf16 ? 14 : 8));
     *out = p;
     return LAC_OK;
+}
+
+#ifndef LAC_Q1_FUSE_BATCH
+#define LAC_Q1_FUSE_BATCH 16
+#endif
+constexpr int kQ1FuseBatch = LAC_Q1_FUSE_BATCH;
+constexpr int kQ1FuseMaxOwn = 16;
+static_assert(kQ1FuseBatch >= 1 && kQ1FuseBatch <= 64, "a batch is one wave's lanes");
+struct Q1FusePlan {
+    bool fused = false;
+    int64_t grid = 0;
+    int max_own = kQ1FuseMaxOwn;
+    int batch = kQ1FuseBatch;
+    int64_t resident = 0;
+};
+inline Q1FusePlan q1_fuse_plan(int cus, int per_cu, int64_t B, const Q1Plan &plan, int path, bool has_trace) {
+    Q1FusePlan f;
+    if (cus < 1 || per_cu < 1) return f;
+    const int64_t cap = (int64_t)cus * per_cu;
+    f.resident = cap;
+    if (path == LAC_PATH_SPLIT || has_trace || B < 1) return f;
+    if (plan.family != Q1_TILED || plan.tiled < 0) return f;
+    const int *t = kQ1Tiled[plan.tiled];
+    if (t[1] != t[5] || t[3] != 0 || t[5] != 8) return f;
+    if (path != LAC_PATH_FUSED && B < cap) return f;
+    const int64_t G = B < cap ? B : cap;
+    if ((B + G - 1) / G > kQ1FuseMaxOwn) return f;
+    f.fused = true;
+    f.grid = G;
+    return f;
+}
+LAC_SEL_HD inline int64_t q1_fuse_own(int64_t B, int64_t G, int64_t k) { return k < B ? (B - k + G - 1) / G : 0; }
+LAC_SEL_HD inline bool q1_fuse_batch_end(int64_t t, int64_t n, int batch) { return (t + 1) % batch == 0 || t == n - 1; }
+LAC_SEL_HD inline int64_t q1_fuse_batch_first(int64_t t, int batch) { return t / batch * batch; }
+template <typename Visit, typename Batch>
+inline void q1_fuse_walk_host(int64_t B, int64_t G, int64_t n, int batch, Visit visit, Batch bat) {
+    for (int64_t k = 0; k < G; k++) {
+        const int64_t nk = q1_fuse_own(B, G, k);
+        for (int64_t t = 0; t < n; t++) {
+            for (int64_t j = 0; j < nk; j++) visit(k, t, j, k + j * G);
+            if (nk > 0 && q1_fuse_batch_end(t, n, batch)) bat(k, q1_fuse_batch_first(t, batch), t);
+        }
+    }
 }
 
 constexpr int kQ1StepMaxThreads = 1024;
```

Measured after the change: 52.82 million symbols/s. 0.979x the previous value.
